# JeremieDona/spatiotemporal_variable_separation

Hardware: AMD Instinct MI355X
Metric: training frames/sec (seq x nt_pred) (higher is better)
Workload: dtype bf16; 1 GPU; waveeq: mlp enc/dec, batch 128/GPU, nt_cond 5, nt_pred 20, offset 5; global_batch=128, parallelism=dp1, grad_allreduce=none (1 rank), launch=hipGraph replay

## Files before the change

### include/varsep_hip.h

```cpp
#ifndef VARSEP_HIP_H
#define VARSEP_HIP_H

#include <stddef.h>
#include <stdint.h>

#ifdef __cplusplus
extern "C" {
#endif

#define VS_OK 0
#define VS_ERR_ARG (-1)
#define VS_ERR_WORKSPACE (-2)
#define VS_ERR_LAUNCH (-3)
#define VS_ERR_UNSUPPORTED (-4)

#define VS_F32 0
#define VS_BF16 1
#define VS_F16 2

#define VS_ACT_NONE 0
#define VS_ACT_RELU 1
#define VS_ACT_LEAKY 2
#define VS_ACT_SIGMOID 3
#define VS_ACT_TANH 4
// ... 83 lines not shown
int vs_conv3_band_bn_supported(int compute, int B, int Cin, int H, int W, int Cout, int groups);
int vs_conv3_band_bn(int compute, const void* x, const void* w_packed, const float* bias, void* y, int y_dtype, int B, int Cin, int H, int W, int Cout,
                     double* bn_sums, int groups, void* stream);
int vs_conv_k4s2_band_bn(int compute, const void* planes, const void* w_packed, const float* bias, void* y, int y_dtype, int B, int K, int H, int W, int M,
                         double* bn_sums, int groups, void* stream);
int vs_bn_stats_from_sums_fold(double* sums, int groups, int C, int64_t n_per_group, float* mean, float* invstd, float* running_mean, float* running_var,
                               float momentum, float eps, int reset, void* stream);
int vs_conv3_band_bn_parts_rows(int B, int H, int W);
int vs_conv3_band_bn_parts(int compute, const void* x, const void* w_packed, const float* bias, void* y, int y_dtype, int B, int Cin, int H, int W, int Cout,
                           float* parts, int k4, void* stream);
int vs_bn_stats_from_parts_fold(const float* parts, int rows_per_group, int groups, int C, int64_t n_per_group, float* mean, float* invstd,
                                float* var_scratch, float* running_mean, float* running_var, float momentum, float eps, void* stream);
int vs_conv3_wgrad_band_slabs(int B, int Cin, int H, int W, int Cout);
int vs_conv3_wgrad_band(int compute, const void* x, const void* dz, float* slabs, int B, int Cin, int H, int W, int Cout, void* stream);
size_t vs_conv3_img16_bn_workspace_bytes(void);
int vs_conv3_img16_bn_supported(int compute, int B, int Cin, int Cout);
int vs_conv3_img16_bn_form_supported(int backward, int act, int y_dtype, int compute);
int vs_exchange_epoch_advance(void* ws, void* stream);
int vs_conv3_img16_bn_fwd(int compute, const void* x, const void* w_packed, void* ws, unsigned call_idx, const float* bias, const float* gamma,
                          const float* beta, int act, float* running_mean, float* running_var, float momentum, float eps, void* z, void* y, int y_dtype,
                          float* mean, float* invstd, const float* skip, float* xnew, void* xnew16, int B, int Cin, int Cout, void* stream);
int vs_conv3_img16_bn_bwd(int compute, const void* dz_next, const void* w_packed, void* ws, unsigned call_idx, const void* z, const float* mean,
                          const float* invstd, const float* gamma, const float* beta, int act, void* dz, float* dgamma, float* dbeta, int accumulate,
                          int B, int Cin, int Cout, void* stream);
int vs_slab_sum(const float* slabs, int nslabs, const float* bias, const float* addend, void* out, int out_dtype, int B, int C, int64_t HW,
                void* stream);
int vs_slab_sum2(const float* slabs, int nslabs, const float* bias, const float* addend, const float* addend2, void* out, int out_dtype, int B, int C,
                 int64_t HW, void* stream);
int vs_bn_stats_from_sums(const double* sums, int groups, int C, int64_t n_per_group, float* mean, float* invstd, float* var_scratch,
                          float* running_mean, float* running_var, float momentum, float eps, void* stream);

int vs_conv_thin_supported(int compute, int B, int C, int H, int W, int M, int k, int stride, int pad);
int vs_conv_thin_expand(int compute, const void* thin, const void* w, int64_t w_sc, int64_t w_sm, int flip, const float* bias, void* out, int out_dtype,
                        int B, int C, int H, int W, int M, int k, int stride, void* stream);
int vs_conv_thin_reduce(int compute, const void* big, const void* w, int64_t w_sc, int64_t w_sm, int flip, const float* bias, void* out, int out_dtype,
                        int B, int C, int H, int W, int M, int k, int stride, void* stream);
size_t vs_conv_thin_wgrad_workspace_bytes(int B, int C, int H, int W, int M, int k);
int vs_conv_thin_wgrad(int compute, const void* big, const void* thin, float* ws, size_t ws_bytes, const float* addend, float* out, int64_t o_sc,
                       int64_t o_sm, int flip, int B, int C, int H, int W, int M, int k, int stride, void* stream);

int vs_frame_metrics(const float* pred, const float* target, int64_t planes, int H, int W, float max_val, float k1, float k2, float sigma,
                     float* mse, float* ssim, void* stream);

int vs_moving_mnist_batch(const uint8_t* digits, int64_t n_digits_total, int digit_h, int digit_w, const int32_t* init, int batch,
                          int num_digits, int seq_len, int frame_size, void* out, int out_dtype, void* stream);

int vs_moving_mnist_testset(const uint8_t* digits, int64_t n_digits_total, int digit_h, int digit_w, const int32_t* init, int n_videos,
                            int num_digits, int seq_len, int frame_size, void* frames, int frames_fp32, int64_t frame_stride_t,
                            int64_t frame_stride_v, int32_t* latents, void* stream);

int vs_chairs_gather(const uint8_t* frames, int64_t n_objects, int views_per_object, int H, int W, int C, const int32_t* desc, int64_t rows,
                     int seq_len, void* out, int out_dtype, int32_t* bad, void* stream);

int vs_gather_timeline(const float* frames, int64_t n_frames, int64_t frame_elems, const int32_t* first, int64_t n_windows, int step,
                       const int32_t* item_idx, int64_t rows, int seq_len, void* out, int out_dtype, int32_t* bad, void* stream);

int vs_wave_simulate(int n_seq, int T, int frame_size, const float* c2, const float* source, const float* h, const float* init, float* out,
                     float* minmax, int normalise, void* stream);

int vs_resample_u8(const uint8_t* src, int64_t n, int H, int W, int C, int box_x0, int box_y0, int box_w, int box_h, const int32_t* kx,
                   const int32_t* bx, int ksize_x, const int32_t* ky, const int32_t* by, int ksize_y, int out_w, int out_h, uint8_t* out,
                   void* stream);

#define VS_INFLATE_OK 0
#define VS_INFLATE_HEADER 1
#define VS_INFLATE_BLOCK_TYPE 2
#define VS_INFLATE_STORED_LEN 3
#define VS_INFLATE_LENGTHS 4
#define VS_INFLATE_SYMBOL 5
#define VS_INFLATE_DISTANCE 6
#define VS_INFLATE_INPUT 7
#define VS_INFLATE_OUT_LONG 8
#define VS_INFLATE_OUT_SHORT 9
#define VS_INFLATE_ADLER 10
#define VS_PNG_BAD_FILTER 11

int vs_inflate_zlib(const uint8_t* packed, int64_t packed_bytes, const int64_t* offsets, int64_t n, const int64_t* out_len, uint8_t* out,
                    int64_t out_stride, int32_t* status, int64_t* produced, void* stream);

int vs_png_unfilter(const uint8_t* raw, int64_t raw_stride, int64_t n, int H, int W, int C, uint8_t* pixels, int32_t* status, void* stream);

#define VS_DEFLATE_MIN_CHUNK 1024
#define VS_DEFLATE_MAX_CHUNK 32768
#define VS_DEFLATE_SLOT_EXTRA 10
int vs_deflate_chunks(const uint8_t* src, int64_t n_bytes, int chunk_bytes, uint8_t* slots, int64_t slot_stride, int64_t* sizes, void* stream);
int vs_deflate_pack(const uint8_t* slots, int64_t slot_stride, const int64_t* sizes, const int64_t* offsets, int64_t n_chunks, uint8_t* dst,
                    int64_t dst_bytes, void* stream);
int vs_crc32(const uint8_t* src, int64_t n_bytes, int64_t chunk_bytes, uint32_t init, uint32_t* partial, void* stream);

#define VS_MT19937_STATE_WORDS 625
#define VS_MT19937_MAX_COLS 8
#define VS_MT19937_MAX_ROWS (1ll << 40)
int vs_mt19937_randint(uint32_t* state, const int32_t* lows, const int32_t* highs, int k, int64_t n_rows, int32_t* out, int32_t* bad,
                       void* stream);

#define VS_MMNIST_WALK_MAX_PRE 5
#define VS_MMNIST_WALK_MAX_TRAJ (1ll << 24)
#define VS_MMNIST_WALK_STATUS_BOUNCE 3
int vs_mmnist_stochastic_trajectories(uint32_t* state, const int32_t* lows, const int32_t* highs, int n_pre, int64_t n_traj, int seq_len,
                                      int x_max, int y_max, int max_speed, const int32_t* start, int32_t* pre, int32_t* positions,
                                      int32_t* latents, int32_t* desc, int desc_nd, int32_t* bad, void* stream);

int vs_moving_mnist_place(const uint8_t* digits, int64_t n_digits_total, int digit_h, int digit_w, const int32_t* positions, int n_seq,
                          int num_digits, const int32_t* desc, int n_videos, int seq_len, int frame_size, void* out, int out_dtype,
                          int32_t* bad, void* stream);
int vs_frame_metrics_multi(const float* pred, const float* targets, int64_t batch, int n_targets, int64_t planes_per_sample, int H, int W,
                           float max_val, float k1, float k2, float sigma, float* mse, float* ssim, void* stream);
int vs_frames_to_u8_nhwc(const void* x, int x_dtype, int64_t n, int channels, int64_t hw, uint8_t* out, void* stream);
int vs_sst_frame_metrics(const float* pred, const float* target, int64_t rows, int T, int H, int W, const float* consts, int64_t n_days,
                         const int32_t* day0, const int32_t* zone, const float* zone_range, int64_t n_zones, float k1, float k2, float sigma,
                         float* mse, float* ssim, int32_t* bad, void* stream);

int vs_mix_codes_fwd(const float* s, const float* t_rand, const float* t_codes, int64_t B, int n, int Cs, int Ct, int mixing, float* out,
                     void* out_lowp, int lowp_dtype, void* stream);
int vs_mix_codes_bwd(const float* dz, const float* s, const float* t_rand, const float* t_codes, int64_t B, int n, int Cs, int Ct,
                     int mixing, float* ds, float* dt_rand, float* dt_codes, void* stream);

int vs_train_losses_fwd(const float* frames, const float* full, const int32_t* idx, const int32_t* t_random_dev, int ae_shift,
                        int first_forecast, int64_t B, int G, int T, int64_t D,
                        const float* s_old, const float* s_new, int64_t n_s, const float* t0, int64_t Bt, int64_t Ct,
                        int average_tloss, const float* lambdas, float* out, void* stream);
int vs_train_losses_bwd(const float* frames, const float* full, const int32_t* idx, const int32_t* t_random_dev, int ae_shift,
                        int first_forecast, int64_t B, int G, int T, int64_t D,
                        const float* s_old, const float* s_new, int64_t n_s, const float* t0, int64_t Bt, int64_t Ct,
                        int average_tloss, const float* lambdas, const float* grad_total, float* dframes, float* ds_old,
                        float* ds_new, float* dt0, int frames_act, void* dz, int dz_dtype, void* stream);
int vs_train_losses_fwd_grad(const float* frames, const float* full, const int32_t* idx, const int32_t* t_random_dev, int ae_shift,
                             int first_forecast, int64_t B, int G, int T, int64_t D, const float* s_old, const float* s_new, int64_t n_s,
                             const float* t0, int64_t Bt, int64_t Ct, int average_tloss, const float* lambdas, float* out,
                             const float* grad_total, float* ds_old, float* ds_new, float* dt0, int frames_act, void* dz, int dz_dtype,
                             void* stream);

int vs_gemm_frame_loss(int compute, int64_t M, int64_t N, int64_t K, const void* A, int64_t lda, const void* W, int64_t ldw,
                       const float* bias, int act, const float* full, const int32_t* t_random_dev, int ae_shift, int first_forecast,
                       int G, int T, const float* s_old, const float* s_new, int64_t n_s, const float* t0, int64_t Bt, int64_t Ct,
                       int average_tloss, const float* lambdas, const float* grad_total, void* dz, int dz_dtype, float* ds_old,
                       float* ds_new, float* dt0, float* out, void* stream);

int vs_adam_multi(int n_tensors, float* const* params, const void* const* grads, const int32_t* grad_dtype, float* const* exp_avg,
                  float* const* exp_avg_sq, void* const* shadow_bf16, const int64_t* numel, const int32_t* skipped, int32_t* step,
                  double lr, double beta1, double beta2, double eps, void* stream);
int vs_adam_step_increment(int32_t* step, void* stream);

int vs_check_finite_multi(int n_tensors, const void* const* grads, const int32_t* grad_dtype, const int64_t* numel, float* found_inf,
                          void* stream);
int vs_adam_multi_scaled(int n_tensors, float* const* params, const void* const* grads, const int32_t* grad_dtype, float* const* exp_avg,
                         float* const* exp_avg_sq, void* const* shadow, int shadow_dtype, const int64_t* numel, const int32_t* skipped,
                         int32_t* step, double lr, double beta1, double beta2, double eps, const float* scale_state, void* stream);
int vs_adam_step_increment_scaled(int32_t* step, const float* scale_state, void* stream);
int vs_adam_set_max_blocks(int blocks);
int vs_gemm_adam(int compute, int64_t M, int64_t N, int64_t K, const void* A, int64_t lda, int layout_a, const void* B, int64_t ldb,
                 int layout_b, float alpha, float* param, float* exp_avg, float* exp_avg_sq, void* shadow, int shadow_dtype,
                 const int32_t* step, int32_t skipped, double lr, double beta1, double beta2, double eps, void* stream);
int vs_loss_scale_update(float* scale_state, float growth_factor, float backoff_factor, int growth_interval, void* stream);

int vs_frames_sse_fwd(const float* frames, const float* full, const int32_t* idx, int64_t B, int G, int T, int64_t D, float* sums,
                      void* stream);
int vs_frames_sse_bwd(const float* frames, const float* full, const int32_t* idx, int64_t B, int G, int T, int64_t D, const float* coef,
                      float* dframes, void* stream);

int vs_cat_bcast_fwd(const void* a, int a_dtype, const void* x, int x_dtype, void* out, int out_dtype, int B, int n, int Ca, int Cb, int64_t HW, void* stream);
int vs_cat_bcast_bwd(const void* dout, int dout_dtype, void* da, int a_dtype, void* dx, int x_dtype, int B, int n, int Ca, int Cb, int64_t HW, void* stream);
int64_t vs_code_losses_chunks(int n_pairs, const int64_t* count, int64_t t_count);
int vs_code_losses_fwd(int n_pairs, const void* const* a, const void* const* b, const int* dtype, const int64_t* count, const float* t0, int64_t t_count,
                       const float* sse_ae, const float* sse_pred, float scale_ae, float scale_pred, float l_ae, float l_s, float l_pred, float l_t,
                       float inv_s, float inv_t, float* partial, float* out, void* stream);
int vs_code_losses_bwd(int n_pairs, const void* const* a, const void* const* b, void* const* da, void* const* db, const int* dtype, const int64_t* count,
                       const float* t0, float* dt0, int64_t t_count, const float* g, float scale_ae, float scale_pred, float l_ae, float l_s, float l_pred,
                       float l_t, float inv_s, float inv_t, float* coefs, void* stream);

int vs_act_bwd(const void* dy, int dy_dtype, const void* y, int y_dtype, void* dz, int dz_dtype, int act,
               int64_t n, void* stream);

int vs_act_fwd(const void* x, int x_dtype, void* y, int y_dtype, int act, int64_t n, void* stream);

int vs_transpose_cast(const void* src, int src_dtype, void* dst, int dst_dtype, int rows, int cols, void* stream);

size_t vs_rollout_packed_elems(int compute, int N, int K);
int vs_pack_rollout_weight(int compute, const float* src, int transpose, int N, int K, void* dst, void* stream);
int vs_pack_rollout_weights(int compute, int n_jobs, const float* const* src, const int* transpose, const int* N, const int* K,
                            void* const* dst, void* stream);

int vs_mlp_rollout_parts(int compute, int B, int C, int H);
size_t vs_mlp_rollout_workspace_bytes(int compute, int B, int C, int H);
int vs_mlp_rollout_xcd_local_get(int compute, int B, int C, int H, int n_blocks);
int vs_mlp_rollout_xcd_local_set(int allowed);
int vs_exchange_guard_set(void* word);
void* vs_exchange_guard_get(void);
int vs_exchange_skip_counter_set(void* word);
int vs_mlp_rollout_fwd(int compute, int B, int C, int H, int n_blocks, int n_steps, const float* x0,
                       const void* const* weights, const float* const* biases, float* t_codes, float* residuals,
                       void* xin_save, void* h1_save, void* h2_save, uint32_t* m1_save, uint32_t* m2_save, void* workspace,
                       size_t workspace_bytes, void* stream);

int vs_mlp_rollout_bwd(int compute, int B, int C, int H, int n_blocks, int n_steps, const float* grad_t_codes,
                       const void* const* weights_t, const void* h1_save, const void* h2_save,
                       const uint32_t* m1_save, const uint32_t* m2_save, float* dx0,
                       void* dr_save, void* dh2_save, void* dh1_save, void* workspace, size_t workspace_bytes, void* stream);

size_t vs_conv_workspace_bytes(int compute, int B, int Cin, int H, int W, int Cout, int kh, int kw, int stride, int pad);
size_t vs_conv_wgrad_workspace_bytes(int B, int Cin, int OH, int OW, int Cout, int kh, int kw);
size_t vs_conv_packed_elems(int D0, int D1, int kh, int kw, int stride, int pad);
int vs_conv_pack_weight(int compute, const float* w, int D0, int D1, int kh, int kw, int stride, int pad, void* dst, void* stream);
int vs_conv2d_fwd(int compute, const void* x, const void* w, const float* bias, void* y, int y_dtype, int B, int Cin, int H, int W,
                  int Cout, int kh, int kw, int stride, int pad, void* workspace, size_t workspace_bytes, void* stream);
int vs_conv2d_dgrad(int compute, const void* dy, const void* w_packed, void* dx, int dx_dtype, int B, int Cin, int H, int W, int Cout, int kh,
                    int kw, int stride, int pad, void* workspace, size_t workspace_bytes, void* stream);
int vs_conv2d_wgrad(int compute, const void* dy, const void* x, float* dw, int B, int Cin, int H, int W, int Cout, int kh, int kw,
                    int stride, int pad, void* workspace, size_t workspace_bytes, void* stream);
int vs_conv2d_wgrad_acc(int compute, const void* dy, const void* x, float* dw, int B, int Cin, int H, int W, int Cout, int kh, int kw,
                        int stride, int pad, void* workspace, size_t workspace_bytes, int accumulate, void* stream);
int vs_conv_transpose2d_wgrad_acc(int compute, const void* dy, const void* x, float* dw, int B, int Cin, int H, int W, int Cout, int kh,
                                  int kw, int stride, int pad, void* workspace, size_t workspace_bytes, int accumulate, void* stream);
int vs_conv_transpose2d_fwd(int compute, const void* x, const void* w_packed, const float* bias, void* y, int y_dtype, int B, int Cin, int H,
                            int W, int Cout, int kh, int kw, int stride, int pad, void* workspace, size_t workspace_bytes, void* stream);
int vs_conv_transpose2d_dgrad(int compute, const void* dy, const void* w, void* dx, int dx_dtype, int B, int Cin, int H, int W, int Cout,
                              int kh, int kw, int stride, int pad, void* workspace, size_t workspace_bytes, int cols_from_wgrad, void* stream);
int vs_conv_transpose2d_wgrad(int compute, const void* dy, const void* x, float* dw, int B, int Cin, int H, int W, int Cout, int kh,
                              int kw, int stride, int pad, void* workspace, size_t workspace_bytes, void* stream);

int vs_maxpool3s2_fwd(const void* x, int x_dtype, void* y, int y_dtype, int64_t planes, int H, int W, void* stream);
int vs_maxpool3s2_bwd(const void* x, int x_dtype, const void* dy, int dy_dtype, void* dx, int dx_dtype, int64_t planes, int H, int W,
                      void* stream);

int vs_bn_stats(const void* x, int x_dtype, int B, int C, int64_t HW, int groups, float* mean, float* invstd, float* var_scratch,
                float* running_mean, float* running_var, float momentum, float eps, void* stream);
int vs_bn_train_fwd_small_supported(int x_dtype, int B, int C, int64_t HW);
int vs_bn_train_fwd_small(const void* x, int x_dtype, void* y, int y_dtype, const float* gamma, const float* beta, int act, float* mean,
                          float* invstd, float* running_mean, float* running_var, float momentum, float eps, int B, int C, int64_t HW,
                          void* stream);
int vs_bn_train_fwd_small_groups(const void* x, int x_dtype, void* y, int y_dtype, const float* gamma, const float* beta, int act, float* mean,
                                 float* invstd, float* var_scratch, float* running_mean, float* running_var, float momentum, float eps, int B, int C,
                                 int64_t HW, int groups, void* stream);
int vs_bn_train_fwd_small_slabs(const float* slabs, int nslabs, const float* bias, void* z, int z_dtype, void* y, int y_dtype, const float* gamma,
                                const float* beta, int act, float* mean, float* invstd, float* running_mean, float* running_var,
                                float momentum, float eps, const float* skip, float* xnew, void* xnew16, int B, int C, int64_t HW,
                                void* stream);
int vs_bn_act_bwd_small_ex(const void* dy_a, int dy_a_dtype, const float* dy_b, const float* slabs, int nslabs, const void* z, int z_dtype,
                           const float* mean, const float* invstd, const float* gamma, const float* beta, int act, float* dgamma,
                           float* dbeta, int accumulate, void* dx, int dx_dtype, int B, int C, int64_t HW, void* stream);
int vs_bn_train_fwd_slab_supported(int x_dtype, int Bg, int C, int64_t HW);
int vs_bn_train_fwd_slab(const void* x, int x_dtype, void* y, int y_dtype, const float* gamma, const float* beta, int act, float* mean, float* invstd,
                         float* var_scratch, float* running_mean, float* running_var, float momentum, float eps, int B, int C, int64_t HW, int groups,
                         void* stream);
int vs_bn_act_fwd(const void* x, int x_dtype, void* y, int y_dtype, const float* mean, const float* invstd, const float* gamma,
                  const float* beta, int act, int B, int C, int64_t HW, int groups, void* stream);
int vs_bn_act_bwd(const void* dy, int dy_dtype, const void* x, int x_dtype, const float* mean, const float* invstd, const float* gamma,
                  const float* beta, int act, int training, int groups, float* dgamma, float* dbeta, void* dx, int dx_dtype, int B,
                  int C, int64_t HW, void* stream);
int vs_bn_act_bwd_gsum(const void* dy, int dy_dtype, const void* x, int x_dtype, const float* mean, const float* invstd, const float* gamma,
                       const float* beta, int act, int training, int groups, float* dgamma, float* dbeta, void* dx, int dx_dtype, int B,
                       int C, int64_t HW, float* dgamma_sum, float* dbeta_sum, void* stream);
int vs_bn_stats_ub(const void* x, int x_dtype, int B, int C, int64_t HW, int groups, float* mean, float* invstd, float* ubvar, float eps, void* stream);
int vs_bn_act_fwd_running(const void* x, int x_dtype, void* y, int y_dtype, const float* mean, const float* invstd, const float* gamma, const float* beta,
                          int act, int B, int C, int64_t HW, int groups, const float* ubvar, float* running_mean, float* running_var, float momentum,
                          void* stream);
int vs_chan_sum(const void* x, int x_dtype, int B, int C, int64_t HW, float* out, void* stream);
size_t vs_chan_sum_workspace_bytes(int B, int C, int64_t HW);
int vs_chan_sum_ws(const void* x, int x_dtype, int B, int C, int64_t HW, void* ws, size_t ws_bytes, float* out, void* stream);
int vs_maxpool2_fwd(const void* x, int x_dtype, void* y, int y_dtype, int64_t planes, int H, int W, void* stream);
int vs_maxpool2_bwd(const void* x, int x_dtype, const void* dy, int dy_dtype, void* dx, int dx_dtype, int64_t planes, int H, int W,
                    void* stream);
int vs_upsample2_fwd(const void* x, int x_dtype, void* y, int y_dtype, int64_t planes, int H, int W, void* stream);
int vs_upsample2_bwd(const void* dy, int dy_dtype, void* dx, int dx_dtype, int64_t planes, int H, int W, void* stream);

#ifdef __cplusplus
}
#endif
#endif
```

### spatiotemporal_variable_separation_amd/_lib.py

```python
import ctypes
import os
import subprocess
import sys
from concurrent.futures import ThreadPoolExecutor

import torch

_HERE = os.path.dirname(os.path.abspath(__file__))
_CSRC = os.path.join(_HERE, 'csrc')
LIB_PATH = os.path.join(_HERE, 'libvarsep_hip.so')
SOURCES = ['vs_gemm.hip', 'vs_eltwise.hip', 'vs_conv.hip', 'vs_rollout.hip', 'vs_norm.hip', 'vs_optim.hip', 'vs_data.hip', 'vs_conv_tap.hip', 'vs_metrics.hip', 'vs_conv_img.hip', 'vs_conv_k4s2.hip',
           'vs_conv_thin.hip', 'vs_conv_band2.hip', 'vs_conv_wgrad2.hip', 'vs_eval.hip', 'vs_wave_sim.hip', 'vs_resample.hip', 'vs_png.hip', 'vs_deflate.hip',
           'vs_mt19937.hip', 'vs_mmnist_walk.hip']

F32, BF16, F16 = 0, 1, 2
TORCH_DTYPE = {F32: torch.float32, BF16: torch.bfloat16, F16: torch.float16}
ACT = {'none': 0, None: 0, 'identity': 0, 'relu': 1, 'leaky_relu': 2, 'sigmoid': 3, 'tanh': 4, 'elu': 5}
LAYOUT_R, LAYOUT_S = 0, 1

_lib = None


class VarsepHipError(RuntimeError):
    pass


def _sources():
    return [os.path.join(_CSRC, s) for s in SOURCES if os.path.exists(os.path.join(_CSRC, s))]


def _headers():
    import glob
    return sorted(glob.glob(os.path.join(_CSRC, '*.h'))) + [os.path.join(_HERE, '..', 'include', 'varsep_hip.h')]


def _deps(src, _seen=None):
    import re
    seen = _seen if _seen is not None else set()
    if src in seen or not os.path.exists(src):
        return seen
    seen.add(src)
    with open(src, errors='replace') as f:
        for name in re.findall(r'^\s*#\s*include\s+"([^"]+)"', f.read(), flags=re.M):
            for d in (os.path.dirname(src), _CSRC, os.path.join(_HERE, '..', 'include')):
                cand = os.path.normpath(os.path.join(d, name))
                if os.path.exists(cand):
                    _deps(cand, seen)
                    break
    return seen


def library_is_stale():
    if not os.path.exists(LIB_PATH):
        return True
    t = os.path.getmtime(LIB_PATH)
    return any(os.path.getmtime(d) > t for d in _sources() + _headers())


def build_library(force=False, verbose=False):
    if not force and not library_is_stale():
        return LIB_PATH
    hipcc = os.environ.get('HIPCC', '/opt/rocm/bin/hipcc')
    objdir = os.path.join(_HERE, 'build')
    os.makedirs(objdir, exist_ok=True)
    flags = ['--offload-arch=gfx950', '-O3', '-std=c++17', '-fPIC'] + os.environ.get('VARSEP_HIPCC_FLAGS', '').split()

    def compile_one(src):
        obj = os.path.join(objdir, os.path.basename(src) + '.o')
        if not force and os.path.exists(obj) and os.path.getmtime(obj) > max(os.path.getmtime(d) for d in _deps(src)):
            return obj
        cmd = [hipcc] + flags + ['-c', src, '-o', obj]
        r = subprocess.run(cmd, capture_output=True, text=True)
        if r.returncode != 0:
            raise VarsepHipError('hipcc failed for %s:\n%s' % (src, r.stderr[-4000:]))
        if verbose:
            print('compiled', os.path.basename(src), file=sys.stderr)
        return obj

    with ThreadPoolExecutor(max_workers=4) as ex:
        objs = list(ex.map(compile_one, _sources()))
    tmp = LIB_PATH + '.tmp'
    r = subprocess.run([hipcc, '--offload-arch=gfx950', '-shared', '-fPIC', '-o', tmp] + objs, capture_output=True, text=True)
    if r.returncode != 0:
        raise VarsepHipError('link failed:\n' + r.stderr[-4000:])
    os.replace(tmp, LIB_PATH)
    return LIB_PATH


_i64, _i32, _f32, _vp, _sz = ctypes.c_int64, ctypes.c_int, ctypes.c_float, ctypes.c_void_p, ctypes.c_size_t

SIGNATURES = {
    'vs_version': (ctypes.c_char_p, []),
    'vs_last_error': (ctypes.c_char_p, []),
    'vs_gemm_workspace_bytes': (_sz, [_i64, _i64, _i64]),
    'vs_gemm_plan': (_i32, [_i32, _i32, _i64, _i64, _i64, _vp, _i64, _i64, _i32, _vp, _i64, _i64, _i32, ctypes.POINTER(_i64)]),
    'vs_gemm': (_i32, [_i32, _i64, _i64, _i64, _vp, _i64, _i32, _vp, _i64, _i32, _vp, _i64, _i32, _f32, _vp, _i32,
                       _vp, _i64, _i32, _i32, _i32, _vp, _sz, _vp]),
    'vs_cast': (_i32, [_vp, _i32, _vp, _i32, _i64, _vp]),
    'vs_copy2d': (_i32, [_vp, _i32, _i64, _vp, _i32, _i64, _i64, _i64, _vp, _i64, _vp]),
    'vs_copy2d_pair': (_i32, [_vp, _i32, _i64, _vp, _i32, _i64, _i64, _i64, _vp, _i64, _i64, _i64, _vp]),
    'vs_colsum': (_i32, [_vp, _i32, _i64, _i64, _i64, _vp, _i32, _vp]),
    'vs_colsum_multi': (_i32, [_i32, _vp, _vp, _vp, _vp, _vp, _vp, _vp, _i64, _vp]),
    'vs_adam_multi': (_i32, [_i32, _vp, _vp, _vp, _vp, _vp, _vp, _vp, _vp, _vp, ctypes.c_double, ctypes.c_double, ctypes.c_double,
                             ctypes.c_double, _vp]),
    'vs_adam_step_increment': (_i32, [_vp, _vp]),
    'vs_check_finite_multi': (_i32, [_i32, _vp, _vp, _vp, _vp, _vp]),
    'vs_adam_set_max_blocks': (_i32, [_i32]),
    'vs_gemm_adam': (_i32, [_i32, _i64, _i64, _i64, _vp, _i64, _i32, _vp, _i64, _i32, ctypes.c_float, _vp, _vp, _vp, _vp, _i32, _vp, _i32,
                     ctypes.c_double, ctypes.c_double, ctypes.c_double, ctypes.c_double, _vp]),
    'vs_adam_multi_scaled': (_i32, [_i32, _vp, _vp, _vp, _vp, _vp, _vp, _i32, _vp, _vp, _vp, ctypes.c_double, ctypes.c_double, ctypes.c_double,
                                    ctypes.c_double, _vp, _vp]),
    'vs_adam_step_increment_scaled': (_i32, [_vp, _vp, _vp]),
    'vs_loss_scale_update': (_i32, [_vp, _f32, _f32, _i32, _vp]),
    'vs_gemm_batched_workspace_bytes': (_sz, [_i32, _i64, _i64, _i64]),
    'vs_gemm_batched': (_i32, [_i32, _i32, _i64, _i64, _i64, _vp, _i64, _i64, _i32, _vp, _i64, _i64, _i32, _vp, _i64, _i64, _i32, _f32, _i32,
                               _vp, _sz, _vp]),
    'vs_train_losses_fwd': (_i32, [_vp, _vp, _vp, _vp, _i32, _i32, _i64, _i32, _i32, _i64, _vp, _vp, _i64, _vp, _i64, _i64, _i32, _vp, _vp, _vp]),
    'vs_train_losses_fwd_grad': (_i32, [_vp, _vp, _vp, _vp, _i32, _i32, _i64, _i32, _i32, _i64, _vp, _vp, _i64, _vp, _i64, _i64, _i32, _vp, _vp,
                                        _vp, _vp, _vp, _vp, _i32, _vp, _i32, _vp]),
    'vs_gemm_frame_loss': (_i32, [_i32, _i64, _i64, _i64, _vp, _i64, _vp, _i64, _vp, _i32, _vp, _vp, _i32, _i32, _i32, _i32, _vp, _vp, _i64, _vp, _i64,
                                  _i64, _i32, _vp, _vp, _vp, _i32, _vp, _vp, _vp, _vp, _vp]),
    'vs_train_losses_bwd': (_i32, [_vp, _vp, _vp, _vp, _i32, _i32, _i64, _i32, _i32, _i64, _vp, _vp, _i64, _vp, _i64, _i64, _i32, _vp, _vp, _vp, _vp,
                                   _vp, _vp, _i32, _vp, _i32, _vp]),
    'vs_convt_tap_supported': (_i32, [_i32] * 7),
    'vs_convt_tap_packed_elems': (_sz, [_i32, _i32]),
    'vs_convt_tap_pack_weight': (_i32, [_i32, _vp, _i32, _i32, _vp, _vp]),
    'vs_convt_k4s2_tap_fwd': (_i32, [_i32, _vp, _vp, _vp, _vp, _vp] + [_i32] * 6 + [_vp]),
    'vs_convt_k4s2_tap_fwd_f32': (_i32, [_i32, _vp, _vp, _vp, _vp] + [_i32] * 5 + [_vp]),
    'vs_conv_k3_tap_supported': (_i32, [_i32] * 7),
    'vs_conv_k3_tap_packed_elems': (_sz, [_i32, _i32]),
    'vs_conv_k3_tap_pack_weight': (_i32, [_i32, _vp, _i32, _i32, _i32, _vp, _vp]),
    'vs_conv_k3s1_tap_fwd': (_i32, [_i32, _vp, _vp, _vp, _vp, _i32, _vp] + [_i32] * 6 + [_vp]),
    'vs_bn_stats_from_sums': (_i32, [_vp, _i32, _i32, _i64, _vp, _vp, _vp, _vp, _vp, _f32, _f32, _vp]),
    'vs_moving_mnist_batch': (_i32, [_vp, _i64, _i32, _i32, _vp, _i32, _i32, _i32, _i32, _vp, _i32, _vp]),
    'vs_moving_mnist_testset': (_i32, [_vp, _i64, _i32, _i32, _vp, _i32, _i32, _i32, _i32, _vp, _i32, _i64, _i64, _vp, _vp]),
    'vs_chairs_gather': (_i32, [_vp, _i64, _i32, _i32, _i32, _i32, _vp, _i64, _i32, _vp, _i32, _vp, _vp]),
    'vs_gather_timeline': (_i32, [_vp, _i64, _i64, _vp, _i64, _i32, _vp, _i64, _i32, _vp, _i32, _vp, _vp]),
    'vs_gather_windows': (_i32, [_vp, _i64, _i64, _i64, _vp, _i32, _i32, _i32, _vp, _i32, _vp, _i32, _vp]),
    'vs_wave_simulate': (_i32, [_i32, _i32, _i32, _vp, _vp, _vp, _vp, _vp, _vp, _i32, _vp]),
    'vs_resample_u8': (_i32, [_vp, _i64, _i32, _i32, _i32, _i32, _i32, _i32, _i32, _vp, _vp, _i32, _vp, _vp, _i32, _i32, _i32, _vp, _vp]),
    'vs_inflate_zlib': (_i32, [_vp, _i64, _vp, _i64, _vp, _vp, _i64, _vp, _vp, _vp]),
    'vs_png_unfilter': (_i32, [_vp, _i64, _i64, _i32, _i32, _i32, _vp, _vp, _vp]),
    'vs_deflate_chunks': (_i32, [_vp, _i64, _i32, _vp, _i64, _vp, _vp]),
    'vs_deflate_pack': (_i32, [_vp, _i64, _vp, _vp, _i64, _vp, _i64, _vp]),
    'vs_crc32': (_i32, [_vp, _i64, _i64, ctypes.c_uint32, _vp, _vp]),
    'vs_mt19937_randint': (_i32, [_vp, _vp, _vp, _i32, _i64, _vp, _vp, _vp]),
    'vs_mmnist_stochastic_trajectories': (_i32, [_vp, _vp, _vp, _i32, _i64, _i32, _i32, _i32, _i32, _vp, _vp, _vp, _vp, _vp, _i32, _vp, _vp]),
    'vs_mix_codes_fwd': (_i32, [_vp, _vp, _vp, _i64, _i32, _i32, _i32, _i32, _vp, _vp, _i32, _vp]),
    'vs_mix_codes_bwd': (_i32, [_vp, _vp, _vp, _vp, _i64, _i32, _i32, _i32, _i32, _vp, _vp, _vp, _vp]),
    'vs_pack_rollout_weights': (_i32, [_i32, _i32, _vp, _vp, _vp, _vp, _vp, _vp]),
    'vs_frames_sse_fwd': (_i32, [_vp, _vp, _vp, _i64, _i32, _i32, _i64, _vp, _vp]),
    'vs_frames_sse_bwd': (_i32, [_vp, _vp, _vp, _i64, _i32, _i32, _i64, _vp, _vp, _vp]),
    'vs_cat_bcast_fwd': (_i32, [_vp, _i32, _vp, _i32, _vp, _i32, _i32, _i32, _i32, _i32, _i64, _vp]),
    'vs_cat_bcast_bwd': (_i32, [_vp, _i32, _vp, _i32, _vp, _i32, _i32, _i32, _i32, _i32, _i64, _vp]),
    'vs_code_losses_chunks': (_i64, [_i32, _vp, _i64]),
    'vs_code_losses_fwd': (_i32, [_i32, _vp, _vp, _vp, _vp, _vp, _i64, _vp, _vp, ctypes.c_float, ctypes.c_float, ctypes.c_float, ctypes.c_float, ctypes.c_float, ctypes.c_float, ctypes.c_float, ctypes.c_float, _vp, _vp, _vp]),
    'vs_code_losses_bwd': (_i32, [_i32, _vp, _vp, _vp, _vp, _vp, _vp, _vp, _vp, _i64, _vp, ctypes.c_float, ctypes.c_float, ctypes.c_float, ctypes.c_float, ctypes.c_float, ctypes.c_float, ctypes.c_float, ctypes.c_float, _vp, _vp]),
    'vs_act_bwd': (_i32, [_vp, _i32, _vp, _i32, _vp, _i32, _i32, _i64, _vp]),
    'vs_act_fwd': (_i32, [_vp, _i32, _vp, _i32, _i32, _i64, _vp]),
    'vs_conv_wgrad_workspace_bytes': (_sz, [_i32] * 7),
    'vs_conv_packed_elems': (_sz, [_i32] * 6),
    'vs_conv_pack_weight': (_i32, [_i32, _vp, _i32, _i32, _i32, _i32, _i32, _i32, _vp, _vp]),
    'vs_conv_workspace_bytes': (_sz, [_i32] * 10),
    'vs_conv2d_fwd': (_i32, [_i32, _vp, _vp, _vp, _vp, _i32] + [_i32] * 9 + [_vp, _sz, _vp]),
    'vs_conv2d_dgrad': (_i32, [_i32, _vp, _vp, _vp, _i32] + [_i32] * 9 + [_vp, _sz, _vp]),
    'vs_conv2d_wgrad': (_i32, [_i32, _vp, _vp, _vp] + [_i32] * 9 + [_vp, _sz, _vp]),
    'vs_frame_metrics': (_i32, [_vp, _vp, _i64, _i32, _i32, ctypes.c_float, ctypes.c_float, ctypes.c_float, ctypes.c_float, _vp, _vp, _vp]),
    'vs_moving_mnist_place': (_i32, [_vp, _i64, _i32, _i32, _vp, _i32, _i32, _vp, _i32, _i32, _i32, _vp, _i32, _vp, _vp]),
    'vs_frame_metrics_multi': (_i32, [_vp, _vp, _i64, _i32, _i64, _i32, _i32, _f32, _f32, _f32, _f32, _vp, _vp, _vp]),
    'vs_frames_to_u8_nhwc': (_i32, [_vp, _i32, _i64, _i32, _i64, _vp, _vp]),
    'vs_sst_frame_metrics': (_i32, [_vp, _vp, _i64, _i32, _i32, _i32, _vp, _i64, _vp, _vp, _vp, _i64, _f32, _f32, _f32, _vp, _vp, _vp, _vp]),
    'vs_conv3_img16_supported': (_i32, [_i32] * 6),
    'vs_conv3_img16_splits': (_i32, [_i32] * 3),
    'vs_conv3_img16_packed_elems': (_sz, [_i32, _i32]),
    'vs_conv3_img16_pack_weight': (_i32, [_i32, _vp, _i32, _i32, _i32, _vp, _vp]),
    'vs_conv3_img16_pack_weights': (_i32, [_i32, _i32, _vp, _vp, _vp, _vp, _vp, _vp]),
    'vs_conv3_img16': (_i32, [_i32, _vp, _vp, _vp, _i32, _i32, _i32, _vp]),
    'vs_space_to_depth2_supported': (_i32, [_i32] * 5),
    'vs_space_to_depth2': (_i32, [_i32, _vp, _vp, _i32, _i32, _i32, _i32, _vp]),
    'vs_conv_k4s2_packed_elems': (_sz, [_i32, _i32]),
    'vs_conv_k4s2_pack_weight': (_i32, [_i32, _vp, _i32, _i32, _vp, _vp]),
    'vs_conv_k4s2_wgrad_finish': (_i32, [_vp, _i32, _vp, _vp, _i32, _i32, _vp]),
    'vs_conv_k4s2_skip_form': (_i32, [_i32]),
    'vs_conv_k4s2_band': (_i32, [_i32, _vp, _vp, _vp, _vp, _i32, _i32, _i32, _i32, _i32, _i32, _vp]),
    'vs_conv_k4s2_wgrad_band': (_i32, [_i32, _vp, _vp, _vp, _i32, _i32, _i32, _i32, _i32, _vp]),
    'vs_conv_k4s2_wgrad_band_slabs': (_i32, [_i32, _i32, _i32, _i32, _i32]),
    'vs_conv_thin_supported': (_i32, [_i32] * 9),
    'vs_conv_thin_expand': (_i32, [_i32, _vp, _vp, _i64, _i64, _i32, _vp, _vp, _i32] + [_i32] * 7 + [_vp]),
    'vs_conv_thin_reduce': (_i32, [_i32, _vp, _vp, _i64, _i64, _i32, _vp, _vp, _i32] + [_i32] * 7 + [_vp]),
    'vs_conv_thin_wgrad_workspace_bytes': (_sz, [_i32] * 6),
    'vs_conv_thin_wgrad': (_i32, [_i32, _vp, _vp, _vp, _sz, _vp, _vp, _i64, _i64, _i32] + [_i32] * 7 + [_vp]),
    'vs_conv3_band_supported': (_i32, [_i32] * 6),
    'vs_conv3_band_bn_supported': (_i32, [_i32] * 7),
    'vs_conv3_band_bn': (_i32, [_i32, _vp, _vp, _vp, _vp, _i32, _i32, _i32, _i32, _i32, _i32, _vp, _i32, _vp]),
    'vs_conv_k4s2_band_bn': (_i32, [_i32, _vp, _vp, _vp, _vp, _i32, _i32, _i32, _i32, _i32, _i32, _vp, _i32, _vp]),
    'vs_bn_stats_from_sums_fold': (_i32, [_vp, _i32, _i32, _i64, _vp, _vp, _vp, _vp, ctypes.c_float, ctypes.c_float, _i32, _vp]),
    'vs_conv3_band_bn_parts_rows': (_i32, [_i32, _i32, _i32]),
    'vs_conv3_band_bn_parts': (_i32, [_i32, _vp, _vp, _vp, _vp, _i32, _i32, _i32, _i32, _i32, _i32, _vp, _i32, _vp]),
    'vs_bn_stats_from_parts_fold': (_i32, [_vp, _i32, _i32, _i32, _i64, _vp, _vp, _vp, _vp, _vp, ctypes.c_float, ctypes.c_float, _vp]),
    'vs_conv3_band': (_i32, [_i32, _vp, _vp, _vp, _vp, _i32, _i32, _i32, _i32, _i32, _i32, _vp]),
    'vs_conv3_wgrad_band_supported': (_i32, [_i32] * 6),
    'vs_conv3_wgrad_band_slabs': (_i32, [_i32] * 5),
    'vs_conv3_wgrad_band': (_i32, [_i32, _vp, _vp, _vp, _i32, _i32, _i32, _i32, _i32, _vp]),
    'vs_conv3_wgrad_band_pieces': (_i32, [_i32, _i32, _vp, _vp, _i32, _vp, _i32, _i32, _i32, _i32, _vp]),
    'vs_conv3_wgrad_band_finish': (_i32, [_vp, _i32, _vp, _vp, _i32, _i32, _vp]),
    'vs_slab_sum_grouped': (_i32, [_vp, _i32, _i32, _vp, _i64, _vp]),
    'vs_slab_sum': (_i32, [_vp, _i32, _vp, _vp, _vp, _i32, _i32, _i32, _i64, _vp]),
    'vs_slab_sum2': (_i32, [_vp, _i32, _vp, _vp, _vp, _vp, _i32, _i32, _i32, _i64, _vp]),
    'vs_conv3_img16_bn_workspace_bytes': (ctypes.c_size_t, []),
    'vs_conv3_img16_bn_supported': (_i32, [_i32, _i32, _i32, _i32]),
    'vs_conv3_img16_bn_form_supported': (_i32, [_i32, _i32, _i32, _i32]),
    'vs_exchange_epoch_advance': (_i32, [_vp, _vp]),
    'vs_conv3_img16_bn_fwd': (_i32, [_i32, _vp, _vp, _vp, ctypes.c_uint, _vp, _vp, _vp, _i32, _vp, _vp, ctypes.c_float, ctypes.c_float, _vp, _vp, _i32,
                                     _vp, _vp, _vp, _vp, _vp, _i32, _i32, _i32, _vp]),
    'vs_conv3_img16_bn_bwd': (_i32, [_i32, _vp, _vp, _vp, ctypes.c_uint, _vp, _vp, _vp, _vp, _vp, _i32, _vp, _vp, _vp, _i32, _i32, _i32, _i32, _vp]),
    'vs_bn_train_fwd_small_slabs': (_i32, [_vp, _i32, _vp, _vp, _i32, _vp, _i32, _vp, _vp, _i32, _vp, _vp, _vp, _vp, ctypes.c_float, ctypes.c_float,
                                           _vp, _vp, _vp, _i32, _i32, _i64, _vp]),
    'vs_bn_act_bwd_small_ex': (_i32, [_vp, _i32, _vp, _vp, _i32, _vp, _i32, _vp, _vp, _vp, _vp, _i32, _vp, _vp, _i32, _vp, _i32, _i32, _i32, _i64, _vp]),
    'vs_bn_train_fwd_small_supported': (_i32, [_i32, _i32, _i32, _i64]),
    'vs_bn_train_fwd_small': (_i32, [_vp, _i32, _vp, _i32, _vp, _vp, _i32, _vp, _vp, _vp, _vp, ctypes.c_float, ctypes.c_float, _i32, _i32, _i64, _vp]),
    'vs_bn_train_fwd_small_groups': (_i32, [_vp, _i32, _vp, _i32, _vp, _vp, _i32, _vp, _vp, _vp, _vp, _vp, ctypes.c_float, ctypes.c_float, _i32, _i32, _i64, _i32,
                                            _vp]),
    'vs_conv2d_wgrad_acc': (_i32, [_i32, _vp, _vp, _vp] + [_i32] * 9 + [_vp, _sz, _i32, _vp]),
    'vs_conv_transpose2d_wgrad_acc': (_i32, [_i32, _vp, _vp, _vp] + [_i32] * 9 + [_vp, _sz, _i32, _vp]),
    'vs_conv_transpose2d_fwd': (_i32, [_i32, _vp, _vp, _vp, _vp, _i32] + [_i32] * 9 + [_vp, _sz, _vp]),
    'vs_conv_transpose2d_dgrad': (_i32, [_i32, _vp, _vp, _vp, _i32] + [_i32] * 9 + [_vp, _sz, _i32, _vp]),
    'vs_conv_transpose2d_wgrad': (_i32, [_i32, _vp, _vp, _vp] + [_i32] * 9 + [_vp, _sz, _vp]),
    'vs_bn_stats': (_i32, [_vp, _i32, _i32, _i32, _i64, _i32, _vp, _vp, _vp, _vp, _vp, _f32, _f32, _vp]),
    'vs_bn_train_fwd_slab_supported': (_i32, [_i32, _i32, _i32, _i64]),
    'vs_bn_train_fwd_slab': (_i32, [_vp, _i32, _vp, _i32, _vp, _vp, _i32, _vp, _vp, _vp, _vp, _vp, ctypes.c_float, ctypes.c_float, _i32, _i32, _i64, _i32, _vp]),
    'vs_bn_act_fwd': (_i32, [_vp, _i32, _vp, _i32, _vp, _vp, _vp, _vp, _i32, _i32, _i32, _i64, _i32, _vp]),
    'vs_bn_act_bwd': (_i32, [_vp, _i32, _vp, _i32, _vp, _vp, _vp, _vp, _i32, _i32, _i32, _vp, _vp, _vp, _i32, _i32, _i32, _i64, _vp]),
    'vs_bn_act_bwd_gsum': (_i32, [_vp, _i32, _vp, _i32, _vp, _vp, _vp, _vp, _i32, _i32, _i32, _vp, _vp, _vp, _i32, _i32, _i32, _i64, _vp, _vp, _vp]),
    'vs_bn_stats_ub': (_i32, [_vp, _i32, _i32, _i32, _i64, _i32, _vp, _vp, _vp, ctypes.c_float, _vp]),
    'vs_bn_act_fwd_running': (_i32, [_vp, _i32, _vp, _i32, _vp, _vp, _vp, _vp, _i32, _i32, _i32, _i64, _i32, _vp, _vp, _vp, ctypes.c_float, _vp]),
    'vs_chan_sum': (_i32, [_vp, _i32, _i32, _i32, _i64, _vp, _vp]),
    'vs_chan_sum_workspace_bytes': (_sz, [_i32, _i32, _i64]),
    'vs_chan_sum_ws': (_i32, [_vp, _i32, _i32, _i32, _i64, _vp, _sz, _vp, _vp]),
    'vs_maxpool2_fwd': (_i32, [_vp, _i32, _vp, _i32, _i64, _i32, _i32, _vp]),
    'vs_maxpool2_bwd': (_i32, [_vp, _i32, _vp, _i32, _vp, _i32, _i64, _i32, _i32, _vp]),
    'vs_maxpool3s2_fwd': (_i32, [_vp, _i32, _vp, _i32, _i64, _i32, _i32, _vp]),
    'vs_maxpool3s2_bwd': (_i32, [_vp, _i32, _vp, _i32, _vp, _i32, _i64, _i32, _i32, _vp]),
    'vs_upsample2_fwd': (_i32, [_vp, _i32, _vp, _i32, _i64, _i32, _i32, _vp]),
    'vs_upsample2_bwd': (_i32, [_vp, _i32, _vp, _i32, _i64, _i32, _i32, _vp]),
    'vs_transpose_cast': (_i32, [_vp, _i32, _vp, _i32, _i32, _i32, _vp]),
    'vs_rollout_packed_elems': (_sz, [_i32, _i32, _i32]),
    'vs_pack_rollout_weight': (_i32, [_i32, _vp, _i32, _i32, _i32, _vp, _vp]),
    'vs_mlp_rollout_parts': (_i32, [_i32] * 4),
    'vs_mlp_rollout_workspace_bytes': (_sz, [_i32] * 4),
    'vs_mlp_rollout_xcd_local_get': (_i32, [_i32] * 5),
    'vs_mlp_rollout_xcd_local_set': (_i32, [_i32]),
    'vs_exchange_guard_set': (_i32, [_vp]),
    'vs_exchange_guard_get': (_vp, []),
    'vs_exchange_skip_counter_set': (_i32, [_vp]),
    'vs_mlp_rollout_fwd': (_i32, [_i32] * 6 + [_vp] * 11 + [_sz, _vp]),
    'vs_mlp_rollout_bwd': (_i32, [_i32] * 6 + [_vp] * 11 + [_sz, _vp]),
}


def load_library():
    global _lib
    if _lib is not None:
# ... 46 lines not shown
```

### spatiotemporal_variable_separation_amd/csrc/vs_gemm.hip

```cpp
#include <type_traits>
#include "vs_gemm_plan.h"
#include "vs_loss.h"

namespace {

struct GemmCall {
    const void* A; int64_t lda; int la;
    const void* B; int64_t ldb; int lb;
    int64_t M, N, K;
    int batch;
    hipStream_t stream;
};

template <int V> using IC = std::integral_constant<int, V>;
template <class F>
int with_compute(int compute, F&& f) {
    return compute == VS_BF16 ? f(IC<VS_BF16>{}) : compute == VS_F16 ? f(IC<VS_F16>{}) : f(IC<VS_F32>{});
}
template <class F>
int with_types(int compute, int la, int lb, F&& f) {
    return with_compute(compute, [&](auto ct) {
        if (la == LR && lb == LR) return f(ct, IC<LR>{}, IC<LR>{});
        if (la == LR && lb == LS) return f(ct, IC<LR>{}, IC<LS>{});
        if (la == LS && lb == LR) return f(ct, IC<LS>{}, IC<LR>{});
        return f(ct, IC<LS>{}, IC<LS>{});
    });
}

template <int CT, int LA, int LB, int BM, int BN>
int launch(const GemmCall& c, const GemmPlan& plan, const Epi& epi, float* slabs) {
    typedef typename CTraits<CT>::T T;
    constexpr int BK = bk_of<CT>();
    constexpr int U = CTraits<CT>::U;
    Dense<CT, LA> a{(const T*)c.A, c.lda, c.M, c.K, ((uintptr_t)c.A % 16 == 0) && (c.lda % U == 0) && (epi.batch_a % U == 0)};
    Dense<CT, LB> b{(const T*)c.B, c.ldb, c.N, c.K, ((uintptr_t)c.B % 16 == 0) && (c.ldb % U == 0) && (epi.batch_b % U == 0)};
    constexpr size_t smem = (TileGeom<CT, LA, BM, BK>::ELEMS + TileGeom<CT, LB, BN, BK>::ELEMS) * sizeof(T);
    dim3 grid((unsigned)vs_cdiv(c.N, BN), (unsigned)vs_cdiv(c.M, BM), (unsigned)(plan.splits * c.batch));
    Epi e = epi;
    e.xcd_runs = (int64_t)grid.x * grid.y * grid.z >= 64;
    hipLaunchKernelGGL((gemm_kernel<CT, Dense<CT, LA>, Dense<CT, LB>, BM, BN, BK>), grid, dim3(256), smem, c.stream, a, b, c.M, c.N,
                       c.K, (int)plan.k_tiles_per_split, e, slabs);
    VS_CHECK_LAUNCH("vs_gemm");
    return VS_OK;
}

template <int CT, int LA, int LB>
int launch_reg(const GemmCall& c, const GemmPlan& plan, const Epi& epi, float* slabs) {
    if (plan.bm == 128 && plan.bn == 128) return launch<CT, LA, LB, 128, 128>(c, plan, epi, slabs);
    if (plan.bm == 128 && plan.bn == 64) return launch<CT, LA, LB, 128, 64>(c, plan, epi, slabs);
    if constexpr (CT != VS_F32)
        if (plan.bm == 64 && plan.bn == 128) return launch<CT, LA, LB, 64, 128>(c, plan, epi, slabs);
    return launch<CT, LA, LB, 64, 64>(c, plan, epi, slabs);
}

template <int CT, int LA, int LB>
int launch_glds(const GemmCall& c, const GemmPlan& plan, const Epi& epi, float* slabs) {
    if constexpr (CT == VS_F32) {
        return vs_fail(VS_ERR_UNSUPPORTED, "vs_gemm: the LDS-DMA 128x128 tile is a 16-bit kernel");
    } else {
        dim3 grid((unsigned)vs_cdiv(c.N, 128), (unsigned)vs_cdiv(c.M, 128), (unsigned)(plan.splits * c.batch));
        static const int forced = getenv("VS_GEMM_GLDS_STAGES") ? atoi(getenv("VS_GEMM_GLDS_STAGES")) : 0;
        const int stages = forced ? forced : ((int64_t)grid.x * grid.y * grid.z >= 1024 ? 2 : 1);
        if (stages == 2)
            hipLaunchKernelGGL((gemm_glds_kernel<LA, LB, false, 2, CT>), grid, dim3(256), 65536, c.stream, (const __bf16*)c.A, c.lda, (const __bf16*)c.B,
                               c.ldb, c.M, c.N, c.K, (int)plan.k_tiles_per_split, epi, slabs);
        else
            hipLaunchKernelGGL((gemm_glds_kernel<LA, LB, false, 1, CT>), grid, dim3(256), 32768, c.stream, (const __bf16*)c.A, c.lda, (const __bf16*)c.B,
                               c.ldb, c.M, c.N, c.K, (int)plan.k_tiles_per_split, epi, slabs);
        VS_CHECK_LAUNCH("vs_gemm (LDS-DMA tile)");
        return VS_OK;
    }
}

template <int CT, int LA, int LB, bool LOSS = false>
int launch_big(const GemmCall& c, const GemmPlan& bp, const Epi& epi, float* slabs) {
    if constexpr (CT == VS_F32) {
        return vs_fail(VS_ERR_UNSUPPORTED, "vs_gemm: the 256x256 tile is a 16-bit kernel");
    } else {
        auto kfn = gemm_big_kernel<CT, LA, LB, false, LOSS>;
        static bool attr_set = false;
        if (!attr_set) {
            if (hipFuncSetAttribute((const void*)kfn, hipFuncAttributeMaxDynamicSharedMemorySize, GEMM_BIG_STAGES * BIG_TILE_BYTES) != hipSuccess)
                return vs_fail(VS_ERR_LAUNCH, "vs_gemm: cannot raise the dynamic LDS limit to 160 KiB");
            attr_set = true;
        }
        dim3 grid((unsigned)(bp.tiles_m * bp.tiles_n), 1, (unsigned)(bp.splits * c.batch));
        hipLaunchKernelGGL(kfn, grid, dim3(512), GEMM_BIG_STAGES * BIG_TILE_BYTES, c.stream, (const unsigned short*)c.A, c.lda, (const unsigned short*)c.B,
                           c.ldb, c.M, c.N, c.K, (int)bp.k_tiles_per_split, bp.tiles_n, epi, slabs);
        VS_CHECK_LAUNCH("vs_gemm (256x256 tile)");
        return VS_OK;
    }
}

template <int CT, int LA, int LB, int NI, int LOSS = 0, int MI = 4>
int launch_p8(const GemmCall& c, const GemmPlan& pp, const Epi& epi, float* slabs) {
    if constexpr (CT == VS_F32) {
        return vs_fail(VS_ERR_UNSUPPORTED, "vs_gemm: the staggered 256-row tile is a 16-bit kernel");
    } else {
        auto kfn = gemm_p8_kernel<CT, LA, LB, NI, false, LOSS, MI>;
        constexpr int lds = 2 * (2 * 32 * MI * P8_BK * 2 + 2 * 64 * NI * P8_BK * 2);
        static bool attr_set = false;
        if (!attr_set) {
            if (hipFuncSetAttribute((const void*)kfn, hipFuncAttributeMaxDynamicSharedMemorySize, lds) != hipSuccess)
                return vs_fail(VS_ERR_LAUNCH, "vs_gemm: cannot raise the dynamic LDS limit to %d bytes", lds);
            attr_set = true;
        }
        dim3 grid((unsigned)(pp.tiles_m * pp.tiles_n), 1, (unsigned)(pp.splits * c.batch));
        hipLaunchKernelGGL(kfn, grid, dim3(512), lds, c.stream, (const unsigned short*)c.A, c.lda, (const unsigned short*)c.B, c.ldb, c.M, c.N, c.K,
                           (int)pp.k_tiles_per_split, pp.tiles_n, epi, slabs);
        VS_CHECK_LAUNCH("vs_gemm (staggered 256-row tile)");
        return VS_OK;
    }
}

template <int CT, int LA, int LB>
int launch_mid(const GemmCall& c, const GemmPlan& mp, const Epi& epi, float* slabs) {
    const int rc = mid_launch<CT, LA, LB>(c.A, c.lda, c.B, c.ldb, c.M, c.N, c.K, mp.splits, mp.k_tiles_per_split, mp.stages, c.batch, epi, slabs, c.stream);
    if (rc != VS_OK) return rc;
    VS_CHECK_LAUNCH("vs_gemm (128x128 ring tile)");
    return VS_OK;
}

int launch_plan(int compute, const GemmCall& c, const GemmPlan& p, const Epi& epi, float* slabs) {
    return with_types(compute, c.la, c.lb, [&](auto ct, auto la, auto lb) -> int {
        constexpr int CT = decltype(ct)::value, LA = decltype(la)::value, LB = decltype(lb)::value;
        switch (p.kind) {
            case GEMM_P8:
                if (p.ni == 1 && p.mi == 2) return launch_p8<CT, LA, LB, 1, 0, 2>(c, p, epi, slabs);
                if (p.ni == 1) return launch_p8<CT, LA, LB, 1>(c, p, epi, slabs);
                return launch_p8<CT, LA, LB, 2>(c, p, epi, slabs);
            case GEMM_BIG: return launch_big<CT, LA, LB>(c, p, epi, slabs);
            case GEMM_MID: return launch_mid<CT, LA, LB>(c, p, epi, slabs);
            case GEMM_GLDS: return launch_glds<CT, LA, LB>(c, p, epi, slabs);
            default: return launch_reg<CT, LA, LB>(c, p, epi, slabs);
        }
    });
}

constexpr unsigned SK_POOL = 1u << 20;
}
__device__ unsigned vs_sk_pool[1u << 20];
namespace {

constexpr int64_t SK_FUSED_MAX_BYTES = 96 << 10;
unsigned* sk_take(int64_t words, int64_t tile_slab_bytes) {
    static unsigned* base = nullptr;
    static unsigned next = 0;
    const char* env = getenv("VS_GEMM_SPLITK_FUSED");
    const int fused = env ? atoi(env) : 0;
    if (!fused || words <= 0 || words > SK_POOL / 4 || (fused == 1 && tile_slab_bytes > SK_FUSED_MAX_BYTES)) return nullptr;
    if (!base && hipGetSymbolAddress((void**)&base, HIP_SYMBOL(vs_sk_pool)) != hipSuccess) { base = nullptr; return nullptr; }
    if (next + words > SK_POOL) next = 0;
    unsigned* p = base + next;
    next += (unsigned)words;
    return p;
}

int run_gemm(const char* who, int compute, const GemmCall& c, const GemmPlan& plan, Epi epi, void* workspace, size_t workspace_bytes) {
    float* slabs = nullptr;
    if (plan.splits > 1) {
        const size_t need = gemm_slab_bytes(plan, c.M, c.N, c.batch);
        if (!workspace || workspace_bytes < need)
            return vs_fail(VS_ERR_WORKSPACE, "%s: split-K needs %zu workspace bytes, got %zu", who, need, workspace_bytes);
        slabs = (float*)workspace;
        if (gemm_splitk_in_launch(plan)) {
            epi.sk_counters = sk_take(gemm_splitk_counters(plan, c.M, c.N, c.batch), gemm_splitk_tile_bytes(plan));
            epi.sk_splits = plan.splits;
            epi.sk_bytes = (int64_t)need;
        }
    }
    const int rc = launch_plan(compute, c, plan, epi, slabs);
    if (rc != VS_OK) return rc;
    if (slabs && !epi.sk_counters) return launch_splitk_reduce(slabs, plan.splits, c.M, c.N, epi, c.batch, c.stream);
    return VS_OK;
}

}

extern "C" size_t vs_gemm_workspace_bytes(int64_t M, int64_t N, int64_t K) { return gemm_workspace_bytes(M, N, K, 1); }
extern "C" size_t vs_gemm_batched_workspace_bytes(int batch, int64_t M, int64_t N, int64_t K) { return gemm_workspace_bytes(M, N, K, batch); }

extern "C" int vs_gemm_plan(int compute, int batch, int64_t M, int64_t N, int64_t K, const void* A, int64_t lda, int64_t stride_a, int layout_a,
                            const void* B, int64_t ldb, int64_t stride_b, int layout_b, int64_t* out) {
    VS_CHECK_ARG(vs_dtype_ok(compute), "vs_gemm_plan: compute type %d", compute);
    VS_CHECK_ARG(batch >= 1 && batch <= 1024 && M > 0 && N > 0 && K > 0, "vs_gemm_plan: bad sizes");
    VS_CHECK_ARG((layout_a == LR || layout_a == LS) && (layout_b == LR || layout_b == LS), "vs_gemm_plan: bad layout");
    VS_CHECK_ARG(out, "vs_gemm_plan: null pointer");
    const GemmPlan p = plan_gemm(compute, M, N, K, batch, A, lda, layout_a, stride_a, B, ldb, layout_b, stride_b);
    const int64_t row[12] = {p.kind, p.bm, p.bn, p.splits, p.k_tiles_per_split, p.tiles_m, p.tiles_n, p.stages, p.ni, p.mi,
                             gemm_splitk_in_launch(p) && gemm_splitk_counters(p, M, N, batch) > 0, (int64_t)gemm_slab_bytes(p, M, N, batch)};
    memcpy(out, row, sizeof(row));
    return VS_OK;
}

extern "C" int vs_gemm_batched(int compute, int batch, int64_t M, int64_t N, int64_t K, const void* A, int64_t lda, int64_t stride_a,
                               int layout_a, const void* B, int64_t ldb, int64_t stride_b, int layout_b, void* C, int64_t ldc,
                               int64_t stride_c, int c_dtype, float alpha, int accumulate, void* workspace, size_t workspace_bytes,
                               void* stream_) {
    VS_CHECK_ARG(vs_dtype_ok(compute), "vs_gemm_batched: compute type %d", compute);
    VS_CHECK_ARG(batch >= 1 && batch <= 1024 && M > 0 && N > 0 && K > 0, "vs_gemm_batched: bad sizes");
    VS_CHECK_ARG(A && B && C, "vs_gemm_batched: null operand");
    VS_CHECK_ARG((layout_a == LR || layout_a == LS) && (layout_b == LR || layout_b == LS), "vs_gemm_batched: bad layout");
    VS_CHECK_ARG(vs_dtype_ok(c_dtype), "vs_gemm_batched: bad c_dtype");
    VS_CHECK_ARG(lda >= (layout_a == LR ? K : M) && ldb >= (layout_b == LR ? K : N) && ldc >= N, "vs_gemm_batched: leading dimension too small");
    const GemmPlan plan = plan_gemm(compute, M, N, K, batch, A, lda, layout_a, stride_a, B, ldb, layout_b, stride_b);
    Epi epi = plain_epi(C, ldc, c_dtype, alpha);
    epi.accumulate = accumulate;
    epi.splits_per_batch = plan.splits;
    epi.batch_a = stride_a; epi.batch_b = stride_b; epi.batch_c = stride_c;
    const GemmCall call{A, lda, layout_a, B, ldb, layout_b, M, N, K, batch, (hipStream_t)stream_};
    return run_gemm("vs_gemm_batched", compute, call, plan, epi, workspace, workspace_bytes);
}

extern "C" int vs_gemm_adam(int compute, int64_t M, int64_t N, int64_t K, const void* A, int64_t lda, int layout_a, const void* B, int64_t ldb,
                            int layout_b, float alpha, float* param, float* exp_avg, float* exp_avg_sq, void* shadow, int shadow_dtype,
                            const int32_t* step, int32_t skipped, double lr, double beta1, double beta2, double eps, void* stream_) {
    VS_CHECK_ARG(compute == VS_BF16 || compute == VS_F16, "vs_gemm_adam: 16-bit compute types only (%d)", compute);
    VS_CHECK_ARG(M > 0 && N > 0 && K > 0, "vs_gemm_adam: M, N, K must be positive");
    VS_CHECK_ARG(A && B && param && exp_avg && exp_avg_sq && step, "vs_gemm_adam: null pointer");
    VS_CHECK_ARG((layout_a == LR || layout_a == LS) && (layout_b == LR || layout_b == LS), "vs_gemm_adam: bad layout");
    VS_CHECK_ARG(lda >= (layout_a == LR ? K : M) && ldb >= (layout_b == LR ? K : N), "vs_gemm_adam: leading dimension too small");
    VS_CHECK_ARG(!shadow || shadow_dtype == VS_BF16 || shadow_dtype == VS_F16, "vs_gemm_adam: bad shadow dtype");
    if (!dma_operands_ok(GEMM_MID, A, lda, layout_a, 0, B, ldb, layout_b, 0, M, N, K))
        return vs_fail(VS_ERR_UNSUPPORTED, "vs_gemm_adam: operands do not fit the LDS-DMA loader (16-byte alignment, multiples of 8)");
    Epi epi = plain_epi(param, N, VS_F32, alpha);
    epi.adam_m = exp_avg; epi.adam_v = exp_avg_sq; epi.adam_shadow = (unsigned short*)shadow; epi.adam_shadow_dtype = shadow_dtype;
    epi.adam_step = step; epi.adam_skipped = skipped; epi.adam_guard = vs_g_exchange_guard;
    epi.adam_lr = lr; epi.adam_beta1 = beta1; epi.adam_beta2 = beta2; epi.adam_eps = (float)eps;
    const GemmPlan mp = ring_plan_one_split(M, N, K);
    if ((int64_t)mp.tiles_m * mp.tiles_n > 0x7fffffffll) return vs_fail(VS_ERR_UNSUPPORTED, "vs_gemm_adam: too many tiles");
    const GemmCall call{A, lda, layout_a, B, ldb, layout_b, M, N, K, 1, (hipStream_t)stream_};
    return launch_plan(compute, call, mp, epi, nullptr);
}

extern "C" int vs_gemm_frame_loss(int compute, int64_t M, int64_t N, int64_t K, const void* A, int64_t lda, const void* W, int64_t ldw,
                                  const float* bias, int act, const float* full, const int32_t* t_random_dev, int ae_shift, int first_forecast,
                                  int G, int T, const float* s_old, const float* s_new, int64_t n_s, const float* t0, int64_t Bt, int64_t Ct,
                                  int average_tloss, const float* lambdas, const float* grad_total, void* dz, int dz_dtype, float* ds_old,
                                  float* ds_new, float* dt0, float* out, void* stream_) {
    hipStream_t stream = (hipStream_t)stream_;
    VS_CHECK_ARG(compute == VS_BF16 || compute == VS_F16, "vs_gemm_frame_loss: 16-bit compute types only (%d)", compute);
    VS_CHECK_ARG(M > 0 && M < (1ll << 31) && N > 0 && K > 0 && G >= 1 && M % G == 0 && N % 4 == 0, "vs_gemm_frame_loss: bad sizes (rows = B * G, N %% 4 == 0)");
    VS_CHECK_ARG(!bias || ((uintptr_t)bias & 15) == 0, "vs_gemm_frame_loss: the bias must be 16-byte aligned");
    VS_CHECK_ARG(A && W && full && t_random_dev && grad_total && dz && dt0 && out && (n_s == 0 || (ds_old && ds_new)), "vs_gemm_frame_loss: null pointer");
    VS_CHECK_ARG(lda >= K && ldw >= K, "vs_gemm_frame_loss: leading dimension too small");
    VS_CHECK_ARG(vs_dtype_ok(dz_dtype) && act >= VS_ACT_NONE && act <= VS_ACT_ELU, "vs_gemm_frame_loss: bad dz dtype / activation");
    LossArgs a;
    int rc = fill_loss_args(a, nullptr, full, nullptr, t_random_dev, ae_shift, first_forecast, M / G, G, T, N, s_old, s_new, n_s, t0, Bt, Ct,
                            average_tloss, lambdas);
    if (rc != VS_OK) return rc;
    const GemmPlan pp = p8_plan(compute, M, N, K, 1), bp = big_plan(compute, M, N, K, 1);
    auto takes = [&](const GemmPlan& p) {
        return p.use && dma_operands_ok(p.kind, A, lda, LR, 0, W, ldw, LR, 0, M, N, K) && p.splits == 1 && (int64_t)p.tiles_m * p.tiles_n <= VS_LOSS_MAX_PARTIALS;
    };
    const bool p8 = takes(pp) && pp.ni == 2;
    if (!p8 && !takes(bp)) return vs_fail(VS_ERR_UNSUPPORTED, "vs_gemm_frame_loss: the problem does not run on the 256x256 tile kernels");
    Epi epi = plain_epi(nullptr, N, VS_F32, 1.f);
    epi.bias = bias; epi.act = act;
    epi.fl_full = full; epi.fl_tdev = t_random_dev; epi.fl_ae_shift = ae_shift; epi.fl_first = first_forecast; epi.fl_G = G; epi.fl_T = T;
    epi.fl_up = grad_total; epi.fl_l_ae = a.l_ae; epi.fl_l_pred = a.l_pred; epi.fl_inv_ae = a.inv_ae; epi.fl_inv_pred = a.inv_pred;
    epi.fl_dz = dz; epi.fl_dz_dtype = dz_dtype; epi.fl_partials = out + 16;
    const GemmCall call{A, lda, LR, W, ldw, LR, M, N, K, 1, stream};
    rc = with_compute(compute, [&](auto ct) -> int {
        constexpr int CT = decltype(ct)::value;
        if (p8 && act == VS_ACT_SIGMOID) return launch_p8<CT, LR, LR, 2, 2>(call, pp, epi, nullptr);
        if (p8) return launch_p8<CT, LR, LR, 2, 1>(call, pp, epi, nullptr);
        return launch_big<CT, LR, LR, true>(call, bp, epi, nullptr);
    });
    if (rc != VS_OK) return rc;
    LossGrads gr{grad_total, dz, dz_dtype, act, ds_old, ds_new, dt0};
    hipLaunchKernelGGL(frame_loss_finish_kernel, dim3(1), dim3(256), 0, stream, a, out, p8 ? pp.tiles_m * pp.tiles_n : bp.tiles_m * bp.tiles_n, gr);
    VS_CHECK_LAUNCH("vs_gemm_frame_loss");
    return VS_OK;
}

extern "C" int vs_gemm(int compute, int64_t M, int64_t N, int64_t K, const void* A, int64_t lda, int layout_a, const void* B,
                       int64_t ldb, int layout_b, void* C, int64_t ldc, int c_dtype, float alpha, const float* bias, int act,
                       const void* mask, int64_t ldmask, int mask_dtype, int mask_act, int accumulate, void* workspace,
                       size_t workspace_bytes, void* stream_) {
    VS_CHECK_ARG(vs_dtype_ok(compute), "vs_gemm: compute type %d", compute);
    VS_CHECK_ARG(M > 0 && N > 0 && K > 0, "vs_gemm: M, N, K must be positive (%lld %lld %lld)", (long long)M, (long long)N, (long long)K);
    VS_CHECK_ARG(A && B && C, "vs_gemm: null operand");
    VS_CHECK_ARG((layout_a == LR || layout_a == LS) && (layout_b == LR || layout_b == LS), "vs_gemm: bad layout");
    VS_CHECK_ARG(vs_dtype_ok(c_dtype) && (!mask || vs_dtype_ok(mask_dtype)), "vs_gemm: bad c_dtype / mask_dtype");
    VS_CHECK_ARG(lda >= (layout_a == LR ? K : M) && ldb >= (layout_b == LR ? K : N) && ldc >= N, "vs_gemm: leading dimension too small");
    VS_CHECK_ARG(!mask || ldmask >= N, "vs_gemm: ldmask too small");
    VS_CHECK_ARG(act >= VS_ACT_NONE && act <= VS_ACT_ELU, "vs_gemm: bad activation");
    Epi epi = plain_epi(C, ldc, c_dtype, alpha);
    epi.bias = bias; epi.act = act;
    epi.mask = mask; epi.ldmask = ldmask; epi.mask_dtype = mask_dtype; epi.mask_act = mask_act;
    epi.accumulate = accumulate;
    const GemmPlan plan = plan_gemm(compute, M, N, K, 1, A, lda, layout_a, 0, B, ldb, layout_b, 0);
    const GemmCall call{A, lda, layout_a, B, ldb, layout_b, M, N, K, 1, (hipStream_t)stream_};
    return run_gemm("vs_gemm", compute, call, plan, epi, workspace, workspace_bytes);
}
```

### spatiotemporal_variable_separation_amd/csrc/vs_gemm_big.h

```cpp
#pragma once
#include <type_traits>
#include "vs_gemm_glds.h"

namespace {

constexpr int BIG_BK = 32;
constexpr int BIG_STAGES = 4;
#define VS_GB_ST 5
#define VS_GB_WAIT_FIRST 16
#define VS_GB_WAIT_LOOP 12
#define VS_STR_(x) #x
#define VS_STR(x) VS_STR_(x)
static_assert(VS_GB_WAIT_FIRST == 4 * (VS_GB_ST - 1) && VS_GB_WAIT_LOOP == 4 * (VS_GB_ST - 2), "vmcnt immediates follow the ring depth");
constexpr int GEMM_BIG_STAGES = VS_GB_ST;
constexpr int BIG_TILE_BYTES = 4 * 8192;

template <int LAYOUT>
struct BigOperand {
    const char* base;
    uint32_t voff[2];
    int kofs;
    int64_t step;

    __device__ __forceinline__ void prepare(const unsigned short* p, int64_t ld, int64_t rows, int64_t i0, int64_t k_begin) {
        const int u = (int)threadIdx.x;
#pragma unroll
        for (int h = 0; h < 2; ++h) {
            const int64_t first = i0 + 128 * h;
            if (LAYOUT == LR) {
                const int row = u >> 2, piece = (u & 3) ^ ((row >> 2) & 3);
                int64_t r = first + row;
                if (r > rows - 1) r = rows - 1;
                kofs = piece * 8;
                voff[h] = (uint32_t)(((r - i0) * ld + piece * 8) * 2);
            } else {
                const int k = u >> 4, piece = (u & 15) ^ ((k & 3) << 2);
                int64_t c = first + piece * 8;
                if (c > rows - 8) c = rows - 8;
                kofs = k;
                voff[h] = (uint32_t)((k * ld + (c - i0)) * 2);
            }
        }
        if (LAYOUT == LR) {
            base = reinterpret_cast<const char*>(p + i0 * ld + k_begin);
            step = BIG_BK * 2;
        } else {
            base = reinterpret_cast<const char*>(p + k_begin * ld + i0);
            step = BIG_BK * ld * 2;
        }
    }
    __device__ __forceinline__ void advance() { base += step; }
    __device__ __forceinline__ void stage(int h, char* lds) const {
        const uint32_t dst = (uint32_t)(uintptr_t)lds;
        asm volatile("s_mov_b32 m0, %0\n\ts_nop 0\n\tglobal_load_lds_dwordx4 %1, %2" ::"s"(dst), "v"(voff[h]), "s"(base) : "memory", "m0");
    }
    __device__ __forceinline__ void stage_checked(int h, char* lds, int64_t k0, int64_t K, bool live) const {
        const void* g = (live && k0 + kofs < K) ? (const void*)(base + voff[h]) : (const void*)vs_glds_zero;
        const uint32_t dst = (uint32_t)(uintptr_t)lds;
        asm volatile("s_mov_b32 m0, %0\n\ts_nop 0\n\tglobal_load_lds_dwordx4 %1, off" ::"s"(dst), "v"(g) : "memory", "m0");
    }
};

template <int LAYOUT>
__device__ __forceinline__ u32x4 big_frag(const unsigned short* tile, int row0, int kk, int lane) {
    if (LAYOUT == LR) {
        const int row = row0 + (lane & 31), q = (kk >> 3) + (lane >> 5);
        return *reinterpret_cast<const u32x4*>(tile + row * 32 + ((q ^ ((row >> 2) & 3)) << 3));
    } else {
        const int li = lane & 15, q = li >> 2, p = li & 3, cb = (lane >> 4) & 1, h = lane >> 5;
        const int k1 = kk + 8 * h + q;
        const int rowoff = row0 + 16 * cb + 4 * p;
        const int slot = (rowoff >> 3) ^ ((k1 & 3) << 2);
        return vs_tr16_pair(tile + k1 * 128 + slot * 8 + (rowoff & 7), 4 * 128);
    }
}


__device__ __forceinline__ void big_adam4(const Epi& e, const AdamCoef& c, int64_t m, int64_t n, int64_t N, const f32x4& g) {
    const int64_t idx = m * e.ldc + n;
    float* P = (float*)e.C + idx;
    float* Mo = e.adam_m + idx;
    float* Vo = e.adam_v + idx;
    if (n + 3 < N && (e.ldc & 3) == 0 && (n & 3) == 0) {
        f32x4 p = *reinterpret_cast<const f32x4*>(P), mm = *reinterpret_cast<const f32x4*>(Mo), vv = *reinterpret_cast<const f32x4*>(Vo);
#pragma unroll
        for (int t = 0; t < 4; ++t) {
            float pe = p[t], me = mm[t], ve = vv[t];
            vs_adam_elem(c, g[t] * e.alpha, pe, me, ve);
            p[t] = pe; mm[t] = me; vv[t] = ve;
        }
        *reinterpret_cast<f32x4*>(P) = p;
        *reinterpret_cast<f32x4*>(Mo) = mm;
        *reinterpret_cast<f32x4*>(Vo) = vv;
        if (e.adam_shadow) {
            const u16x4 h = {vs_f2h(p[0], e.adam_shadow_dtype), vs_f2h(p[1], e.adam_shadow_dtype), vs_f2h(p[2], e.adam_shadow_dtype),
                             vs_f2h(p[3], e.adam_shadow_dtype)};
            *reinterpret_cast<u16x4*>(e.adam_shadow + idx) = h;
        }
    } else {
        for (int t = 0; t < 4; ++t)
            if (n + t < N) {
                float pe = P[t], me = Mo[t], ve = Vo[t];
                vs_adam_elem(c, g[t] * e.alpha, pe, me, ve);
                P[t] = pe; Mo[t] = me; Vo[t] = ve;
                if (e.adam_shadow) e.adam_shadow[idx + t] = vs_f2h(pe, e.adam_shadow_dtype);
            }
    }
}

template <bool NCHW>
__device__ __forceinline__ void big_store4(const Epi& e, int64_t m, int64_t n, int64_t N, const f32x4& v, float* slab_row, const float* through = nullptr,
                                           int64_t through_bytes = 0) {
    if (slab_row) {
        if (through) {
            const auto rs = sk_rsrc(through, through_bytes);
            const int64_t e = (slab_row + n) - through;
            if (n + 3 < N && ((uintptr_t)(slab_row + n) & 15) == 0) sk_store4(rs, e, v);
            else
                for (int t = 0; t < 4; ++t)
                    if (n + t < N) sk_store(rs, e + t, v[t]);
            return;
        }
        if (n + 3 < N && ((uintptr_t)(slab_row + n) & 15) == 0) *reinterpret_cast<f32x4*>(slab_row + n) = v;
        else
            for (int t = 0; t < 4; ++t)
                if (n + t < N) slab_row[n + t] = v[t];
        return;
    }
    if constexpr (NCHW) {
        if (n + 3 < N && e.g_hw == 0 && (e.nchw_hw & 3) == 0 && (n & 3) == 0 && !e.mask && !e.accumulate && ((uintptr_t)e.C & 15) == 0) {
            const int64_t idx = nchw_col_base(e, n) + m * e.nchw_hw;
            const float bsv = e.bias ? e.bias[m] : 0.f;
            f32x4 r;
#pragma unroll
            for (int t = 0; t < 4; ++t) r[t] = vs_act(v[t] * e.alpha + bsv, e.act);
            if (e.c_dtype == VS_F32) {
                *reinterpret_cast<f32x4*>((float*)e.C + idx) = r;
            } else {
                const u16x4 h = {vs_f2h(r[0], e.c_dtype), vs_f2h(r[1], e.c_dtype), vs_f2h(r[2], e.c_dtype), vs_f2h(r[3], e.c_dtype)};
                *reinterpret_cast<u16x4*>((unsigned short*)e.C + idx) = h;
            }
        } else {
            for (int t = 0; t < 4; ++t)
                if (n + t < N) epi_store_nchw(e, m, nchw_col_base(e, n + t), v[t]);
        }
    } else {
        const bool vec = n + 3 < N && ((e.ldc | n) & 3) == 0 && !e.mask && !e.accumulate && ((uintptr_t)e.C & 15) == 0;
        if (vec) {
            f32x4 r;
#pragma unroll
            for (int t = 0; t < 4; ++t) {
                float x = v[t] * e.alpha;
                if (e.bias) x += e.bias[n + t];
                r[t] = vs_act(x, e.act);
            }
            if (e.c_dtype == VS_F32) {
                *reinterpret_cast<f32x4*>((float*)e.C + m * e.ldc + n) = r;
            } else {
                const u16x4 h = {vs_f2h(r[0], e.c_dtype), vs_f2h(r[1], e.c_dtype), vs_f2h(r[2], e.c_dtype), vs_f2h(r[3], e.c_dtype)};
                *reinterpret_cast<u16x4*>((unsigned short*)e.C + m * e.ldc + n) = h;
            }
        } else {
            for (int t = 0; t < 4; ++t)
                if (n + t < N) epi_store(e, m, n + t, v[t]);
        }
    }
}

__device__ __forceinline__ const float* big_loss_target(const Epi& e, int64_t m, int64_t n, int64_t N, int t_rand, int& g_out) {
    const unsigned b = (unsigned)m / (unsigned)e.fl_G;
    const int g = (int)((unsigned)m - b * (unsigned)e.fl_G);
    const int frame = g == 0 ? t_rand - e.fl_ae_shift : e.fl_first + g - 1;
    g_out = g;
    return e.fl_full + ((int64_t)b * e.fl_T + frame) * N + n;
}
__device__ __forceinline__ void big_loss4(const Epi& e, int64_t m, int64_t n, int64_t N, int g, const f32x4& v, const f32x4& t, const f32x4& bias4, float up,
                                          float& s0, float& s1) {
    const float k = g == 0 ? up * e.fl_l_ae * 2.f * e.fl_inv_ae : up * e.fl_l_pred * 2.f * e.fl_inv_pred;
    float rr[4], s = 0.f;
#pragma unroll
    for (int j = 0; j < 4; ++j) {
        const float x = vs_act(v[j] * e.alpha + bias4[j], e.act);
        const float d = x - t[j];
        s += d * d;
        rr[j] = (k * d) * vs_act_grad_from_out(x, e.act);
    }
    if (g == 0) s0 += s; else s1 += s;
    const int64_t o = m * N + n;
    if (e.fl_dz_dtype == VS_F32) *reinterpret_cast<f32x4*>((float*)e.fl_dz + o) = f32x4{rr[0], rr[1], rr[2], rr[3]};
    else {
        const u16x4 w = {vs_f2h(rr[0], e.fl_dz_dtype), vs_f2h(rr[1], e.fl_dz_dtype), vs_f2h(rr[2], e.fl_dz_dtype), vs_f2h(rr[3], e.fl_dz_dtype)};
        *reinterpret_cast<u16x4*>((unsigned short*)e.fl_dz + o) = w;
    }
}

#define VS_FENCE __builtin_amdgcn_sched_barrier(0)

template <int CT, int LA, int LB, bool NCHW, bool LOSS = false>
__global__ __launch_bounds__(512) void gemm_big_kernel(const unsigned short* Ap, int64_t lda, const unsigned short* Bp, int64_t ldb, int64_t M, int64_t N,
                                                       int64_t K, int k_tiles_per_split, int tiles_n, Epi epi_in, float* slabs) {
    int zsplit = blockIdx.z;
    int batch = 0;
    if (epi_in.splits_per_batch > 0) {
        batch = blockIdx.z / epi_in.splits_per_batch;
        zsplit = blockIdx.z - batch * epi_in.splits_per_batch;
        Ap += batch * epi_in.batch_a;
        Bp += batch * epi_in.batch_b;
    }
    const Epi epi = epi_for_batch(epi_in, batch);
    extern __shared__ __attribute__((aligned(16))) char smem[];

    const int lane = threadIdx.x & 63;
    const int wave = __builtin_amdgcn_readfirstlane((int)(threadIdx.x >> 6));
    const int wr = wave >> 2, wc = wave & 3;
    const unsigned tile = big_tile_of(blockIdx.x, gridDim.x);
    const int64_t m0 = (int64_t)(tile / (unsigned)tiles_n) * 256, n0 = (int64_t)(tile % (unsigned)tiles_n) * 256;
    const int64_t kt_total = (K + BIG_BK - 1) / BIG_BK;
    const int64_t kt_begin = (int64_t)zsplit * k_tiles_per_split;
    int64_t kt_end = kt_begin + k_tiles_per_split;
    if (kt_end > kt_total) kt_end = kt_total;
    int64_t kt_full = K / BIG_BK;
    if (kt_full > kt_end) kt_full = kt_end;

    f32x16 acc[4][2];
#pragma unroll
    for (int i = 0; i < 4; ++i)
#pragma unroll
        for (int j = 0; j < 2; ++j)
#pragma unroll
            for (int v = 0; v < 16; ++v) acc[i][j][v] = 0.f;

    BigOperand<LA> ga;
    BigOperand<LB> gb;
    ga.prepare(Ap, lda, M, m0, kt_begin * BIG_BK);
    gb.prepare(Bp, ldb, N, n0, kt_begin * BIG_BK);

    char* const my_piece = smem + wave * 1024;
    auto stage_full = [&](int slot, int q) {
        char* base = my_piece + slot * BIG_TILE_BYTES + q * 8192;
        if (q < 2) ga.stage(q, base); else gb.stage(q - 2, base);
        if (q == 1) ga.advance();
        if (q == 3) gb.advance();
    };
    int64_t kt = kt_begin;
    auto stage_any = [&](int slot, int q) {
        char* base = my_piece + slot * BIG_TILE_BYTES + q * 8192;
        const int64_t k4 = kt + GEMM_BIG_STAGES;
        const bool live = k4 < kt_end;
        if (q < 2) ga.stage_checked(q, base, k4 * BIG_BK, K, live); else gb.stage_checked(q - 2, base, k4 * BIG_BK, K, live);
        if (q == 1) ga.advance();
        if (q == 3) gb.advance();
    };

    struct Frags { u32x4 a[4], b[2]; };
    Frags f0, f1, f2;
    const int bcol = (wc & 1) * 64;
    const int a_off = wr * 8192, b_off = 16384 + (wc >> 1) * 8192;
    auto rd_a = [&](Frags& f, int slot_, int kk, int i) {
        f.a[i] = big_frag<LA>(reinterpret_cast<const unsigned short*>(smem + slot_ * BIG_TILE_BYTES + a_off), 32 * i, kk, lane);
    };
    auto rd_b = [&](Frags& f, int slot_, int kk, int j) {
// ... 131 lines not shown
```

### spatiotemporal_variable_separation_amd/csrc/vs_gemm_core.h

```cpp
#pragma once
#include <stdlib.h>
#include <string.h>
#include "vs_common.h"

namespace {

enum { LR = VS_LAYOUT_R, LS = VS_LAYOUT_S };

template <int CT> struct CTraits;
template <> struct CTraits<VS_F32> { typedef float T; static constexpr int U = 4; static constexpr int KSTEP = 8; };
template <> struct CTraits<VS_BF16> { typedef __bf16 T; static constexpr int U = 8; static constexpr int KSTEP = 16; };
template <> struct CTraits<VS_F16> { typedef _Float16 T; static constexpr int U = 8; static constexpr int KSTEP = 16; };

template <int CT>
__device__ __forceinline__ f32x16 mfma16_32(const u32x4& a, const u32x4& b, const f32x16& c) {
    if constexpr (CT == VS_BF16)
        return __builtin_amdgcn_mfma_f32_32x32x16_bf16(__builtin_bit_cast(bf16x8, a), __builtin_bit_cast(bf16x8, b), c, 0, 0, 0);
    else
        return __builtin_amdgcn_mfma_f32_32x32x16_f16(__builtin_bit_cast(f16x8, a), __builtin_bit_cast(f16x8, b), c, 0, 0, 0);
}

#include "vs_adam_math.h"

struct Epi {
    void* C; int64_t ldc; int c_dtype;
    float alpha; const float* bias; int act;
    const void* mask; int64_t ldmask; int mask_dtype; int mask_act;
    int accumulate;
    int64_t nchw_hw, nchw_c;
    int g_w, g_hw, o_w, sy, sx, oy, ox;
    int splits_per_batch;
    int64_t batch_a, batch_b, batch_c;
    float* adam_m; float* adam_v; unsigned short* adam_shadow; int adam_shadow_dtype;
    const int* adam_step; int adam_skipped;
    const unsigned* adam_guard;
    double adam_lr, adam_beta1, adam_beta2; float adam_eps;
    int xcd_runs;
    unsigned* sk_counters; int sk_splits; int64_t sk_bytes;
    const float* fl_full; const int* fl_tdev; int fl_ae_shift, fl_first, fl_G, fl_T;
    const float* fl_up; float fl_l_ae, fl_l_pred, fl_inv_ae, fl_inv_pred;
    void* fl_dz; int fl_dz_dtype; float* fl_partials;
};

inline Epi plain_epi(void* C, int64_t ldc, int c_dtype, float alpha) {
    Epi e{};
    e.C = C; e.ldc = ldc; e.c_dtype = c_dtype; e.alpha = alpha;
    return e;
}

__device__ __forceinline__ unsigned big_tile_of(unsigned b, unsigned nwg) {
    const unsigned xcd = b & 7u, q = nwg >> 3, r = nwg & 7u;
    return (xcd < r ? xcd * (q + 1) : r * (q + 1) + (xcd - r) * q) + (b >> 3);
}

__device__ __forceinline__ Epi epi_for_batch(const Epi& e, int64_t batch) {
    Epi r = e;
    if (batch) r.C = (char*)e.C + batch * e.batch_c * vs_esize(e.c_dtype);
    return r;
}

typedef __attribute__((address_space(8))) void* sk_rsrc_t;
__device__ __forceinline__ auto sk_rsrc(const float* base, int64_t bytes) {
    return __builtin_amdgcn_make_buffer_rsrc(const_cast<float*>(base), 0, (int)bytes, 0x00020000);
}
template <class R> __device__ __forceinline__ void sk_store(R r, int64_t elem, float v) {
    __builtin_amdgcn_raw_buffer_store_b32(__float_as_uint(v), r, (int)(elem * 4), 0, 16);
}
template <class R> __device__ __forceinline__ void sk_store4(R r, int64_t elem, const f32x4& v) {
    __builtin_amdgcn_raw_buffer_store_b128(__builtin_bit_cast(u32x4, v), r, (int)(elem * 4), 0, 16);
}
template <class R> __device__ __forceinline__ float sk_load(R r, int64_t elem) {
    return __uint_as_float(__builtin_amdgcn_raw_buffer_load_b32(r, (int)(elem * 4), 0, 16));
}
template <class R> __device__ __forceinline__ f32x4 sk_load4(R r, int64_t elem) {
    return __builtin_bit_cast(f32x4, __builtin_amdgcn_raw_buffer_load_b128(r, (int)(elem * 4), 0, 16));
}
__device__ __forceinline__ bool sk_arrive_last(const Epi& e, unsigned tile_id, volatile unsigned* lds_word) {
    asm volatile("s_waitcnt vmcnt(0)" ::: "memory");
    __syncthreads();
    if (threadIdx.x == 0) {
        const unsigned old = atomicAdd(e.sk_counters + tile_id, 1u);
        const unsigned last = old == (unsigned)(e.sk_splits - 1);
        if (last) atomicExch(e.sk_counters + tile_id, 0u);
        *lds_word = last;
    }
    __syncthreads();
    return *lds_word != 0u;
}

__device__ __forceinline__ void epi_store(const Epi& e, int64_t m, int64_t n, float v) {
    v *= e.alpha;
    if (e.bias) v += e.bias[n];
    v = vs_act(v, e.act);
    if (e.mask) v *= vs_act_grad_from_out(vs_ld(e.mask, e.mask_dtype, m * e.ldmask + n), e.mask_act);
    const int64_t idx = m * e.ldc + n;
    if (e.accumulate) v += vs_ld(e.C, e.c_dtype, idx);
    vs_st(e.C, e.c_dtype, idx, v);
}

__device__ __forceinline__ void epi_store_nchw(const Epi& e, int64_t m, int64_t col_base, float v) {
    v *= e.alpha;
    if (e.bias) v += e.bias[m];
    v = vs_act(v, e.act);
    const int64_t idx = col_base + m * e.nchw_hw;
    if (e.mask) v *= vs_act_grad_from_out(vs_ld(e.mask, e.mask_dtype, idx), e.mask_act);
    if (e.accumulate) v += vs_ld(e.C, e.c_dtype, idx);
    vs_st(e.C, e.c_dtype, idx, v);
}

__device__ __forceinline__ int64_t nchw_col_base(const Epi& e, int64_t n) {
    if (e.g_hw == 0) {
        const int64_t b = n / e.nchw_hw;
        return b * e.nchw_c * e.nchw_hw + (n - b * e.nchw_hw);
    }
    const int64_t b = n / e.g_hw;
    const int r = (int)(n - b * e.g_hw);
    const int gy = r / e.g_w, gx = r - gy * e.g_w;
    return b * e.nchw_c * e.nchw_hw + (int64_t)(gy * e.sy + e.oy) * e.o_w + gx * e.sx + e.ox;
}

template <int CT, int LAYOUT>
struct Dense {
    typedef typename CTraits<CT>::T T;
    static constexpr int U = CTraits<CT>::U;
    static constexpr int layout = LAYOUT;
    const T* p; int64_t ld; int64_t rows; int64_t K; int vec_ok;
    __device__ __forceinline__ void shift(int64_t elems) { p += elems; }

    struct State { const T* base; int ok; };
    __device__ __forceinline__ State prepare(int64_t i) const {
        State st;
        if (LAYOUT == LR) { st.ok = i < rows; st.base = p + i * ld; }
        else { st.ok = i < rows ? (i + U <= rows ? 2 : 1) : 0; st.base = p + i; }
        return st;
    }
    __device__ __forceinline__ u32x4 load(const State& st, int64_t i, int64_t k) const {
        u32x4 r = {0u, 0u, 0u, 0u};
        if (!st.ok || k >= K) return r;
        if (LAYOUT == LR) {
            const T* q = st.base + k;
            if (vec_ok && k + U <= K) return *reinterpret_cast<const u32x4*>(q);
            T tmp[U];
#pragma unroll
            for (int j = 0; j < U; ++j) tmp[j] = (k + j < K) ? q[j] : (T)0.f;
            return *reinterpret_cast<u32x4*>(tmp);
        } else {
            const T* q = st.base + k * ld;
            if (vec_ok && st.ok == 2) return *reinterpret_cast<const u32x4*>(q);
            T tmp[U];
#pragma unroll
            for (int j = 0; j < U; ++j) tmp[j] = (i + j < rows) ? q[j] : (T)0.f;
            return *reinterpret_cast<u32x4*>(tmp);
        }
    }
};

template <int CT, int LAYOUT, int ROWS, int BK>
struct TileGeom {
    static constexpr int U = CTraits<CT>::U;
    static constexpr int PITCH = LAYOUT == LR ? BK + U : (CT != VS_F32 ? ROWS + 32 : ROWS + 4);
    static constexpr int ELEMS = LAYOUT == LR ? ROWS * PITCH : BK * PITCH;
    static constexpr int UNITS = ROWS * BK / U;
    static constexpr int PER_THREAD = UNITS / 256;
    static_assert(UNITS % 256 == 0, "tile must split evenly over 256 threads");
    __device__ static __forceinline__ void map(int u, int& di, int& dk, int& lds_off) {
        if (LAYOUT == LR) {
            constexpr int CH = BK / U;
            di = u / CH; dk = (u % CH) * U; lds_off = di * PITCH + dk;
        } else {
            constexpr int CH = ROWS / U;
            dk = u / CH; di = (u % CH) * U; lds_off = dk * PITCH + di;
        }
    }
};

template <int CT, class Op, int ROWS, int BK>
__device__ __forceinline__ void tile_prepare(const Op& op, int64_t i0, typename Op::State (&st)[TileGeom<CT, Op::layout, ROWS, BK>::PER_THREAD]) {
    typedef TileGeom<CT, Op::layout, ROWS, BK> G;
#pragma unroll
    for (int it = 0; it < G::PER_THREAD; ++it) {
        int di, dk, off;
        G::map(threadIdx.x + it * 256, di, dk, off);
        st[it] = op.prepare(i0 + di);
    }
}

template <int CT, class Op, int ROWS, int BK>
__device__ __forceinline__ void tile_fetch(const Op& op, const typename Op::State (&st)[TileGeom<CT, Op::layout, ROWS, BK>::PER_THREAD], int64_t i0,
                                           int64_t k0, u32x4 (&regs)[TileGeom<CT, Op::layout, ROWS, BK>::PER_THREAD]) {
    typedef TileGeom<CT, Op::layout, ROWS, BK> G;
#pragma unroll
    for (int it = 0; it < G::PER_THREAD; ++it) {
        int di, dk, off;
        G::map(threadIdx.x + it * 256, di, dk, off);
        regs[it] = op.load(st[it], i0 + di, k0 + dk);
    }
}

template <int CT, int LAYOUT, int ROWS, int BK>
__device__ __forceinline__ void tile_commit(typename CTraits<CT>::T* lds,
                                            const u32x4 (&regs)[TileGeom<CT, LAYOUT, ROWS, BK>::PER_THREAD]) {
    typedef TileGeom<CT, LAYOUT, ROWS, BK> G;
#pragma unroll
    for (int it = 0; it < G::PER_THREAD; ++it) {
        int di, dk, off;
        G::map(threadIdx.x + it * 256, di, dk, off);
        *reinterpret_cast<u32x4*>(lds + off) = regs[it];
    }
}

typedef __attribute__((ext_vector_type(4))) short vs_i16x4;
__device__ __forceinline__ u32x4 vs_tr16_pair(const unsigned short* a, int second_offset_elems) {
    typedef __attribute__((address_space(3))) vs_i16x4 lds_i16x4;
    const vs_i16x4 lo = __builtin_amdgcn_ds_read_tr16_b64_v4i16((lds_i16x4*)(a));
    const vs_i16x4 hi = __builtin_amdgcn_ds_read_tr16_b64_v4i16((lds_i16x4*)(a + second_offset_elems));
    typedef __attribute__((ext_vector_type(8))) short i16x8;
    const i16x8 both = __builtin_shufflevector(lo, hi, 0, 1, 2, 3, 4, 5, 6, 7);
    return __builtin_bit_cast(u32x4, both);
}

template <int LAYOUT, int PITCH>
__device__ __forceinline__ u32x4 frag_bf16(const unsigned short* tile, int row0, int kk, int lane) {
    if (LAYOUT == LR) {
        const int r = lane & 31, h = lane >> 5;
        return *reinterpret_cast<const u32x4*>(tile + (row0 + r) * PITCH + kk + 8 * h);
    } else {
        const int li = lane & 15, q = li >> 2, p = li & 3, cb = (lane >> 4) & 1, h = lane >> 5;
        const unsigned short* a = tile + (kk + 8 * h + q) * PITCH + row0 + 16 * cb + 4 * p;
        return vs_tr16_pair(a, 4 * PITCH);
    }
}

template <int LAYOUT, int PITCH>
__device__ __forceinline__ f32x4 frag_f32(const float* tile, int row0, int kk, int lane) {
    const int r = lane & 31, q = lane >> 5;
    if (LAYOUT == LR) {
        return *reinterpret_cast<const f32x4*>(tile + (row0 + r) * PITCH + kk + 4 * q);
    } else {
        const float* a = tile + (kk + 4 * q) * PITCH + row0 + r;
        f32x4 v;
        v[0] = a[0]; v[1] = a[PITCH]; v[2] = a[2 * PITCH]; v[3] = a[3 * PITCH];
        return v;
    }
}

template <int CT, class OpA, class OpB, int BM, int BN, int BK, bool NCHW = false>
__global__ __launch_bounds__(256) void gemm_kernel(OpA A, OpB B, int64_t M, int64_t N, int64_t K,
                                                   int k_tiles_per_split, Epi epi_in, float* slabs) {
    unsigned bx = blockIdx.x, by = blockIdx.y, bz = blockIdx.z;
    if (epi_in.xcd_runs) {
        const unsigned gx = gridDim.x, gy = gridDim.y;
        const unsigned t = big_tile_of(bx + gx * (by + gy * bz), gx * gy * gridDim.z);
        bz = t / (gx * gy);
        by = (t - bz * gx * gy) / gx;
        bx = t - (bz * gy + by) * gx;
    }
    int zsplit = bz;
    if (epi_in.splits_per_batch > 0) {
        const int batch = bz / epi_in.splits_per_batch;
        zsplit = bz - batch * epi_in.splits_per_batch;
        A.shift(batch * epi_in.batch_a);
        B.shift(batch * epi_in.batch_b);
    }
    const Epi epi = epi_for_batch(epi_in, epi_in.splits_per_batch > 0 ? bz / epi_in.splits_per_batch : 0);
    typedef typename CTraits<CT>::T T;
    typedef TileGeom<CT, OpA::layout, BM, BK> GA;
    typedef TileGeom<CT, OpB::layout, BN, BK> GB;
    constexpr int WM = BM / 2, WN = BN / 2;
    constexpr int TM = WM / 32, TN = WN / 32;
    static_assert(TM >= 1 && TN >= 1, "tile too small");

    extern __shared__ __attribute__((aligned(16))) char smem[];
    T* sA = reinterpret_cast<T*>(smem);
    T* sB = sA + GA::ELEMS;

    const int lane = threadIdx.x & 63, wave = threadIdx.x >> 6;
    const int wm = (wave >> 1) * WM, wn = (wave & 1) * WN;
    const int64_t m0 = (int64_t)by * BM, n0 = (int64_t)bx * BN;
    const int64_t kt_total = (K + BK - 1) / BK;
    const int64_t kt_begin = (int64_t)zsplit * k_tiles_per_split;
    int64_t kt_end = kt_begin + k_tiles_per_split;
    if (kt_end > kt_total) kt_end = kt_total;

    f32x16 acc[TM][TN];
#pragma unroll
    for (int i = 0; i < TM; ++i)
#pragma unroll
        for (int j = 0; j < TN; ++j)
#pragma unroll
            for (int v = 0; v < 16; ++v) acc[i][j][v] = 0.f;

    u32x4 ra[GA::PER_THREAD], rb[GB::PER_THREAD];
    typename OpA::State sta[GA::PER_THREAD];
    typename OpB::State stb[GB::PER_THREAD];
    tile_prepare<CT, OpA, BM, BK>(A, m0, sta);
    tile_prepare<CT, OpB, BN, BK>(B, n0, stb);
    if (kt_begin < kt_end) {
        tile_fetch<CT, OpA, BM, BK>(A, sta, m0, kt_begin * BK, ra);
        tile_fetch<CT, OpB, BN, BK>(B, stb, n0, kt_begin * BK, rb);
    }
    for (int64_t kt = kt_begin; kt < kt_end; ++kt) {
        tile_commit<CT, OpA::layout, BM, BK>(sA, ra);
        tile_commit<CT, OpB::layout, BN, BK>(sB, rb);
        __syncthreads();
        if (kt + 1 < kt_end) {
            tile_fetch<CT, OpA, BM, BK>(A, sta, m0, (kt + 1) * BK, ra);
            tile_fetch<CT, OpB, BN, BK>(B, stb, n0, (kt + 1) * BK, rb);
        }
        if constexpr (CT != VS_F32) {
#pragma unroll
            for (int kk = 0; kk < BK; kk += 16) {
                u32x4 fa[TM], fb[TN];
#pragma unroll
                for (int i = 0; i < TM; ++i)
                    fa[i] = frag_bf16<OpA::layout, GA::PITCH>(reinterpret_cast<const unsigned short*>(sA), wm + 32 * i, kk, lane);
#pragma unroll
                for (int j = 0; j < TN; ++j)
                    fb[j] = frag_bf16<OpB::layout, GB::PITCH>(reinterpret_cast<const unsigned short*>(sB), wn + 32 * j, kk, lane);
#pragma unroll
                for (int i = 0; i < TM; ++i)
#pragma unroll
                    for (int j = 0; j < TN; ++j) acc[i][j] = mfma16_32<CT>(fa[i], fb[j], acc[i][j]);
            }
        } else {
            f32x16 part[TM][TN];
#pragma unroll
            for (int i = 0; i < TM; ++i)
#pragma unroll
                for (int j = 0; j < TN; ++j)
#pragma unroll
                    for (int v = 0; v < 16; ++v) part[i][j][v] = 0.f;
#pragma unroll
            for (int kk = 0; kk < BK; kk += 8) {
                f32x4 fa[TM], fb[TN];
#pragma unroll
                for (int i = 0; i < TM; ++i)
                    fa[i] = frag_f32<OpA::layout, GA::PITCH>(reinterpret_cast<const float*>(sA), wm + 32 * i, kk, lane);
#pragma unroll
                for (int j = 0; j < TN; ++j)
                    fb[j] = frag_f32<OpB::layout, GB::PITCH>(reinterpret_cast<const float*>(sB), wn + 32 * j, kk, lane);
#pragma unroll
                for (int e = 0; e < 4; ++e)
#pragma unroll
                    for (int i = 0; i < TM; ++i)
#pragma unroll
                        for (int j = 0; j < TN; ++j)
                            part[i][j] = __builtin_amdgcn_mfma_f32_32x32x2f32(fa[i][e], fb[j][e], part[i][j], 0, 0, 0);
            }
#pragma unroll
            for (int i = 0; i < TM; ++i)
#pragma unroll
                for (int j = 0; j < TN; ++j) acc[i][j] += part[i][j];
        }
        __syncthreads();
    }

    const int cj = lane & 31, rh = 4 * (lane >> 5);
#pragma unroll
    for (int i = 0; i < TM; ++i)
#pragma unroll
        for (int j = 0; j < TN; ++j) {
            const int64_t n = n0 + wn + 32 * j + cj;
            if (n >= N) continue;
            int64_t col_base = 0;
            if constexpr (NCHW) col_base = nchw_col_base(epi, n);
#pragma unroll
            for (int v = 0; v < 16; ++v) {
                const int64_t m = m0 + wm + 32 * i + (v & 3) + 8 * (v >> 2) + rh;
                if (m >= M) continue;
                if (slabs) {
                    if (epi_in.sk_counters) sk_store(sk_rsrc(slabs, epi_in.sk_bytes), ((int64_t)bz * M + m) * N + n, acc[i][j][v]);
                    else slabs[((int64_t)bz * M + m) * N + n] = acc[i][j][v];
                }
                else if constexpr (NCHW) epi_store_nchw(epi, m, col_base, acc[i][j][v]);
                else epi_store(epi, m, n, acc[i][j][v]);
            }
        }
    if (slabs && epi_in.sk_counters) {
        const int splits = epi_in.sk_splits;
        const unsigned pb = (unsigned)(bz / (unsigned)splits);
        if (!sk_arrive_last(epi_in, (pb * gridDim.y + by) * gridDim.x + bx, reinterpret_cast<volatile unsigned*>(smem))) return;
        const int64_t total = M * N;
        const auto rs = sk_rsrc(slabs, epi_in.sk_bytes);
        const int64_t first = (int64_t)pb * splits * total;
#pragma unroll
        for (int i = 0; i < TM; ++i)
#pragma unroll
            for (int j = 0; j < TN; ++j) {
                const int64_t n = n0 + wn + 32 * j + cj;
                if (n >= N) continue;
                int64_t col_base = 0;
                if constexpr (NCHW) col_base = nchw_col_base(epi, n);
#pragma unroll 4
                for (int v = 0; v < 16; ++v) {
                    const int64_t m = m0 + wm + 32 * i + (v & 3) + 8 * (v >> 2) + rh;
                    if (m >= M) continue;
                    const int64_t q = first + m * N + n;
                    float sum = 0.f;
#pragma unroll 4
                    for (int s = 0; s < splits; ++s) sum += sk_load(rs, q + (int64_t)s * total);
                    if constexpr (NCHW) epi_store_nchw(epi, m, col_base, sum);
                    else epi_store(epi, m, n, sum);
                }
            }
    }
}

__global__ __launch_bounds__(256) void splitk_reduce_kernel(const float* slabs, int splits, int64_t M, int64_t N, Epi epi_in) {
    const int64_t total = M * N;
    slabs += (int64_t)blockIdx.y * splits * total;
    const Epi epi = epi_for_batch(epi_in, blockIdx.y);
    for (int64_t idx = (int64_t)blockIdx.x * 256 + threadIdx.x; idx < total; idx += (int64_t)gridDim.x * 256) {
        float v = 0.f;
        for (int s = 0; s < splits; ++s) v += slabs[(int64_t)s * total + idx];
        const int64_t m = idx / N, n = idx - m * N;
        if (epi.nchw_hw > 0) epi_store_nchw(epi, m, nchw_col_base(epi, n), v);
        else epi_store(epi, m, n, v);
    }
}

inline int launch_splitk_reduce(const float* slabs, int splits, int64_t M, int64_t N, const Epi& epi, int batch, hipStream_t stream) {
    int64_t blocks = vs_cdiv(M * N, 256);
    if (blocks > 2048) blocks = 2048;
    hipLaunchKernelGGL(splitk_reduce_kernel, dim3((unsigned)blocks, (unsigned)batch), dim3(256), 0, stream, slabs, splits, M, N, epi);
    VS_CHECK_LAUNCH("split-K reduce");
    return VS_OK;
}

template <int CT> constexpr int bk_of() { return CT != VS_F32 ? 64 : 16; }

}
```

### spatiotemporal_variable_separation_amd/csrc/vs_gemm_mid.h

```cpp
#pragma once
#include "vs_gemm_big.h"

namespace {

constexpr int MID_TILE_BYTES = 2 * 8192;

template <int N>
__device__ __forceinline__ void vs_wait_vm() { asm volatile("s_waitcnt vmcnt(%0)" ::"n"(N) : "memory"); }
template <int N>
__device__ __forceinline__ void vs_wait_vm_lgkm0() { asm volatile("s_waitcnt vmcnt(%0) lgkmcnt(0)" ::"n"(N) : "memory"); }

template <int LAYOUT>
struct MidOperand {
    const char* base;
    uint32_t voff[2];
    int kofs[2];
    int64_t step;

    __device__ __forceinline__ void prepare(const unsigned short* p, int64_t ld, int64_t rows, int64_t i0, int64_t k_begin) {
#pragma unroll
        for (int q = 0; q < 2; ++q) {
            const int u = (int)threadIdx.x + 256 * q;
            if (LAYOUT == LR) {
                const int row = u >> 2, piece = (u & 3) ^ ((row >> 2) & 3);
// ... 28 lines not shown
        run_tiles = (int)(HW / BIG_BK);
        t_in_run = (int)(r / BIG_BK);
        run_jump = (C * HW - HW) * 2;
    }
    __device__ __forceinline__ void advance() {
        base += step;
        if (run_tiles && ++t_in_run == run_tiles) { t_in_run = 0; base += run_jump; }
    }
    __device__ __forceinline__ void stage(int q, char* lds) const {
        const uint32_t dst = (uint32_t)(uintptr_t)lds;
        asm volatile("s_mov_b32 m0, %0\n\ts_nop 0\n\tglobal_load_lds_dwordx4 %1, %2" ::"s"(dst), "v"(voff[q]), "s"(base) : "memory", "m0");
    }
    __device__ __forceinline__ void stage_checked(int q, char* lds, int64_t k0, int64_t K, bool live) const {
        const void* g = (live && k0 + kofs[q] < K) ? (const void*)(base + voff[q]) : (const void*)vs_glds_zero;
        const uint32_t dst = (uint32_t)(uintptr_t)lds;
        asm volatile("s_mov_b32 m0, %0\n\ts_nop 0\n\tglobal_load_lds_dwordx4 %1, off" ::"s"(dst), "v"(g) : "memory", "m0");
    }
};

template <int CT, int LA, int LB, bool NCHW, int ST, bool ADAM>
__global__ __launch_bounds__(256) void gemm_mid_kernel(const unsigned short* Ap, int64_t lda, const unsigned short* Bp, int64_t ldb, int64_t M, int64_t N,
                                                          int64_t K, int k_tiles_per_split, int tiles_n, Epi epi_in, float* slabs, int64_t a_chan_hw) {
    unsigned tile, bz = blockIdx.z;
    if (epi_in.xcd_runs) {
        const unsigned t = big_tile_of(blockIdx.x + gridDim.x * blockIdx.z, gridDim.x * gridDim.z);
        bz = t / gridDim.x;
        tile = t - bz * gridDim.x;
    } else {
        tile = big_tile_of(blockIdx.x, gridDim.x);
    }
    int zsplit = bz;
    int batch = 0;
    if (epi_in.splits_per_batch > 0) {
        batch = bz / epi_in.splits_per_batch;
        zsplit = bz - batch * epi_in.splits_per_batch;
        Ap += batch * epi_in.batch_a;
        Bp += batch * epi_in.batch_b;
    }
    const Epi epi = epi_for_batch(epi_in, batch);
    extern __shared__ __attribute__((aligned(16))) char smem[];

    const int lane = threadIdx.x & 63;
    const int wave = __builtin_amdgcn_readfirstlane((int)(threadIdx.x >> 6));
    const int wr = wave >> 1, wc = wave & 1;
    const int64_t m0 = (int64_t)(tile / (unsigned)tiles_n) * 128, n0 = (int64_t)(tile % (unsigned)tiles_n) * 128;
    const int64_t kt_total = (K + BIG_BK - 1) / BIG_BK;
    const int64_t kt_begin = (int64_t)zsplit * k_tiles_per_split;
    int64_t kt_end = kt_begin + k_tiles_per_split;
    if (kt_end > kt_total) kt_end = kt_total;
    int64_t kt_full = K / BIG_BK;
    if (kt_full > kt_end) kt_full = kt_end;

    f32x16 acc[2][2];
#pragma unroll
    for (int i = 0; i < 2; ++i)
#pragma unroll
        for (int j = 0; j < 2; ++j)
#pragma unroll
            for (int v = 0; v < 16; ++v) acc[i][j][v] = 0.f;

    MidOperand<LA> ga;
    MidOperand<LB> gb;
    if (LA == LR && a_chan_hw > 0) ga.prepare_runs(Ap, M, a_chan_hw, m0, kt_begin * BIG_BK);
    else ga.prepare(Ap, lda, M, m0, kt_begin * BIG_BK);
    gb.prepare(Bp, ldb, N, n0, kt_begin * BIG_BK);

    char* const my_piece = smem + wave * 1024;
    auto dst_of = [&](int slot, int q) { return my_piece + slot * MID_TILE_BYTES + (q >> 1) * 8192 + (q & 1) * 4096; };
    auto stage_full = [&](int slot, int q) {
        if (q < 2) ga.stage(q, dst_of(slot, q)); else gb.stage(q - 2, dst_of(slot, q));
        if (q == 1) ga.advance();
        if (q == 3) gb.advance();
    };
    int64_t kt = kt_begin;
    auto stage_any = [&](int slot, int q) {
        const int64_t k4 = kt + ST;
        const bool live = k4 < kt_end;
        if (q < 2) ga.stage_checked(q, dst_of(slot, q), k4 * BIG_BK, K, live); else gb.stage_checked(q - 2, dst_of(slot, q), k4 * BIG_BK, K, live);
        if (q == 1) ga.advance();
        if (q == 3) gb.advance();
    };

    struct Frags { u32x4 a[2], b[2]; };
    Frags f0, f1, f2;
    auto rd_a = [&](Frags& f, int slot_, int kk, int i) {
        f.a[i] = big_frag<LA>(reinterpret_cast<const unsigned short*>(smem + slot_ * MID_TILE_BYTES), wr * 64 + 32 * i, kk, lane);
    };
    auto rd_b = [&](Frags& f, int slot_, int kk, int j) {
        f.b[j] = big_frag<LB>(reinterpret_cast<const unsigned short*>(smem + slot_ * MID_TILE_BYTES + 8192), wc * 64 + 32 * j, kk, lane);
    };
    auto mf = [&](const Frags& f, int i, int j) { acc[i][j] = mfma16_32<CT>(f.a[i], f.b[j], acc[i][j]); };

    kt = kt_begin - ST;
    for (int s4 = 0; s4 < ST; ++s4) {
        for (int q = 0; q < 4; ++q) stage_any(s4, q);
        ++kt;
    }
    vs_wait_vm<4 * (ST - 1)>();
    __builtin_amdgcn_s_barrier();
    for (int i = 0; i < 2; ++i) { rd_a(f0, 0, 0, i); rd_a(f1, 0, 16, i); }
    for (int j = 0; j < 2; ++j) { rd_b(f0, 0, 0, j); rd_b(f1, 0, 16, j); }
    int slot = 0;
#define VS_MID_BODY(X, Y, Z, STAGE)                                                                   \
    {                                                                                                 \
        mf(X, 0, 0); VS_FENCE;                                                                        \
        vs_wait_vm_lgkm0<4 * (ST - 2)>();             \
        __builtin_amdgcn_s_barrier();                                                                 \
        VS_FENCE;                                                                                     \
        const int nslot = slot + 1 == ST ? 0 : slot + 1;                                              \
        STAGE(slot, 0); rd_a(Z, nslot, 0, 0); VS_FENCE;                                               \
        mf(X, 0, 1); VS_FENCE; rd_a(Z, nslot, 0, 1); VS_FENCE;                                        \
        mf(X, 1, 0); VS_FENCE; STAGE(slot, 1); rd_b(Z, nslot, 0, 0); VS_FENCE;                        \
        mf(X, 1, 1); VS_FENCE; rd_b(Z, nslot, 0, 1); VS_FENCE;                                        \
        mf(Y, 0, 0); VS_FENCE; STAGE(slot, 2); rd_a(X, nslot, 16, 0); VS_FENCE;                       \
        mf(Y, 0, 1); VS_FENCE; rd_a(X, nslot, 16, 1); VS_FENCE;                                       \
        mf(Y, 1, 0); VS_FENCE; STAGE(slot, 3); rd_b(X, nslot, 16, 0); VS_FENCE;                       \
        mf(Y, 1, 1); VS_FENCE; rd_b(X, nslot, 16, 1); VS_FENCE;                                       \
        slot = nslot;                                                                                 \
        ++kt;                                                                                         \
    }
    {
        int64_t n3 = (kt_full - ST - kt_begin) / 3;
        for (; n3 > 0; --n3) {
            VS_MID_BODY(f0, f1, f2, stage_full)
            VS_MID_BODY(f2, f0, f1, stage_full)
            VS_MID_BODY(f1, f2, f0, stage_full)
        }
    }
    while (kt < kt_end) {
        VS_MID_BODY(f0, f1, f2, stage_any)
        if (kt >= kt_end) break;
        VS_MID_BODY(f2, f0, f1, stage_any)
        if (kt >= kt_end) break;
        VS_MID_BODY(f1, f2, f0, stage_any)
    }
#undef VS_MID_BODY
    asm volatile("s_waitcnt vmcnt(0) lgkmcnt(0)" ::: "memory");
    __builtin_amdgcn_s_barrier();

    float* stg = reinterpret_cast<float*>(smem) + wave * (64 * 64);
    const int cj = lane & 31, rh = 4 * (lane >> 5);
    float* slab_base = slabs ? slabs + (int64_t)bz * M * N : nullptr;
#pragma unroll
    for (int ii = 0; ii < 2; ++ii)
#pragma unroll
        for (int j = 0; j < 2; ++j)
#pragma unroll
            for (int v = 0; v < 16; ++v)
                stg[(32 * ii + (v & 3) + 8 * (v >> 2) + rh) * 64 + 32 * j + cj] = acc[ii][j][v];
    asm volatile("s_waitcnt lgkmcnt(0)" ::: "memory");
    const int64_t nn = n0 + wc * 64 + (lane & 15) * 4;
    if constexpr (ADAM) {
        if (epi.adam_guard && *epi.adam_guard != 0u) return;
        const AdamCoef coef = vs_adam_coef(epi.adam_lr, epi.adam_beta1, epi.adam_beta2, epi.adam_eps, (double)(epi.adam_step[0] + 1 - epi.adam_skipped));
        if (m0 + 128 <= M && nn + 3 < N && ((epi.ldc | nn) & 3) == 0 &&
            (((uintptr_t)epi.C | (uintptr_t)epi.adam_m | (uintptr_t)epi.adam_v) & 15) == 0 && (!epi.adam_shadow || ((uintptr_t)epi.adam_shadow & 7) == 0)) {
            constexpr int G = 4;
            f32x4 p[2][G], mm[2][G], vv[2][G];
            const int64_t idx0 = (m0 + wr * 64 + (lane >> 4)) * epi.ldc + nn;
            const int64_t rstep = 4 * epi.ldc;
            const float* __restrict__ Pp = (const float*)epi.C + idx0;
            const float* __restrict__ Mp = epi.adam_m + idx0;
            const float* __restrict__ Vp = epi.adam_v + idx0;
            const int sdt = epi.adam_shadow_dtype;
            auto ld4 = [&](const float* q) { return *reinterpret_cast<const f32x4*>(q); };
            auto st4 = [&](float* q, const f32x4& v) { *reinterpret_cast<f32x4*>(q) = v; };
#pragma unroll
            for (int t = 0; t < G; ++t) {
                p[0][t] = ld4(Pp + t * rstep);
                mm[0][t] = ld4(Mp + t * rstep);
                vv[0][t] = ld4(Vp + t * rstep);
            }
#pragma unroll
            for (int g = 0; g < 16 / G; ++g) {
                if (g + 1 < 16 / G) {
#pragma unroll
                    for (int t = 0; t < G; ++t) {
                        const int64_t o = ((g + 1) * G + t) * rstep;
                        p[(g + 1) & 1][t] = ld4(Pp + o);
                        mm[(g + 1) & 1][t] = ld4(Mp + o);
                        vv[(g + 1) & 1][t] = ld4(Vp + o);
                    }
                }
#pragma unroll
                for (int t = 0; t < G; ++t) {
                    const int r = (g * G + t) * 4 + (lane >> 4);
                    const f32x4 g4 = *reinterpret_cast<const f32x4*>(stg + r * 64 + (lane & 15) * 4);
                    f32x4 pe = p[g & 1][t], me = mm[g & 1][t], ve = vv[g & 1][t];
#pragma unroll
                    for (int e = 0; e < 4; ++e) {
                        float a = pe[e], b = me[e], c = ve[e];
                        vs_adam_elem(coef, g4[e] * epi.alpha, a, b, c);
                        pe[e] = a; me[e] = b; ve[e] = c;
                    }
                    const int64_t idx = idx0 + (g * G + t) * rstep;
                    st4((float*)epi.C + idx, pe);
                    st4(epi.adam_m + idx, me);
                    st4(epi.adam_v + idx, ve);
                    if (epi.adam_shadow) {
                        const u16x4 h = {vs_f2h(pe[0], sdt), vs_f2h(pe[1], sdt), vs_f2h(pe[2], sdt), vs_f2h(pe[3], sdt)};
                        *reinterpret_cast<u16x4*>(epi.adam_shadow + idx) = h;
                    }
                }
            }
            return;
        }
        for (int it = 0; it < 16; ++it) {
            const int r = it * 4 + (lane >> 4);
            const int64_t m = m0 + wr * 64 + r;
            const f32x4 v4 = *reinterpret_cast<const f32x4*>(stg + r * 64 + (lane & 15) * 4);
            if (m < M && nn < N) big_adam4(epi, coef, m, nn, N, v4);
        }
        return;
    }
    for (int it = 0; it < 16; ++it) {
        const int r = it * 4 + (lane >> 4);
        const int64_t m = m0 + wr * 64 + r;
        const f32x4 v4 = *reinterpret_cast<const f32x4*>(stg + r * 64 + (lane & 15) * 4);
        if (m < M && nn < N) big_store4<NCHW>(epi, m, nn, N, v4, slab_base ? slab_base + m * N : nullptr, epi_in.sk_counters ? slabs : nullptr, epi_in.sk_bytes);
    }
    if (slab_base && epi_in.sk_counters) {
        const int splits = epi_in.sk_splits;
        if (!sk_arrive_last(epi_in, (unsigned)batch * gridDim.x + tile, reinterpret_cast<volatile unsigned*>(smem))) return;
        const int64_t total = M * N;
        const auto rs = sk_rsrc(slabs, epi_in.sk_bytes);
        const int64_t first = (int64_t)batch * splits * total;
        const bool vec = nn + 3 < N && (((uintptr_t)slabs | (uintptr_t)(total * 4)) & 15) == 0 && (N & 3) == 0;
        for (int it = 0; it < 16; ++it) {
            const int64_t m = m0 + wr * 64 + it * 4 + (lane >> 4);
            if (m >= M || nn >= N) continue;
            const int64_t q = first + m * N + nn;
            f32x4 sum = {0.f, 0.f, 0.f, 0.f};
            if (vec) {
#pragma unroll 8
                for (int s = 0; s < splits; ++s) sum += sk_load4(rs, q + (int64_t)s * total);
            } else {
                for (int s = 0; s < splits; ++s)
                    for (int t = 0; t < 4; ++t)
                        if (nn + t < N) sum[t] += sk_load(rs, q + (int64_t)s * total + t);
            }
            big_store4<NCHW>(epi, m, nn, N, sum, nullptr);
        }
    }
}

template <int CT, int LA, int LB, bool NCHW = false>
int mid_launch(const void* A, int64_t lda, const void* B, int64_t ldb, int64_t M, int64_t N, int64_t K, int splits, int64_t k_tiles_per_split,
               int stages, int batch, const Epi& epi, float* slabs, hipStream_t stream, int64_t a_chan_hw = 0) {
    if constexpr (CT == VS_F32) {
        return vs_fail(VS_ERR_UNSUPPORTED, "the 128x128 LDS-DMA ring tile is a 16-bit kernel");
    } else {
        const int tiles_m = (int)vs_cdiv(M, 128), tiles_n = (int)vs_cdiv(N, 128);
        dim3 grid((unsigned)(tiles_m * tiles_n), 1, (unsigned)(splits * batch));
        Epi e_runs = epi;
        e_runs.xcd_runs = grid.z > 1;
        const Epi& epi_l = e_runs;
        auto go = [&](auto kfn, int st_, bool& attr_set) -> int {
            const int lds = st_ * MID_TILE_BYTES;
            if (!attr_set) {
                if (hipFuncSetAttribute((const void*)kfn, hipFuncAttributeMaxDynamicSharedMemorySize, lds) != hipSuccess)
                    return vs_fail(VS_ERR_LAUNCH, "cannot raise the dynamic LDS limit to %d bytes", lds);
                attr_set = true;
            }
            hipLaunchKernelGGL(kfn, grid, dim3(256), lds, stream, (const unsigned short*)A, lda, (const unsigned short*)B, ldb, M, N, K,
                               (int)k_tiles_per_split, tiles_n, epi_l, slabs, a_chan_hw);
            return VS_OK;
        };
        static bool set5 = false, set10 = false, set_adam = false;
        if constexpr (NCHW) {
            return stages == 10 ? go(gemm_mid_kernel<CT, LA, LB, true, 10, false>, 10, set10) : go(gemm_mid_kernel<CT, LA, LB, true, 5, false>, 5, set5);
        } else {
            return epi.adam_m ? go(gemm_mid_kernel<CT, LA, LB, false, 5, true>, 5, set_adam)
                   : stages == 10 ? go(gemm_mid_kernel<CT, LA, LB, false, 10, false>, 10, set10)
                                  : go(gemm_mid_kernel<CT, LA, LB, false, 5, false>, 5, set5);
        }
    }
}

}
```

### spatiotemporal_variable_separation_amd/ops.py

```python
import collections
import os

import torch

from . import _lib
from ._lib import F32, BF16, F16, ACT, LAYOUT_R, LAYOUT_S, check, code_of, dtype_code, stream_ptr, require_cuda

_DT = {F32: 'f32', BF16: 'bf16', F16: 'fp16'}

_ws_cache = {}
_retired = []

_PROF = {'on': False, 'events': []}
_LNAME = {0: 'R', 1: 'S'}


def profile_reset(enable=True, pool=0):
    _PROF['on'] = enable
    _PROF['events'] = []
    _PROF['pool'] = []
    if enable and pool:
        for _ in range(pool):
            e = torch.cuda.Event(enable_timing=True)
            e.record()
            _PROF['pool'].append(e)
        torch.cuda.synchronize()


def _new_event():
    pool = _PROF.get('pool')
    e = pool.pop() if pool else torch.cuda.Event(enable_timing=True)
    e.record()
    return e


def _pb():
    if not _PROF['on']:
        return None
    return _new_event()


def _pe(e0, name, flops=0.0, nbytes=0.0):
    if e0 is None:
        return
    _PROF['events'].append((name, e0, _new_event(), flops, nbytes))


def profile_collect():
    torch.cuda.synchronize()
    out = {}
    for name, e0, e1, fl, by in _PROF['events']:
        r = out.setdefault(name, {'ms': 0.0, 'n': 0, 'flops': 0.0, 'bytes': 0.0})
        r['ms'] += e0.elapsed_time(e1)
        r['n'] += 1
        r['flops'] += fl
        r['bytes'] += by
    _PROF['on'] = False
    _PROF['events'] = []
    return out


def _workspace(nbytes, device):
    key = (device.index, torch.cuda.current_stream(device).cuda_stream)
    buf = _ws_cache.get(key)
    if buf is None or buf.numel() < nbytes:
        if buf is not None:
            _retired.append(buf)
        buf = torch.empty(max(nbytes, 2 * buf.numel() if buf is not None else 1 << 20), dtype=torch.uint8, device=device)
        _ws_cache[key] = buf
    return buf


def _ptr(t):
    return 0 if t is None else t.data_ptr()


def gemm(a, layout_a, b, layout_b, M, N, K, out=None, out_dtype=torch.float32, alpha=1.0, bias=None, act='none',
         mask=None, mask_act='none', accumulate=False, lda=None, ldb=None):
    require_cuda(a, b, out, bias, mask)
    lib = _lib.load_library()
    if a.dtype != b.dtype:
        raise _lib.VarsepHipError('gemm operands must share a dtype (%s vs %s)' % (a.dtype, b.dtype))
    assert a.stride(-1) == 1 and b.stride(-1) == 1
    compute = dtype_code(a)
    lda = a.stride(0) if lda is None else lda
    ldb = b.stride(0) if ldb is None else ldb
    if out is None:
        out = torch.empty((M, N), dtype=out_dtype, device=a.device)
    assert out.stride(-1) == 1
    ws_bytes = lib.vs_gemm_workspace_bytes(M, N, K)
    ws = _workspace(ws_bytes, a.device) if ws_bytes else None
    if bias is not None:
        assert bias.dtype == torch.float32 and bias.is_contiguous()
    e0 = _pb()
    check(lib.vs_gemm(compute, M, N, K, a.data_ptr(), lda, layout_a, b.data_ptr(), ldb, layout_b, out.data_ptr(),
                      out.stride(0), dtype_code(out), float(alpha), _ptr(bias), ACT[act], _ptr(mask),
                      mask.stride(0) if mask is not None else 0, dtype_code(mask) if mask is not None else 0,
                      ACT[mask_act], int(bool(accumulate)), _ptr(ws), ws.numel() if ws is not None else 0, stream_ptr()),
          'vs_gemm')
    _pe(e0, 'vs_gemm<%s,%s%s>' % (_DT[compute], _LNAME[layout_a], _LNAME[layout_b]),
        flops=2.0 * M * N * K, nbytes=float((M * K + N * K) * a.element_size() + M * N * out.element_size()))
    return out


def gemm_adam(a, layout_a, b, layout_b, M, N, K, param, exp_avg, exp_avg_sq, shadow, step_dev, skipped, lr, betas, eps, alpha=1.0):
    require_cuda(a, b, param, exp_avg, exp_avg_sq, step_dev)
    lib = _lib.load_library()
    assert a.dtype == b.dtype and a.dtype in (torch.bfloat16, torch.float16) and a.stride(-1) == 1 and b.stride(-1) == 1
    assert param.dtype == torch.float32 and param.is_contiguous() and tuple(param.shape) == (M, N)
    assert exp_avg.is_contiguous() and exp_avg_sq.is_contiguous() and exp_avg.shape == param.shape == exp_avg_sq.shape
    assert shadow is None or (shadow.is_contiguous() and shadow.shape == param.shape and shadow.dtype in (torch.bfloat16, torch.float16))
    e0 = _pb()
    check(lib.vs_gemm_adam(dtype_code(a), M, N, K, a.data_ptr(), a.stride(0), layout_a, b.data_ptr(), b.stride(0), layout_b, float(alpha),
                           param.data_ptr(), exp_avg.data_ptr(), exp_avg_sq.data_ptr(), _ptr(shadow),
                           code_of(shadow.dtype) if shadow is not None else BF16, step_dev.data_ptr(), int(skipped), float(lr),
                           float(betas[0]), float(betas[1]), float(eps), stream_ptr()), 'vs_gemm_adam')
    _pe(e0, 'vs_gemm_adam<%s,%s%s>' % (_DT[dtype_code(a)], _LNAME[layout_a], _LNAME[layout_b]), flops=2.0 * M * N * K,
        nbytes=float((M * K + N * K) * a.element_size() + M * N * (24 + (2 if shadow is not None else 0))))


def gemm_batched(a, layout_a, b, layout_b, M, N, K, out_dtype=torch.float32, out=None):
    require_cuda(a, b)
    lib = _lib.load_library()
    if a.dtype != b.dtype:
        raise _lib.VarsepHipError('gemm operands must share a dtype (%s vs %s)' % (a.dtype, b.dtype))
    assert a.dim() == 3 and b.dim() == 3 and a.is_contiguous() and b.is_contiguous() and a.shape[0] == b.shape[0]
    batch = a.shape[0]
    compute = dtype_code(a)
    if out is None:
        out = torch.empty((batch, M, N), dtype=out_dtype, device=a.device)
    assert out.is_contiguous() and tuple(out.shape) == (batch, M, N)
    ws_bytes = lib.vs_gemm_batched_workspace_bytes(batch, M, N, K)
    ws = _workspace(ws_bytes, a.device) if ws_bytes else None
    e0 = _pb()
    check(lib.vs_gemm_batched(compute, batch, M, N, K, a.data_ptr(), a.stride(1), a.stride(0), layout_a, b.data_ptr(), b.stride(1),
                              b.stride(0), layout_b, out.data_ptr(), N, M * N, dtype_code(out), 1.0, 0, _ptr(ws),
                              ws.numel() if ws is not None else 0, stream_ptr()), 'vs_gemm_batched')
    _pe(e0, 'vs_gemm<%s,%s%s>' % (_DT[compute], _LNAME[layout_a], _LNAME[layout_b]),
        flops=2.0 * batch * M * N * K, nbytes=float(batch * ((M * K + N * K) * a.element_size() + M * N * out.element_size())))
    return out


def cast(src, dtype, out=None):
    require_cuda(src)
    src = src.contiguous()
    if out is None:
        out = torch.empty(src.shape, dtype=dtype, device=src.device)
    check(_lib.load_library().vs_cast(src.data_ptr(), dtype_code(src), out.data_ptr(), dtype_code(out), src.numel(),
                                      stream_ptr()), 'vs_cast')
    return out


def copy2d(src, rows, cols, lds, out, ldd, col_offset_dev=None, col_offset_scale=0, src_elem_offset=0):
    require_cuda(src, out)
    esz = src.element_size()
    check(_lib.load_library().vs_copy2d(src.data_ptr() + src_elem_offset * esz, dtype_code(src), lds, out.data_ptr(),
                                        dtype_code(out), ldd, rows, cols, _ptr(col_offset_dev), col_offset_scale,
                                        stream_ptr()), 'vs_copy2d')
    return out


def copy2d_pair(src, rows, cols, lds, out, ldd, col_offset_dev, col_offset_scale, elem_offset_a, elem_offset_b):
    require_cuda(src, out)
    check(_lib.load_library().vs_copy2d_pair(src.data_ptr(), dtype_code(src), lds, out.data_ptr(), dtype_code(out), ldd, rows, cols,
                                             _ptr(col_offset_dev), col_offset_scale, elem_offset_a, elem_offset_b, stream_ptr()), 'vs_copy2d_pair')
    return out


def colsum(x, M, N, out=None, accumulate=False):
    require_cuda(x)
    if out is None:
        out = torch.empty((N,), dtype=torch.float32, device=x.device)
    check(_lib.load_library().vs_colsum(x.data_ptr(), dtype_code(x), x.stride(0), M, N, out.data_ptr(),
                                        int(bool(accumulate)), stream_ptr()), 'vs_colsum')
    return out


def colsum_alloc(jobs, flat=None):
    if flat is None:
        flat = torch.empty((sum(x.shape[1] for x in jobs),), dtype=torch.float32, device=jobs[0].device)
    views, off = [], 0
    for x in jobs:
        views.append(flat[off:off + x.shape[1]])
        off += x.shape[1]
    return flat, views


def colsum_multi(jobs, outs=None, zero_flat=None):
    import ctypes
    results = []
    for i in range(0, len(jobs), 12):
        chunk = jobs[i:i + 12]
        n = len(chunk)
        require_cuda(*chunk)
        total = sum(x.shape[1] for x in chunk)
        if outs is None:
            flat = torch.empty((total,), dtype=torch.float32, device=chunk[0].device)
            views, off = [], 0
            for x in chunk:
                views.append(flat[off:off + x.shape[1]])
                off += x.shape[1]
            zero_base, zero_count = flat.data_ptr(), total
        else:
            views = outs[i:i + 12]
            for v, x in zip(views, chunk):
                assert v.dtype == torch.float32 and v.is_contiguous() and v.numel() == x.shape[1]
            require_cuda(*views)
            zero_base, zero_count = None, 0
            if zero_flat is not None:
                zero_base, zero_count = views[0].data_ptr(), sum(v.numel() for v in views)
        VP, I32, I64 = ctypes.c_void_p * n, ctypes.c_int * n, ctypes.c_int64 * n
        e0 = _pb()
        check(_lib.load_library().vs_colsum_multi(
            n, VP(*[x.data_ptr() for x in chunk]), I32(*[dtype_code(x) for x in chunk]), I64(*[x.stride(0) for x in chunk]),
            I64(*[x.shape[0] for x in chunk]), I64(*[x.shape[1] for x in chunk]), VP(*[v.data_ptr() for v in views]),
            zero_base, zero_count, stream_ptr()), 'vs_colsum_multi')
        _pe(e0, 'vs_colsum_multi', nbytes=float(sum(x.numel() * x.element_size() for x in chunk)))
        results += list(views)
    return results


def act_fwd(x, act, out=None, out_dtype=None):
    require_cuda(x)
    x = x.contiguous()
    if out is None:
        out = torch.empty(x.shape, dtype=out_dtype or x.dtype, device=x.device)
    check(_lib.load_library().vs_act_fwd(x.data_ptr(), dtype_code(x), out.data_ptr(), dtype_code(out), ACT[act],
                                         x.numel(), stream_ptr()), 'vs_act_fwd')
    return out


def act_bwd(dy, y, act, out_dtype=None):
    require_cuda(dy, y)
    dy, y = dy.contiguous(), y.contiguous()
    out = torch.empty(dy.shape, dtype=out_dtype or dy.dtype, device=dy.device)
    check(_lib.load_library().vs_act_bwd(dy.data_ptr(), dtype_code(dy), y.data_ptr(), dtype_code(y), out.data_ptr(),
                                         dtype_code(out), ACT[act], dy.numel(), stream_ptr()), 'vs_act_bwd')
    return out


def transpose_cast(src, dtype, out=None):
    require_cuda(src)
    assert src.dim() == 2 and src.is_contiguous()
    rows, cols = src.shape
    if out is None:
        out = torch.empty((cols, rows), dtype=dtype, device=src.device)
    check(_lib.load_library().vs_transpose_cast(src.data_ptr(), dtype_code(src), out.data_ptr(), dtype_code(out), rows,
                                                cols, stream_ptr()), 'vs_transpose_cast')
    return out


_roll_ws = {}


def _rollout_workspace(nbytes, device, geometry):
    if not nbytes:
        return None
    key = (device.index,) + tuple(geometry)
    buf = _roll_ws.get(key)
    if buf is None or buf.numel() != nbytes:
        buf = torch.zeros(nbytes, dtype=torch.uint8, device=device)
        _roll_ws[key] = buf
    return buf


_GUARD = {}


def exchange_guard(device):
# ... 2112 lines not shown
```

### spatiotemporal_variable_separation_amd/optim.py

```python
import ctypes

import torch

from . import _lib
from ._lib import VarsepHipError


class Adam(torch.optim.Optimizer):
    def __init__(self, params, lr=1e-3, betas=(0.9, 0.999), eps=1e-8, weight_decay=0, amsgrad=False, capturable=True, fused=None):
        if weight_decay != 0 or amsgrad:
            raise ValueError('the MI355X Adam implements what the reference uses: weight_decay=0, amsgrad=False')
        if not 0.0 < lr or not 0.0 < eps or not 0.0 <= betas[0] < 1.0 or not 0.0 <= betas[1] < 1.0:
            raise ValueError('invalid Adam hyper-parameters')
        super().__init__(params, dict(lr=lr, betas=betas, eps=eps))
        self._tables = {}
        self._buckets, self._bucket_of, self._left, self._launched, self._stream = [], {}, [], set(), None
        self._fused, self._fused_done = [], set()

    def overlap_with_backward(self, buckets):
        assert len(self.param_groups) == 1, 'overlap_with_backward: one param group'
        self._buckets = [[p for p in b if p.requires_grad] for b in buckets]
        self._buckets = [b for b in self._buckets if b]
        self._bucket_of = {id(p): i for i, b in enumerate(self._buckets) for p in b}
        self._left = [len(b) for b in self._buckets]
        self._launched = set()
        for b in self._buckets:
            for p in b:
                p.register_post_accumulate_grad_hook(self._on_grad)

    def fuse_into_wgrad(self, params):
        from . import functional as VF
        assert len(self.param_groups) == 1, 'fuse_into_wgrad: one param group'
        owned = {id(p) for p in self.param_groups[0]['params']}
        self._fused = [p for p in params if id(p) in owned and p.dim() == 2 and p.requires_grad]
        self._fused_done = set()
        VF.set_fused_optimizer({p: self for p in self._fused})

    def unfuse(self):
        from . import functional as VF
        self._fused, self._fused_done = [], set()
        VF.set_fused_optimizer(None)

    def can_fuse(self, p, a, b):
        return (getattr(self, '_scale_state', None) is None and p.is_contiguous() and p.dtype == torch.float32 and a.dtype == b.dtype
                and a.dtype in (torch.bfloat16, torch.float16) and a.data_ptr() % 16 == 0 and b.data_ptr() % 16 == 0
                and a.stride(0) % 8 == 0 and b.stride(0) % 8 == 0 and p.shape[0] % 8 == 0 and p.shape[1] % 8 == 0)

    @torch.no_grad()
    def fused_update(self, p, a, layout_a, b, layout_b, M, N, K):
        from . import functional as VF, ops
        group = self.param_groups[0]
        self._init_group(0, group)
        st = self.state[p]
        shadow = VF.shadow_buffer_for_update(p)
        ops.gemm_adam(a, layout_a, b, layout_b, M, N, K, p, st['exp_avg'], st['exp_avg_sq'], shadow, group['step_dev'], st.get('skipped', 0),
                      group['lr'], group['betas'], group['eps'])
        torch.autograd.graph.increment_version(p)
        if shadow is not None:
            VF.shadows_written([p])
        self._fused_done.add(id(p))

    def _on_grad(self, p):
        bi = self._bucket_of.get(id(p))
        if bi is None or bi in self._launched:
            return
        self._left[bi] -= 1
        if self._left[bi] > 0:
            return
        group = self.param_groups[0]
        self._init_group(0, group)
        from . import functional as VF
        if VF.defer_call(lambda: self._update(0, group, self._buckets[bi], max_blocks=512)):
            self._launched.add(bi)
            return
        main = torch.cuda.current_stream(p.device)
        if self._stream is None:
            self._stream = VF.own_stream(p.device)
        self._stream.wait_stream(main)
        for s in VF.side_streams_in_use():
            self._stream.wait_stream(s)
        with torch.cuda.stream(self._stream):
            self._update(0, group, self._buckets[bi])
        self._launched.add(bi)

    def _init_group(self, gi, group):
        for p in group['params']:
            st = self.state[p]
            if len(st) == 0:
                if not p.is_cuda or p.dtype != torch.float32 or not p.is_contiguous():
                    raise VarsepHipError('HIP Adam needs contiguous fp32 CUDA parameters (no CPU fallback)')
                st['step'] = torch.zeros((), dtype=torch.float32, device=p.device)
                st['exp_avg'] = torch.zeros_like(p, memory_format=torch.preserve_format)
                st['exp_avg_sq'] = torch.zeros_like(p, memory_format=torch.preserve_format)
        if 'step_dev' not in group:
            ps = group['params']
            steps = [int(self.state[p]['step'].item()) for p in ps]
            start = max(steps) if steps else 0
            for p, t in zip(ps, steps):
                self.state[p]['skipped'] = start - t
            group['step_dev'] = torch.full((1,), start, dtype=torch.int32, device=ps[0].device)

    def _table(self, gi, plist, shadows):
        from . import functional as VF
        key = (gi, id(plist[0]), len(plist))
        gsrc = [VF.lowp_gradient(p) for p in plist]
        gsrc = [p.grad if g is None else g for p, g in zip(plist, gsrc)]
        ptrs = tuple((p.data_ptr(), g.data_ptr(), 0 if s is None else s.data_ptr(), self.state[p].get('skipped', 0))
                     for p, g, s in zip(plist, gsrc, shadows))
        ent = self._tables.get(key)
        if ent is not None and ent[0] == ptrs:
            return ent[1]
        n = len(plist)
        VP, I64, I32 = ctypes.c_void_p * n, ctypes.c_int64 * n, ctypes.c_int32 * n
        tab = (VP(*[p.data_ptr() for p in plist]), VP(*[g.data_ptr() for g in gsrc]),
               VP(*[self.state[p]['exp_avg'].data_ptr() for p in plist]), VP(*[self.state[p]['exp_avg_sq'].data_ptr() for p in plist]),
               VP(*[None if s is None else s.data_ptr() for s in shadows]), I64(*[p.numel() for p in plist]),
               I32(*[self.state[p].get('skipped', 0) for p in plist]),
               I32(*[_lib.BF16 if g.dtype == torch.bfloat16 else _lib.F32 for g in gsrc]))
        self._tables[key] = (ptrs, tab)
        return tab

    @torch.no_grad()
    def step(self, closure=None, grad_scale_state=None, defer_increment=False):
        self._scale_state = grad_scale_state
        self._defer_increment = bool(defer_increment) and grad_scale_state is None
        try:
            return self._step(closure)
        finally:
            self._scale_state = None
            self._defer_increment = False

    def _step(self, closure=None):
        loss = None
        if closure is not None:
            with torch.enable_grad():
                loss = closure()
        lib = _lib.load_library()
        for gi, group in enumerate(self.param_groups):
            self._init_group(gi, group)
            done = set()
            if gi == 0 and self._launched:
                for bi in self._launched:
                    done.update(id(p) for p in self._buckets[bi])
            fused_done = getattr(self, '_fused_done', set())
            done |= fused_done
            live = [p for p in group['params'] if p.grad is not None and id(p) not in done]
            for p in group['params']:
                if p.grad is None and id(p) not in fused_done:
                    self.state[p]['skipped'] = self.state[p].get('skipped', 0) + 1
            if live:
                self._update(gi, group, live)
            main = torch.cuda.current_stream(group['params'][0].device)
            if gi == 0 and self._launched and self._stream is not None:
                main.wait_stream(self._stream)
            if getattr(self, '_scale_state', None) is not None:
                _lib.check(lib.vs_adam_step_increment_scaled(group['step_dev'].data_ptr(), self._scale_state.data_ptr(), main.cuda_stream),
                           'vs_adam_step_increment_scaled')
            elif not getattr(self, '_defer_increment', False):
                _lib.check(lib.vs_adam_step_increment(group['step_dev'].data_ptr(), main.cuda_stream), 'vs_adam_step_increment')
        if self._buckets:
            self._left = [len(b) for b in self._buckets]
            self._launched = set()
        if getattr(self, '_fused_done', None):
            self._fused_done = set()
        return loss

    @torch.no_grad()
    def step_subset(self, params):
        for gi, group in enumerate(self.param_groups):
            self._init_group(gi, group)
            ids = {id(p) for p in group['params']}
            live = [p for p in params if id(p) in ids]
            if any(p.grad is None for p in live):
                raise VarsepHipError('step_subset needs a gradient for every listed parameter')
            if live:
                self._update(gi, group, live)

    @torch.no_grad()
    def step_ranges(self, ranges):
        from . import functional as VF
        lib = _lib.load_library()
        if not ranges:
            return
        group = self.param_groups[0]
        self._init_group(0, group)
        stream = torch.cuda.current_stream(ranges[0][0].device).cuda_stream
        lr, (b1, b2), eps = group['lr'], group['betas'], group['eps']
        written = []
        for i in range(0, len(ranges), 64):
            chunk = ranges[i:i + 64]
            n = len(chunk)
            P, G, M_, V, S, NUM, SK, GD = [], [], [], [], [], [], [], []
            sdt = _lib.BF16
            for p, lo, hi in chunk:
                g = VF.lowp_gradient(p)
                if g is None:
                    g = p.grad
                if g is None or not (0 <= lo < hi <= p.numel()):
                    raise VarsepHipError('step_ranges: a range needs a gradient and 0 <= lo < hi <= numel')
                st = self.state[p]
                sh = VF.shadow_buffer_for_update(p)
                P.append(p.data_ptr() + 4 * lo); M_.append(st['exp_avg'].data_ptr() + 4 * lo); V.append(st['exp_avg_sq'].data_ptr() + 4 * lo)
                G.append(g.data_ptr() + g.element_size() * lo)
                GD.append(_lib.BF16 if g.dtype == torch.bfloat16 else _lib.F32)
                S.append(None if sh is None else sh.data_ptr() + 2 * lo)
                if sh is not None:
                    sdt = _lib.code_of(sh.dtype)
                    written.append(p)
                NUM.append(hi - lo); SK.append(st.get('skipped', 0))
# ... 80 lines not shown
```

### spatiotemporal_variable_separation_amd/profiling.py

```python
import hashlib
import os
import re

_PKG = os.path.dirname(os.path.abspath(__file__))


def source_sha():
    h = hashlib.sha256()
    files = sorted(os.path.join(_PKG, 'csrc', f) for f in os.listdir(os.path.join(_PKG, 'csrc')) if f.endswith(('.hip', '.h')))
    for root, dirs, names in sorted(os.walk(_PKG)):
        dirs[:] = sorted(d for d in dirs if d not in ('__pycache__', 'build', 'csrc'))
        files += [os.path.join(root, f) for f in sorted(names) if f.endswith('.py')]
    for f in files:
        h.update(os.path.relpath(f, _PKG).encode())
        h.update(open(f, 'rb').read())
    return h.hexdigest()[:16]


GROUPS = [
    ('vs_gemm_adam', r'^vs_gemm_adam<', r'gemm_mid_kernel<\d, \d, \d, \w+, \d+, true>', 'hbm'),
    ('vs_mlp_rollout_fwd', r'^vs_mlp_rollout_fwd<', r'rollout_(ws|fwd)_kernel<\d+, true|rollout_fwd_kernel', 'mfma'),
    ('vs_mlp_rollout_bwd', r'^vs_mlp_rollout_bwd<', r'rollout_ws_kernel<\d+, false|rollout_bwd_kernel', 'mfma'),
    ('vs_conv_k4s2', r'^vs_conv_k4s2:|^vs_space_to_depth2', r'conv3_band_kernel<\d, \d+, \d+, \d, 1>|conv3_band2_kernel<\d, \d+, \d, 1, \d+>|wgrad3_band_kernel<\d, \d+, \d, 1(, \d)?>|wgrad2_band_kernel<\d, \d+, 1>|space_to_depth2_kernel|'
     r'::k4s2_\w+_kernel', 'mfma'),
    ('vs_conv3_img16_bn', r'^vs_conv3_img16_bn:', r'conv3_img16_bn_kernel|exchange_epoch_advance', 'mfma'),
    ('vs_conv3_img16', r'^vs_conv3_img16:', r'conv3_img16_kernel|(?<!grouped_)slab_sum_kernel', 'mfma'),
    ('vs_conv3_band', r'^vs_conv3_band:', r'conv3_band2?_kernel', 'mfma'),
    ('vs_conv3_wgrad_band', r'^vs_conv3_wgrad_band<', r'wgrad3_band_kernel|wgrad2_band_kernel|wgrad_slab_finish_kernel|slab_sum_grouped_kernel', 'mfma'),
    ('vs_convT_tap', r'^vs_convT_tap:', r'convt_k4s2_tap_kernel', 'mfma'),
    ('vs_conv3_tap', r'^vs_conv3_tap:', r'conv_k3s1_tap_kernel', 'mfma'),
    ('vs_gemm+cols', r'^vs_gemm<|^vs_conv_cols:|^vs_convT_cols:', r'gemm_kernel<|gemm_glds_kernel<|gemm_big_kernel<|gemm_p8_kernel<|gemm_mid_kernel<\d, \d, \d, \w+, \d+, false>|'
     r'splitk_reduce_kernel|im2col_|convt_k4s2_small_kernel|gather_small_s1_kernel|gather_rowdot_kernel', 'mfma'),
    ('vs_bn_small', r'^vs_bn_fwd_small|^vs_bn_bwd_small', r'bn_fwd_small|bn_bwd_small', 'hbm'),
    ('vs_conv_thin', r'^vs_conv_thin:', r'thin_\w+_kernel', 'hbm'),
    ('vs_bn', r'^vs_bn_stats|^vs_bn_act_fwd|^vs_bn_act_bwd|^vs_chan_sum|^vs_bn_fwd_slab',
     r'bn_stats_kernel|bn_act_fwd_kernel|bn_bwd_reduce|bn_bwd_apply|bn_running|bn_from_sums|chan_sum|group_sum2_kernel|bn_fwd_slab|bn_bwd_slab|bn_from_parts', 'hbm'),
    ('vs_resample+join', r'^vs_upsample|^vs_maxpool|^vs_cat_bcast|^vs_act_', r'upsample_\w+_kernel|maxpool_\w+_kernel|cat_bcast_\w+_kernel|act_fwd_kernel|act_bwd_kernel|'
     r'space_to_depth2', 'hbm'),
    ('vs_operand_upkeep', r'^vs_pack|^vs_zero|^vs_cast|^vs_copy2d', r'tap_pack_kernel|pack_weight_kernel|pack_multi_kernel|conv3_img16_pack|vs_zero_kernel|cast_kernel|'
     r'copy2d_\w*kernel|step_increment_kernel', 'hbm'),
    ('vs_adam_multi', r'^vs_adam_multi', r'adam_multi_kernel', 'hbm'),
    ('vs_train_losses', r'^vs_train_losses|^vs_frames_sse', r'train_losses_\w+_kernel|frames_sse|code_losses_\w+_kernel|frame_loss_finish_kernel', 'hbm'),
    ('vs_colsum_multi', r'^vs_colsum_multi', r'colsum_multi(_rows)?_kernel', 'hbm'),
    ('vs_mix_codes', r'^vs_mix_codes', r'mix_codes_\w+_kernel', 'hbm'),
    ('at::native (torch elementwise / cat / reduce)', r'^$', r'^void at::native|^at::native|__amd_rocclr', 'hbm'),
]
_COMPILED = [(g, re.compile(f), re.compile(k), b) for g, f, k, b in GROUPS]


def group_of_family(label):
    for g, f, _, _ in _COMPILED:
        if f.search(label):
            return g
    return None


def group_of_kernel(symbol):
    for g, _, k, _ in _COMPILED:
        if k.search(symbol):
            return g
    return None


def bound_of(group):
    for g, _, _, b in _COMPILED:
        if g == group:
            return b
    return 'hbm'


def replay_table(stats_rows, step_kernel='step_increment'):
    def name(r):
        return r.get('Name') or r.get('KernelName')

    def calls(r):
        return int(r.get('Calls') or r.get('Count'))

    def total(r):
        return float(r.get('TotalDurationNs') or r.get('TotalDuration(ns)') or r['TotalDuration'])
    steps = max([calls(r) for r in stats_rows if step_kernel in name(r)] or [1])
    out, rest = {}, 0.0
    for r in stats_rows:
        g = group_of_kernel(name(r))
        if g is None:
            rest += total(r)
            continue
        e = out.setdefault(g, {'ns': 0.0, 'calls': 0})
        e['ns'] += total(r)
        e['calls'] += calls(r)
    table = {g: {'us_per_step': e['ns'] / steps / 1e3, 'launches_per_step': e['calls'] / steps, 'avg_launch_us': e['ns'] / e['calls'] / 1e3}
             for g, e in out.items()}
    return steps, table, rest / steps / 1e3


def hip_graph_counts(raw_graph, dot_path=None):
    import ctypes
    hip = ctypes.CDLL('libamdhip64.so')
    g = ctypes.c_void_p(int(raw_graph))
    n = ctypes.c_size_t(0)
    if hip.hipGraphGetNodes(g, None, ctypes.byref(n)) != 0:
        return None
    nodes = (ctypes.c_void_p * max(n.value, 1))()
    hip.hipGraphGetNodes(g, nodes, ctypes.byref(n))
    kernels = 0
    for i in range(n.value):
        t = ctypes.c_int(-1)
        hip.hipGraphNodeGetType(ctypes.c_void_p(nodes[i]), ctypes.byref(t))
        kernels += int(t.value == 0)
    e = ctypes.c_size_t(0)
    hip.hipGraphGetEdges(g, None, None, ctypes.byref(e))
    r = ctypes.c_size_t(0)
    hip.hipGraphGetRootNodes(g, None, ctypes.byref(r))
    if dot_path:
        hip.hipGraphDebugDotPrint(g, dot_path.encode(), ctypes.c_uint(0))
    return {'nodes': int(n.value), 'kernel_nodes': kernels, 'edges': int(e.value), 'roots': int(r.value)}
```

### spatiotemporal_variable_separation_amd/train.py

```python
import os

import numpy as np
import torch
import torch.nn.functional as F

from .utils.helper import save


def zero_order_loss(s_code_old, s_code_new, skipco):
    if skipco:
        s_code_old = torch.cat([s_code_old[0].flatten().float()] + [x.flatten().float() for x in s_code_old[1]])
        s_code_new = torch.cat([s_code_new[0].flatten().float()] + [x.flatten().float() for x in s_code_new[1]])
    return (s_code_old - s_code_new).pow(2).mean()


def ae_loss(cond, target, sep_net, nt_cond, offset, skipco, t_random=None):
    full_data = torch.cat([cond, target], dim=1)
    data_new = full_data[:, -nt_cond:]
    data_old = full_data[:, :nt_cond]
    s_code_old = sep_net.Es(data_old, return_skip=skipco)
    s_code_new = sep_net.Es(data_new, return_skip=skipco)
    if t_random is None:
        if offset == 0:
            t_random = np.random.randint(nt_cond, full_data.size(1))
# ... 364 lines not shown
            VF.collect_cuts(False)
            VF.promise_loss_gradient(None)
            VF.enable_side_streams(False)
            VF.set_grad_outputs(None)
            if self._conv_sinks:
                VF.set_conv_grad_outputs(None)
                VF.fold_repeated_gradients(fold_was, flush=False)
        return total.detach()

    def step(self, cond=None, target=None):
        if cond is not None:
            self.cond.copy_(cond, non_blocking=True)
            self.target.copy_(target, non_blocking=True)
        if [g['lr'] for g in self.opt.param_groups] != self._lrs:
            self._capture()
        self._draw()
        self.graph.replay()
        self.steps_replayed += 1
        if self.sync is not None:
            was_presummed, self.sync.presummed = self.sync.presummed, getattr(self, 'presum', False)
        try:
            return self._finish_step()
        finally:
            if self.sync is not None:
                self.sync.presummed = was_presummed

    def _finish_step(self):
        early = {}
        if getattr(self, 'graph2', None) is not None:
            early = {bi: self.sync.reduce_bucket(bi) for bi in self.sync.early_buckets}
            self.graph2.replay()
        if isinstance(self.graph_opt, list):
            events = [early[bi] if bi in early else self.sync.reduce_bucket(bi) for bi in range(len(self.sync.buckets))]
            main = torch.cuda.current_stream()
            for bi, (ev, g) in enumerate(zip(events, self.graph_opt)):
                if ev is not None:
                    main.wait_event(ev)
                g.replay()
                if self.sharded:
                    self.sync.gather_operand_copies(bi)
            self.graph_opt[-1].replay()
            if self.sharded:
                self.sync.wait_comm()
                self.sync.masters_dirty = True
        elif self.graph_opt is not None:
            for bi in range(len(self.sync.buckets)):
                if bi not in early:
                    self.sync.reduce_bucket(bi)
            if self.sync._comm_stream is not None:
                torch.cuda.current_stream().wait_stream(self.sync._comm_stream)
            self.graph_opt.replay()
        from . import functional as VF
        VF.note_replay()
        return self.loss


def backward_decoder_segment(total, up, sep_net):
    from . import functional as VF
    pairs = VF.cut_pairs()
    assert pairs, 'two-segment backward: no tensor was cut at the decoder\'s inputs'
    heads = [p for p in sep_net.decoder.parameters() if p.requires_grad]
    torch.autograd.backward(total, up, inputs=heads + [leaf for _, leaf in pairs], retain_graph=True)
    return pairs


def backward_rest_segment(total, up, sep_net, pairs):
    dec = {id(p) for p in sep_net.decoder.parameters()}
    rest = [p for p in sep_net.parameters() if p.requires_grad and id(p) not in dec]
    live = [(o, leaf) for o, leaf in pairs if leaf.grad is not None]
    torch.autograd.backward([total] + [o for o, _ in live], [up] + [leaf.grad for _, leaf in live], inputs=rest)
    for _, leaf in pairs:
        leaf.grad = None


def local_conv_gradient_sinks(sep_net):
    import torch.nn as nn
    from . import functional as VF
    from .networks.conv import ConvResBlock
    for blk in sep_net.modules():
        if isinstance(blk, ConvResBlock):
            VF.mark_repeated([m.weight for m in blk.modules() if isinstance(m, nn.Conv2d)])
            blk._marked = True
    params = VF.conv_parameters(sep_net)
    offs, n = [], 0
    for prm in params:
        offs.append(n)
        n += (prm.numel() + 3) // 4 * 4
    flat = torch.zeros((n,), dtype=torch.float32, device=params[0].device)
    return flat, {prm: flat[o:o + prm.numel()].view(prm.shape) for prm, o in zip(params, offs)}


def conv_gradient_sinks(sep_net, grad_sync):
    import torch.nn as nn
    from . import functional as VF
    owned = {id(p) for p in grad_sync.params}
    from .networks.conv import ConvResBlock
    for blk in sep_net.modules():
        if isinstance(blk, ConvResBlock):
            VF.mark_repeated([m.weight for m in blk.modules() if isinstance(m, nn.Conv2d)])
            blk._marked = True
    late = [m.weight for m in sep_net.modules() if isinstance(m, nn.Conv2d) and tuple(m.stride) == (1, 1) and id(m.weight) in owned
            and getattr(m.weight, '_vs_repeated', False)]
    if late and hasattr(grad_sync, 'hold_params'):
        grad_sync.hold_params(late)
    return {p: p.grad for p in VF.conv_parameters(sep_net) if id(p) in owned and p.grad is not None}


def chain_weight_parameters(sep_net):
    out = []
    if not _mlp_family(sep_net):
        return out
    for mod in (sep_net.Es, sep_net.Et, sep_net.decoder):
        mlp = getattr(mod, 'mlp', None)
        if mlp is not None:
            out += [lin.weight for lin in mlp.linears()]
    return out


def rollout_weight_stacks(sep_net):
    if not _mlp_family(sep_net):
        return []
    per_block = [[lin.weight for lin in blk.mlp.linears()] for blk in sep_net.t_resnet.blocks]
    if not per_block or any(len(ws) != 3 for ws in per_block):
        return []
    return [[ws[l] for ws in per_block] for l in range(3)]


def shard_optimizer_default():
    return os.environ.get('VARSEP_SHARD_OPT', '1') == '1'


def enable_update_in_backward(optimizer, sep_net, grad_sync=None, force=False, scaler=None):
    from .optim import Adam as HipAdam
    if not force:
        return
    if scaler is not None:
        return
    if isinstance(optimizer, HipAdam) and grad_sync is None and not optimizer._buckets and len(optimizer.param_groups) == 1:
        owned = {id(p) for p in optimizer.param_groups[0]['params']}
        fused = {id(p) for p in getattr(optimizer, '_fused', [])}
        early = [p for m in (sep_net.decoder, sep_net.Es) for p in m.parameters() if id(p) in owned and id(p) not in fused]
        buckets = [early, [p for p in sep_net.t_resnet.parameters() if id(p) in owned and id(p) not in fused],
                   [p for p in sep_net.Et.parameters() if id(p) in owned and id(p) not in fused]]
        if sum(len(b) for b in buckets) + len(fused) == len(owned):
            optimizer.overlap_with_backward(buckets)


def enable_fused_update(optimizer, sep_net, grad_sync=None, scaler=None, min_numel=1 << 22):
    from .optim import Adam as HipAdam
    if os.environ.get('VARSEP_FUSE_ADAM', '1') != '1' or not isinstance(optimizer, HipAdam):
        return False
    if grad_sync is not None or scaler is not None or not _mlp_family(sep_net) or len(optimizer.param_groups) != 1 or optimizer._buckets:
        return False
    big = [p for p in chain_weight_parameters(sep_net) if p.numel() >= min_numel]
    if not big:
        return False
    optimizer.fuse_into_wgrad(big)
    return True


def check_optimizer(optimizer, for_graph=False):
    if getattr(optimizer, 'defaults', {}).get('fused'):
        raise ValueError('torch optimizers with fused=True do not invalidate the bf16 operand copies / weight pre-packs of the HIP '
                         'path; use spatiotemporal_variable_separation_amd.optim.Adam (one HIP launch) or a non-fused optimizer')
    if for_graph:
        from .optim import Adam as HipAdam
        if not isinstance(optimizer, HipAdam) and not getattr(optimizer, 'defaults', {}).get('capturable'):
            raise ValueError('a recorded training step (hipGraph) needs spatiotemporal_variable_separation_amd.optim.Adam or a torch '
                             'optimizer constructed with capturable=True')


class _TrainState:

    def __init__(self, sep_net, optimizer, scaler=None):
        self.tensors = [t for t in list(sep_net.parameters()) + list(sep_net.buffers())]
        for group in optimizer.param_groups:
            if isinstance(group.get('step_dev'), torch.Tensor):
                self.tensors.append(group['step_dev'])
        for st in optimizer.state.values():
            self.tensors += [v for v in st.values() if isinstance(v, torch.Tensor)]
        if scaler is not None:
            self.tensors.append(scaler.state)
        self.fresh_opt = optimizer if not optimizer.state else None
        self.values = [t.detach().clone() for t in self.tensors]
        self.np_state = np.random.get_state()
        self.skipped = {id(p): st.get('skipped') for p, st in optimizer.state.items() if isinstance(st, dict) and 'skipped' in st}
        self.opt = optimizer

    def restore(self):
        with torch.no_grad():
            for t, v in zip(self.tensors, self.values):
                t.copy_(v)
            if self.fresh_opt is not None:
                for st in self.fresh_opt.state.values():
                    for v in st.values():
                        if isinstance(v, torch.Tensor):
                            v.zero_()
                    if 'skipped' in st:
                        st['skipped'] = 0
                for group in self.fresh_opt.param_groups:
                    if isinstance(group.get('step_dev'), torch.Tensor):
                        group['step_dev'].zero_()
            else:
                for p, st in self.opt.state.items():
                    if id(p) in self.skipped:
                        st['skipped'] = self.skipped[id(p)]
        np.random.set_state(self.np_state)


class LossScaler:

    def __init__(self, device, init_scale=65536.0, growth_factor=2.0, backoff_factor=0.5, growth_interval=2000):
        self.state = torch.tensor([init_scale, 0.0, 0.0, 0.0], dtype=torch.float32, device=device)
        self.growth_factor, self.backoff_factor, self.growth_interval = growth_factor, backoff_factor, growth_interval
        self.init_scale = init_scale

    def scale_tensor(self):
        return self.state[0]

    def get_scale(self):
        return float(self.state[0].item())

    def skipped_steps(self):
        return int(self.state[3].item())

    def backward(self, loss):
        loss.backward(self.state[0])

    def step(self, optimizer):
        from . import functional as VF, ops
        from .optim import Adam as HipAdam
        if not isinstance(optimizer, HipAdam):
            raise ValueError('fp16 loss scaling is implemented by spatiotemporal_variable_separation_amd.optim.Adam (device-side skip)')
        if optimizer._buckets or optimizer._fused:
            raise ValueError('fp16 loss scaling cannot be combined with Adam updates issued during backward (overlap_with_backward / '
                             'fuse_into_wgrad): they would apply still-scaled gradients and could not be skipped on overflow')
        grads = []
        for group in optimizer.param_groups:
            for p in group['params']:
                g = VF.lowp_gradient(p)
                g = p.grad if g is None else g
                if g is not None:
                    grads.append(g)
        ops.check_finite_multi(grads, self.state)
        optimizer.step(grad_scale_state=self.state)
        ops.loss_scale_update(self.state, self.growth_factor, self.backoff_factor, self.growth_interval)

    def describe(self):
        return ('dynamic loss scaling (GradScaler semantics on the device: init %g, x%g after %d clean steps, x%g on overflow); '
                'scale now %g, %d step(s) skipped' % (self.init_scale, self.growth_factor, self.growth_interval, self.backoff_factor,
                                                      self.get_scale(), self.skipped_steps()))


def make_loss_scaler(device, **kw):
    return LossScaler(device, **kw)


def check_rollout_exchange(device):
    from . import ops
    from ._lib import VarsepHipError
    err = ops.rollout_exchange_error(device)
    if err:
        raise VarsepHipError('rollout kernel: inter-workgroup exchange timed out (code %d) -- the integrator results of at least one '
                             'step since the last check are invalid; not continuing.  (With 8 / 16 row slabs the exchange relies on the '
                             'workgroups of a slab sharing an XCD; VS_ROLLOUT_XCD_LOCAL=0 selects the placement-independent agent-scope exchange.)' % err)


def recover_exchange(device, log=True, grad_sync=None):
    import sys
    from . import ops
    from ._lib import VarsepHipError
    guarded = ops.exchange_guard(torch.device(device)) is not None
    skipped = ops.exchange_skipped_steps(device) if guarded else 0
    err = ops.rollout_exchange_error(device)
    if grad_sync is not None and grad_sync.world_size > 1:
        import torch.distributed as dist
        word = torch.tensor([err], dtype=torch.int32, device=device if grad_sync.backend == 'nccl' else 'cpu')
        dist.all_reduce(word, op=dist.ReduceOp.BOR, group=grad_sync.group)
        err = int(word.item())
    if not err:
        return 0
    if not guarded:
        raise VarsepHipError('rollout kernel: inter-workgroup exchange timed out (code %d) and no guard word protects the optimizer on this '
                             'device: the results of at least one step are invalid' % err)
    if err & 1:
        ops.rollout_xcd_local(False)
    if err & 2:
        from . import functional as VF
        VF.resblock_two_launch_only(True)
    if log:
        sys.stderr.write('varsep: an in-launch exchange timed out (code %d); the optimizer skipped %s (batches consumed, no update; the first of them '
                         'may have updated the weights whose Adam step runs inside their weight-gradient GEMM).  Continuing with %s\n'
                         % (err, ('%d step(s)' % skipped) if skipped else 'the affected step(s)', ' and '.join((['the agent-scope integrator exchange'] if err & 1 else []) +
                                              (['two-launch ConvResBlock layers'] if err & 2 else []))))
    return err


def compute_losses(cond, target, sep_net, nt_cond, nt_pred, offset, skipco, lamb_ae, lamb_s, lamb_t, lamb_pred,
                   average_tloss=False, t_random=None):
    assert offset == nt_cond or offset == 0
    if cond.is_cuda and _mlp_family(sep_net):
        return _compute_losses_mlp_batched(cond, target, sep_net, nt_cond, nt_pred, offset, lamb_ae, lamb_s, lamb_t,
                                           lamb_pred, average_tloss, t_random)
    if cond.is_cuda and torch.is_grad_enabled():
        from . import ops
        ops.exchange_epoch_advance(cond.device)
    if cond.is_cuda and torch.is_grad_enabled():
        from . import functional as VF
        VF.prepack_conv3_weights(sep_net)
    full_data = torch.cat([cond, target], dim=1)
# ... 213 lines not shown
```

Baseline: 1.932 million frames/s.

## Fuse Adam update into wgrad GEMM epilogue for small encoder weights

Extends the fused GEMM-plus-Adam path to smaller encoder weight matrices. It does this by adding an optimizer epilogue to the register-tile GEMM kernel and a split-K reduce kernel that applies Adam directly. The goal is to avoid writing the weight gradient to memory and then reading it back in a separate multi-tensor Adam launch. The trade-off is extra planning calls per step, workspace use for split-K, and the Adam epilogue's cost inside GEMM kernels that may have fewer tiles.

```diff
diff --git a/include/varsep_hip.h b/include/varsep_hip.h
--- a/include/varsep_hip.h
+++ b/include/varsep_hip.h
@@ -259,6 +259,10 @@
 int vs_gemm_adam(int compute, int64_t M, int64_t N, int64_t K, const void* A, int64_t lda, int layout_a, const void* B, int64_t ldb,
                  int layout_b, float alpha, float* param, float* exp_avg, float* exp_avg_sq, void* shadow, int shadow_dtype,
                  const int32_t* step, int32_t skipped, double lr, double beta1, double beta2, double eps, void* stream);
+int vs_gemm_adam_planned(int compute, int64_t M, int64_t N, int64_t K, const void* A, int64_t lda, int layout_a, const void* B, int64_t ldb,
+                         int layout_b, float alpha, float* param, float* exp_avg, float* exp_avg_sq, void* shadow, int shadow_dtype,
+                         const int32_t* step, int32_t skipped, double lr, double beta1, double beta2, double eps, void* workspace,
+                         size_t workspace_bytes, void* stream);
 int vs_loss_scale_update(float* scale_state, float growth_factor, float backoff_factor, int growth_interval, void* stream);
 
 int vs_frames_sse_fwd(const float* frames, const float* full, const int32_t* idx, int64_t B, int G, int T, int64_t D, float* sums,
diff --git a/spatiotemporal_variable_separation_amd/_lib.py b/spatiotemporal_variable_separation_amd/_lib.py
--- a/spatiotemporal_variable_separation_amd/_lib.py
+++ b/spatiotemporal_variable_separation_amd/_lib.py
@@ -108,6 +108,8 @@
     'vs_adam_set_max_blocks': (_i32, [_i32]),
     'vs_gemm_adam': (_i32, [_i32, _i64, _i64, _i64, _vp, _i64, _i32, _vp, _i64, _i32, ctypes.c_float, _vp, _vp, _vp, _vp, _i32, _vp, _i32,
                      ctypes.c_double, ctypes.c_double, ctypes.c_double, ctypes.c_double, _vp]),
+    'vs_gemm_adam_planned': (_i32, [_i32, _i64, _i64, _i64, _vp, _i64, _i32, _vp, _i64, _i32, ctypes.c_float, _vp, _vp, _vp, _vp, _i32, _vp, _i32,
+                             ctypes.c_double, ctypes.c_double, ctypes.c_double, ctypes.c_double, _vp, _sz, _vp]),
     'vs_adam_multi_scaled': (_i32, [_i32, _vp, _vp, _vp, _vp, _vp, _vp, _i32, _vp, _vp, _vp, ctypes.c_double, ctypes.c_double, ctypes.c_double,
                                     ctypes.c_double, _vp, _vp]),
     'vs_adam_step_increment_scaled': (_i32, [_vp, _vp, _vp]),
diff --git a/spatiotemporal_variable_separation_amd/csrc/vs_gemm.hip b/spatiotemporal_variable_separation_amd/csrc/vs_gemm.hip
--- a/spatiotemporal_variable_separation_amd/csrc/vs_gemm.hip
+++ b/spatiotemporal_variable_separation_amd/csrc/vs_gemm.hip
@@ -38,6 +38,16 @@
     dim3 grid((unsigned)vs_cdiv(c.N, BN), (unsigned)vs_cdiv(c.M, BM), (unsigned)(plan.splits * c.batch));
     Epi e = epi;
     e.xcd_runs = (int64_t)grid.x * grid.y * grid.z >= 64;
+    if (epi.adam_m && !slabs) {
+        if constexpr (CT == VS_F32 || LA != LS || LB != LS) {
+            return vs_fail(VS_ERR_UNSUPPORTED, "vs_gemm_adam_planned: the register tile's optimizer epilogue serves 16-bit S x S operands");
+        } else {
+            hipLaunchKernelGGL((gemm_kernel<CT, Dense<CT, LA>, Dense<CT, LB>, BM, BN, BK, false, true>), grid, dim3(256), smem, c.stream, a, b, c.M,
+                               c.N, c.K, (int)plan.k_tiles_per_split, e, slabs);
+            VS_CHECK_LAUNCH("vs_gemm_adam_planned");
+            return VS_OK;
+        }
+    }
     hipLaunchKernelGGL((gemm_kernel<CT, Dense<CT, LA>, Dense<CT, LB>, BM, BN, BK>), grid, dim3(256), smem, c.stream, a, b, c.M, c.N,
                        c.K, (int)plan.k_tiles_per_split, e, slabs);
     VS_CHECK_LAUNCH("vs_gemm");
@@ -233,6 +243,36 @@
     return launch_plan(compute, call, mp, epi, nullptr);
 }
 
+extern "C" int vs_gemm_adam_planned(int compute, int64_t M, int64_t N, int64_t K, const void* A, int64_t lda, int layout_a, const void* B,
+                                    int64_t ldb, int layout_b, float alpha, float* param, float* exp_avg, float* exp_avg_sq, void* shadow,
+                                    int shadow_dtype, const int32_t* step, int32_t skipped, double lr, double beta1, double beta2, double eps,
+                                    void* workspace, size_t workspace_bytes, void* stream_) {
+    VS_CHECK_ARG(compute == VS_BF16 || compute == VS_F16, "vs_gemm_adam_planned: 16-bit compute types only (%d)", compute);
+    VS_CHECK_ARG(M > 0 && N > 0 && K > 0, "vs_gemm_adam_planned: M, N, K must be positive");
+    VS_CHECK_ARG(A && B && param && exp_avg && exp_avg_sq && step, "vs_gemm_adam_planned: null pointer");
+    VS_CHECK_ARG((layout_a == LR || layout_a == LS) && (layout_b == LR || layout_b == LS), "vs_gemm_adam_planned: bad layout");
+    VS_CHECK_ARG(lda >= (layout_a == LR ? K : M) && ldb >= (layout_b == LR ? K : N), "vs_gemm_adam_planned: leading dimension too small");
+    VS_CHECK_ARG(!shadow || shadow_dtype == VS_BF16 || shadow_dtype == VS_F16, "vs_gemm_adam_planned: bad shadow dtype");
+    VS_CHECK_ARG(((uintptr_t)param | (uintptr_t)exp_avg | (uintptr_t)exp_avg_sq) % 4 == 0 && (uintptr_t)shadow % 2 == 0,
+                 "vs_gemm_adam_planned: misaligned parameter block");
+    Epi epi = plain_epi(param, N, VS_F32, alpha);
+    epi.adam_m = exp_avg; epi.adam_v = exp_avg_sq; epi.adam_shadow = (unsigned short*)shadow; epi.adam_shadow_dtype = shadow_dtype;
+    epi.adam_step = step; epi.adam_skipped = skipped; epi.adam_guard = vs_g_exchange_guard;
+    epi.adam_lr = lr; epi.adam_beta1 = beta1; epi.adam_beta2 = beta2; epi.adam_eps = (float)eps;
+    const GemmPlan plan = plan_gemm(compute, M, N, K, 1, A, lda, layout_a, 0, B, ldb, layout_b, 0);
+    if (plan.splits == 1 && (plan.kind != GEMM_REG || layout_a != LS || layout_b != LS))
+        return vs_fail(VS_ERR_UNSUPPORTED, "vs_gemm_adam_planned: the unsplit plan of these operands has no optimizer epilogue (register tile, S x S only)");
+    if ((int64_t)plan.tiles_m * plan.tiles_n > 0x7fffffffll) return vs_fail(VS_ERR_UNSUPPORTED, "vs_gemm_adam_planned: too many tiles");
+    const GemmCall call{A, lda, layout_a, B, ldb, layout_b, M, N, K, 1, (hipStream_t)stream_};
+    if (plan.splits == 1) return launch_plan(compute, call, plan, epi, nullptr);
+    const size_t need = gemm_slab_bytes(plan, M, N, 1);
+    if (!workspace || workspace_bytes < need)
+        return vs_fail(VS_ERR_WORKSPACE, "vs_gemm_adam_planned: split-K needs %zu workspace bytes, got %zu", need, workspace_bytes);
+    const int rc = launch_plan(compute, call, plan, plain_epi(nullptr, N, VS_F32, 1.f), (float*)workspace);
+    if (rc != VS_OK) return rc;
+    return launch_splitk_reduce_adam((const float*)workspace, plan.splits, M, N, epi, call.stream);
+}
+
 extern "C" int vs_gemm_frame_loss(int compute, int64_t M, int64_t N, int64_t K, const void* A, int64_t lda, const void* W, int64_t ldw,
                                   const float* bias, int act, const float* full, const int32_t* t_random_dev, int ae_shift, int first_forecast,
                                   int G, int T, const float* s_old, const float* s_new, int64_t n_s, const float* t0, int64_t Bt, int64_t Ct,
diff --git a/spatiotemporal_variable_separation_amd/csrc/vs_gemm_big.h b/spatiotemporal_variable_separation_amd/csrc/vs_gemm_big.h
--- a/spatiotemporal_variable_separation_amd/csrc/vs_gemm_big.h
+++ b/spatiotemporal_variable_separation_amd/csrc/vs_gemm_big.h
@@ -75,38 +75,6 @@
     }
 }
 
-
-__device__ __forceinline__ void big_adam4(const Epi& e, const AdamCoef& c, int64_t m, int64_t n, int64_t N, const f32x4& g) {
-    const int64_t idx = m * e.ldc + n;
-    float* P = (float*)e.C + idx;
-    float* Mo = e.adam_m + idx;
-    float* Vo = e.adam_v + idx;
-    if (n + 3 < N && (e.ldc & 3) == 0 && (n & 3) == 0) {
-        f32x4 p = *reinterpret_cast<const f32x4*>(P), mm = *reinterpret_cast<const f32x4*>(Mo), vv = *reinterpret_cast<const f32x4*>(Vo);
-#pragma unroll
-        for (int t = 0; t < 4; ++t) {
-            float pe = p[t], me = mm[t], ve = vv[t];
-            vs_adam_elem(c, g[t] * e.alpha, pe, me, ve);
-            p[t] = pe; mm[t] = me; vv[t] = ve;
-        }
-        *reinterpret_cast<f32x4*>(P) = p;
-        *reinterpret_cast<f32x4*>(Mo) = mm;
-        *reinterpret_cast<f32x4*>(Vo) = vv;
-        if (e.adam_shadow) {
-            const u16x4 h = {vs_f2h(p[0], e.adam_shadow_dtype), vs_f2h(p[1], e.adam_shadow_dtype), vs_f2h(p[2], e.adam_shadow_dtype),
-                             vs_f2h(p[3], e.adam_shadow_dtype)};
-            *reinterpret_cast<u16x4*>(e.adam_shadow + idx) = h;
-        }
-    } else {
-        for (int t = 0; t < 4; ++t)
-            if (n + t < N) {
-                float pe = P[t], me = Mo[t], ve = Vo[t];
-                vs_adam_elem(c, g[t] * e.alpha, pe, me, ve);
-                P[t] = pe; Mo[t] = me; Vo[t] = ve;
-                if (e.adam_shadow) e.adam_shadow[idx + t] = vs_f2h(pe, e.adam_shadow_dtype);
-            }
-    }
-}
 
 template <bool NCHW>
 __device__ __forceinline__ void big_store4(const Epi& e, int64_t m, int64_t n, int64_t N, const f32x4& v, float* slab_row, const float* through = nullptr,
diff --git a/spatiotemporal_variable_separation_amd/csrc/vs_gemm_core.h b/spatiotemporal_variable_separation_amd/csrc/vs_gemm_core.h
--- a/spatiotemporal_variable_separation_amd/csrc/vs_gemm_core.h
+++ b/spatiotemporal_variable_separation_amd/csrc/vs_gemm_core.h
@@ -108,6 +108,46 @@
     vs_st(e.C, e.c_dtype, idx, v);
 }
 
+__device__ __forceinline__ AdamCoef epi_adam_coef(const Epi& e) {
+    return vs_adam_coef(e.adam_lr, e.adam_beta1, e.adam_beta2, e.adam_eps, (double)(e.adam_step[0] + 1 - e.adam_skipped));
+}
+
+__device__ __forceinline__ void adam_piece4(const Epi& e, const AdamCoef& c, int64_t m, int64_t n, int64_t N, const f32x4& g) {
+#pragma clang fp contract(off)
+    const int64_t idx = m * e.ldc + n;
+    float* P = (float*)e.C + idx;
+    float* Mo = e.adam_m + idx;
+    float* Vo = e.adam_v + idx;
+    unsigned short* S = e.adam_shadow ? e.adam_shadow + idx : nullptr;
+    if (n + 3 < N && (((uintptr_t)P | (uintptr_t)Mo | (uintptr_t)Vo) & 15) == 0 && ((uintptr_t)S & 7) == 0) {
+        f32x4 p = *reinterpret_cast<const f32x4*>(P), mm = *reinterpret_cast<const f32x4*>(Mo), vv = *reinterpret_cast<const f32x4*>(Vo);
+#pragma unroll
+        for (int t = 0; t < 4; ++t) {
+            float pe = p[t], me = mm[t], ve = vv[t];
+            const float gt = g[t] * e.alpha;
+            vs_adam_elem(c, gt, pe, me, ve);
+            p[t] = pe; mm[t] = me; vv[t] = ve;
+        }
+        *reinterpret_cast<f32x4*>(P) = p;
+        *reinterpret_cast<f32x4*>(Mo) = mm;
+        *reinterpret_cast<f32x4*>(Vo) = vv;
+        if (S) {
+            const u16x4 h = {vs_f2h(p[0], e.adam_shadow_dtype), vs_f2h(p[1], e.adam_shadow_dtype), vs_f2h(p[2], e.adam_shadow_dtype),
+                             vs_f2h(p[3], e.adam_shadow_dtype)};
+            *reinterpret_cast<u16x4*>(S) = h;
+        }
+    } else {
+        for (int t = 0; t < 4; ++t)
+            if (n + t < N) {
+                float pe = P[t], me = Mo[t], ve = Vo[t];
+                const float gt = g[t] * e.alpha;
+                vs_adam_elem(c, gt, pe, me, ve);
+                P[t] = pe; Mo[t] = me; Vo[t] = ve;
+                if (S) S[t] = vs_f2h(pe, e.adam_shadow_dtype);
+            }
+    }
+}
+
 __device__ __forceinline__ int64_t nchw_col_base(const Epi& e, int64_t n) {
     if (e.g_hw == 0) {
         const int64_t b = n / e.nchw_hw;
@@ -244,7 +284,7 @@
     }
 }
 
-template <int CT, class OpA, class OpB, int BM, int BN, int BK, bool NCHW = false>
+template <int CT, class OpA, class OpB, int BM, int BN, int BK, bool NCHW = false, bool ADAM = false>
 __global__ __launch_bounds__(256) void gemm_kernel(OpA A, OpB B, int64_t M, int64_t N, int64_t K,
                                                    int k_tiles_per_split, Epi epi_in, float* slabs) {
     unsigned bx = blockIdx.x, by = blockIdx.y, bz = blockIdx.z;
@@ -356,6 +396,29 @@
     }
 
     const int cj = lane & 31, rh = 4 * (lane >> 5);
+    if constexpr (ADAM) {
+        if (epi.adam_guard && *epi.adam_guard != 0u) return;
+        const AdamCoef coef = epi_adam_coef(epi);
+        static_assert((GA::ELEMS + GB::ELEMS) * sizeof(T) >= 4 * 32 * 32 * sizeof(float), "operand area too small for the staging blocks");
+        float* stg = reinterpret_cast<float*>(smem) + wave * (32 * 32);
+#pragma unroll
+        for (int i = 0; i < TM; ++i)
+#pragma unroll
+            for (int j = 0; j < TN; ++j) {
+#pragma unroll
+                for (int v = 0; v < 16; ++v) stg[((v & 3) + 8 * (v >> 2) + rh) * 32 + cj] = acc[i][j][v];
+                asm volatile("s_waitcnt lgkmcnt(0)" ::: "memory");
+#pragma unroll
+                for (int it = 0; it < 4; ++it) {
+                    const int r = it * 8 + (lane >> 3);
+                    const f32x4 g4 = *reinterpret_cast<const f32x4*>(stg + r * 32 + (lane & 7) * 4);
+                    const int64_t m = m0 + wm + 32 * i + r, n = n0 + wn + 32 * j + (lane & 7) * 4;
+                    if (m < M && n < N) adam_piece4(epi, coef, m, n, N, g4);
+                }
+                asm volatile("s_waitcnt lgkmcnt(0)" ::: "memory");
+            }
+        return;
+    }
 #pragma unroll
     for (int i = 0; i < TM; ++i)
 #pragma unroll
@@ -419,6 +482,35 @@
     }
 }
 
+__global__ __launch_bounds__(256) void splitk_reduce_adam_kernel(const float* slabs, int splits, int64_t M, int64_t N, Epi epi) {
+    if (epi.adam_guard && *epi.adam_guard != 0u) return;
+    const AdamCoef coef = epi_adam_coef(epi);
+    const int64_t total = M * N, per_row = (N + 3) / 4, pieces = M * per_row;
+    const bool slabs_vec = ((uintptr_t)slabs & 15) == 0 && (total & 3) == 0;
+    for (int64_t q = (int64_t)blockIdx.x * 256 + threadIdx.x; q < pieces; q += (int64_t)gridDim.x * 256) {
+        const int64_t m = q / per_row, n = (q - m * per_row) * 4;
+        const int64_t idx = m * N + n;
+        f32x4 g = {0.f, 0.f, 0.f, 0.f};
+        if (slabs_vec && n + 3 < N && (idx & 3) == 0) {
+#pragma unroll 4
+            for (int s = 0; s < splits; ++s) g += *reinterpret_cast<const f32x4*>(slabs + (int64_t)s * total + idx);
+        } else {
+            for (int s = 0; s < splits; ++s)
+                for (int t = 0; t < 4; ++t)
+                    if (n + t < N) g[t] += slabs[(int64_t)s * total + idx + t];
+        }
+        adam_piece4(epi, coef, m, n, N, g);
+    }
+}
+
+inline int launch_splitk_reduce_adam(const float* slabs, int splits, int64_t M, int64_t N, const Epi& epi, hipStream_t stream) {
+    int64_t blocks = vs_cdiv(M * vs_cdiv(N, 4), 256);
+    if (blocks > 2048) blocks = 2048;
+    hipLaunchKernelGGL(splitk_reduce_adam_kernel, dim3((unsigned)blocks), dim3(256), 0, stream, slabs, splits, M, N, epi);
+    VS_CHECK_LAUNCH("split-K reduce (optimizer epilogue)");
+    return VS_OK;
+}
+
 inline int launch_splitk_reduce(const float* slabs, int splits, int64_t M, int64_t N, const Epi& epi, int batch, hipStream_t stream) {
     int64_t blocks = vs_cdiv(M * N, 256);
     if (blocks > 2048) blocks = 2048;
diff --git a/spatiotemporal_variable_separation_amd/csrc/vs_gemm_mid.h b/spatiotemporal_variable_separation_amd/csrc/vs_gemm_mid.h
--- a/spatiotemporal_variable_separation_amd/csrc/vs_gemm_mid.h
+++ b/spatiotemporal_variable_separation_amd/csrc/vs_gemm_mid.h
@@ -204,7 +204,7 @@
     const int64_t nn = n0 + wc * 64 + (lane & 15) * 4;
     if constexpr (ADAM) {
         if (epi.adam_guard && *epi.adam_guard != 0u) return;
-        const AdamCoef coef = vs_adam_coef(epi.adam_lr, epi.adam_beta1, epi.adam_beta2, epi.adam_eps, (double)(epi.adam_step[0] + 1 - epi.adam_skipped));
+        const AdamCoef coef = epi_adam_coef(epi);
         if (m0 + 128 <= M && nn + 3 < N && ((epi.ldc | nn) & 3) == 0 &&
             (((uintptr_t)epi.C | (uintptr_t)epi.adam_m | (uintptr_t)epi.adam_v) & 15) == 0 && (!epi.adam_shadow || ((uintptr_t)epi.adam_shadow & 7) == 0)) {
             constexpr int G = 4;
@@ -261,7 +261,7 @@
             const int r = it * 4 + (lane >> 4);
             const int64_t m = m0 + wr * 64 + r;
             const f32x4 v4 = *reinterpret_cast<const f32x4*>(stg + r * 64 + (lane & 15) * 4);
-            if (m < M && nn < N) big_adam4(epi, coef, m, nn, N, v4);
+            if (m < M && nn < N) adam_piece4(epi, coef, m, nn, N, v4);
         }
         return;
     }
diff --git a/spatiotemporal_variable_separation_amd/ops.py b/spatiotemporal_variable_separation_amd/ops.py
--- a/spatiotemporal_variable_separation_amd/ops.py
+++ b/spatiotemporal_variable_separation_amd/ops.py
@@ -103,18 +103,33 @@
     return out
 
 
-def gemm_adam(a, layout_a, b, layout_b, M, N, K, param, exp_avg, exp_avg_sq, shadow, step_dev, skipped, lr, betas, eps, alpha=1.0):
+def gemm_plan(a, layout_a, b, layout_b, M, N, K):
+    import ctypes
+    row = (ctypes.c_int64 * 12)()
+    check(_lib.load_library().vs_gemm_plan(dtype_code(a), 1, M, N, K, a.data_ptr(), a.stride(0), 0, layout_a, b.data_ptr(), b.stride(0), 0,
+                                           layout_b, row), 'vs_gemm_plan')
+    return dict(kind=int(row[0]), bm=int(row[1]), bn=int(row[2]), splits=int(row[3]))
+
+
+def gemm_adam(a, layout_a, b, layout_b, M, N, K, param, exp_avg, exp_avg_sq, shadow, step_dev, skipped, lr, betas, eps, alpha=1.0, planned=False):
     require_cuda(a, b, param, exp_avg, exp_avg_sq, step_dev)
     lib = _lib.load_library()
     assert a.dtype == b.dtype and a.dtype in (torch.bfloat16, torch.float16) and a.stride(-1) == 1 and b.stride(-1) == 1
     assert param.dtype == torch.float32 and param.is_contiguous() and tuple(param.shape) == (M, N)
     assert exp_avg.is_contiguous() and exp_avg_sq.is_contiguous() and exp_avg.shape == param.shape == exp_avg_sq.shape
     assert shadow is None or (shadow.is_contiguous() and shadow.shape == param.shape and shadow.dtype in (torch.bfloat16, torch.float16))
-    e0 = _pb()
-    check(lib.vs_gemm_adam(dtype_code(a), M, N, K, a.data_ptr(), a.stride(0), layout_a, b.data_ptr(), b.stride(0), layout_b, float(alpha),
-                           param.data_ptr(), exp_avg.data_ptr(), exp_avg_sq.data_ptr(), _ptr(shadow),
-                           code_of(shadow.dtype) if shadow is not None else BF16, step_dev.data_ptr(), int(skipped), float(lr),
-                           float(betas[0]), float(betas[1]), float(eps), stream_ptr()), 'vs_gemm_adam')
+    args = (dtype_code(a), M, N, K, a.data_ptr(), a.stride(0), layout_a, b.data_ptr(), b.stride(0), layout_b, float(alpha),
+            param.data_ptr(), exp_avg.data_ptr(), exp_avg_sq.data_ptr(), _ptr(shadow),
+            code_of(shadow.dtype) if shadow is not None else BF16, step_dev.data_ptr(), int(skipped), float(lr),
+            float(betas[0]), float(betas[1]), float(eps))
+    if planned:
+        ws_bytes = lib.vs_gemm_workspace_bytes(M, N, K)
+        ws = _workspace(ws_bytes, a.device) if ws_bytes else None
+        e0 = _pb()
+        check(lib.vs_gemm_adam_planned(*args, _ptr(ws), ws.numel() if ws is not None else 0, stream_ptr()), 'vs_gemm_adam_planned')
+    else:
+        e0 = _pb()
+        check(lib.vs_gemm_adam(*args, stream_ptr()), 'vs_gemm_adam')
     _pe(e0, 'vs_gemm_adam<%s,%s%s>' % (_DT[dtype_code(a)], _LNAME[layout_a], _LNAME[layout_b]), flops=2.0 * M * N * K,
         nbytes=float((M * K + N * K) * a.element_size() + M * N * (24 + (2 if shadow is not None else 0))))
 
diff --git a/spatiotemporal_variable_separation_amd/optim.py b/spatiotemporal_variable_separation_amd/optim.py
--- a/spatiotemporal_variable_separation_amd/optim.py
+++ b/spatiotemporal_variable_separation_amd/optim.py
@@ -15,7 +15,7 @@
         super().__init__(params, dict(lr=lr, betas=betas, eps=eps))
         self._tables = {}
         self._buckets, self._bucket_of, self._left, self._launched, self._stream = [], {}, [], set(), None
-        self._fused, self._fused_done = [], set()
+        self._fused, self._fused_done, self._fused_planned = [], set(), set()
 
     def overlap_with_backward(self, buckets):
         assert len(self.param_groups) == 1, 'overlap_with_backward: one param group'
@@ -28,20 +28,28 @@
             for p in b:
                 p.register_post_accumulate_grad_hook(self._on_grad)
 
-    def fuse_into_wgrad(self, params):
+    def fuse_into_wgrad(self, params, planned=()):
         from . import functional as VF
         assert len(self.param_groups) == 1, 'fuse_into_wgrad: one param group'
         owned = {id(p) for p in self.param_groups[0]['params']}
         self._fused = [p for p in params if id(p) in owned and p.dim() == 2 and p.requires_grad]
         self._fused_done = set()
+        self._fused_planned = {id(p) for p in planned}
         VF.set_fused_optimizer({p: self for p in self._fused})
 
     def unfuse(self):
         from . import functional as VF
-        self._fused, self._fused_done = [], set()
+        self._fused, self._fused_done, self._fused_planned = [], set(), set()
         VF.set_fused_optimizer(None)
 
     def can_fuse(self, p, a, b):
+        if id(p) in self._fused_planned:
+            if not (getattr(self, '_scale_state', None) is None and p.is_contiguous() and p.dtype == torch.float32 and a.dtype == b.dtype
+                    and a.dtype in (torch.bfloat16, torch.float16) and a.stride(-1) == 1 and b.stride(-1) == 1):
+                return False
+            from . import ops
+            plan = ops.gemm_plan(a, _lib.LAYOUT_S, b, _lib.LAYOUT_S, p.shape[0], p.shape[1], a.shape[0])
+            return plan['splits'] > 1 or plan['kind'] == 0
         return (getattr(self, '_scale_state', None) is None and p.is_contiguous() and p.dtype == torch.float32 and a.dtype == b.dtype
                 and a.dtype in (torch.bfloat16, torch.float16) and a.data_ptr() % 16 == 0 and b.data_ptr() % 16 == 0
                 and a.stride(0) % 8 == 0 and b.stride(0) % 8 == 0 and p.shape[0] % 8 == 0 and p.shape[1] % 8 == 0)
@@ -54,7 +62,7 @@
         st = self.state[p]
         shadow = VF.shadow_buffer_for_update(p)
         ops.gemm_adam(a, layout_a, b, layout_b, M, N, K, p, st['exp_avg'], st['exp_avg_sq'], shadow, group['step_dev'], st.get('skipped', 0),
-                      group['lr'], group['betas'], group['eps'])
+                      group['lr'], group['betas'], group['eps'], planned=id(p) in self._fused_planned)
         torch.autograd.graph.increment_version(p)
         if shadow is not None:
             VF.shadows_written([p])
diff --git a/spatiotemporal_variable_separation_amd/profiling.py b/spatiotemporal_variable_separation_amd/profiling.py
--- a/spatiotemporal_variable_separation_amd/profiling.py
+++ b/spatiotemporal_variable_separation_amd/profiling.py
@@ -18,7 +18,7 @@
 
 
 GROUPS = [
-    ('vs_gemm_adam', r'^vs_gemm_adam<', r'gemm_mid_kernel<\d, \d, \d, \w+, \d+, true>', 'hbm'),
+    ('vs_gemm_adam', r'^vs_gemm_adam<', r'gemm_mid_kernel<\d, \d, \d, \w+, \d+, true>|::gemm_kernel<.*?, \d+, \d+, \d+, \w+, true>\(|splitk_reduce_adam_kernel', 'hbm'),
     ('vs_mlp_rollout_fwd', r'^vs_mlp_rollout_fwd<', r'rollout_(ws|fwd)_kernel<\d+, true|rollout_fwd_kernel', 'mfma'),
     ('vs_mlp_rollout_bwd', r'^vs_mlp_rollout_bwd<', r'rollout_ws_kernel<\d+, false|rollout_bwd_kernel', 'mfma'),
     ('vs_conv_k4s2', r'^vs_conv_k4s2:|^vs_space_to_depth2', r'conv3_band_kernel<\d, \d+, \d+, \d, 1>|conv3_band2_kernel<\d, \d+, \d, 1, \d+>|wgrad3_band_kernel<\d, \d+, \d, 1(, \d)?>|wgrad2_band_kernel<\d, \d+, 1>|space_to_depth2_kernel|'
diff --git a/spatiotemporal_variable_separation_amd/train.py b/spatiotemporal_variable_separation_amd/train.py
--- a/spatiotemporal_variable_separation_amd/train.py
+++ b/spatiotemporal_variable_separation_amd/train.py
@@ -540,10 +540,15 @@
         return False
     if grad_sync is not None or scaler is not None or not _mlp_family(sep_net) or len(optimizer.param_groups) != 1 or optimizer._buckets:
         return False
-    big = [p for p in chain_weight_parameters(sep_net) if p.numel() >= min_numel]
-    if not big:
+    weights = chain_weight_parameters(sep_net)
+    big = [p for p in weights if p.numel() >= min_numel]
+    small = []
+    if os.environ.get('VARSEP_FUSE_ADAM_SMALL', '1') == '1':
+        encoders = {id(q) for mod in (sep_net.Es, sep_net.Et) for q in mod.parameters()}
+        small = [p for p in weights if p.numel() < min_numel and id(p) in encoders]
+    if not big and not small:
         return False
-    optimizer.fuse_into_wgrad(big)
+    optimizer.fuse_into_wgrad(big + small, planned=small)
     return True
 
 
```

Result: faster. 2.178 million frames/s (median of 6 runs) (+12.7%).
